# jltsiren/gbwt-rs

Measured on AMD Instinct MI355X. Metric: LF-steps/sec (batched path extract), higher is better.
Workload: dtype u32; 1 GPU; bubble-chain GBZ, 5000 paths x 1000002 nodes (333334 sites, mosaic, seed 42), all forward sequences -> device CSR; index replicated, path p walked by GPU p mod 1; lf_steps_per_gpu=3333340000, index_bytes=59619086, records=2000005

## Files before the change

### gbwt_rs_amd/_lib.py

```python
import ctypes as C
import os
import sys

HERE = os.path.dirname(os.path.abspath(__file__))
CSRC = os.path.join(HERE, "csrc")
LIB_PATH = os.environ.get("GBWT_HIP_LIB") or os.path.join(CSRC, "libgbwt_hip.so")
HEADER = os.path.join(os.path.dirname(HERE), "include", "gbwt_hip.h")

OPEN_EXTRACT, OPEN_SEARCH, OPEN_GFA, OPEN_ALL = 1, 2, 4, 7
OK, INVALID_DATA, IO_ERROR, BAD_ARGUMENT, NO_DEVICE, DEVICE_ERROR, CAPACITY, UNSUPPORTED = range(8)
STATUS_NAMES = ["OK", "INVALID_DATA", "IO_ERROR", "BAD_ARGUMENT", "NO_DEVICE", "DEVICE_ERROR", "CAPACITY", "UNSUPPORTED"]


class Pos(C.Structure):
    _fields_ = [("node", C.c_uint64), ("offset", C.c_uint64)]


class State(C.Structure):
    _fields_ = [("node", C.c_uint64), ("start", C.c_uint64), ("end", C.c_uint64)]


class BdState(C.Structure):
    _fields_ = [("forward", State), ("reverse", State)]


class Stats(C.Structure):
    _fields_ = [("size", C.c_uint64), ("sequences", C.c_uint64), ("alphabet_size", C.c_uint64),
                ("alphabet_offset", C.c_uint64), ("records", C.c_uint64), ("data_bytes", C.c_uint64),
                ("paths", C.c_uint64), ("bidirectional", C.c_uint32), ("has_metadata", C.c_uint32),
                ("is_gbz", C.c_uint32), ("has_translation", C.c_uint32), ("max_record_len", C.c_uint64),
                ("max_outdegree", C.c_uint64)]


class OpenTimes(C.Structure):
    _fields_ = [("parse_ms", C.c_double), ("upload_ms", C.c_double), ("sample_ms", C.c_double), ("total_ms", C.c_double),
                ("samples", C.c_uint64), ("checkpoint_walkers", C.c_uint64), ("checkpoint_orphans", C.c_uint64), ("checkpoint_sampling", C.c_uint32),
                ("checkpoint_rounds", C.c_uint32), ("line_sizes_ms", C.c_double)]


class Memory(C.Structure):
    _fields_ = [("index_device_bytes", C.c_uint64), ("index_host_bytes", C.c_uint64), ("workspace_device_bytes", C.c_uint64),
                ("rows_bytes", C.c_uint64), ("text_bytes", C.c_uint64), ("rows_chunks", C.c_uint64)]


class UniqueId(C.Structure):
    _fields_ = [("bytes", C.c_ubyte * 128)]


class CommStats(C.Structure):
    _fields_ = [("ms", C.c_double), ("bytes", C.c_uint64), ("staged_send", C.c_uint32), ("reserved", C.c_uint32)]


class Paths(C.Structure):
    _fields_ = [("d_offsets", C.c_void_p), ("d_nodes", C.c_void_p), ("total", C.c_uint64), ("n", C.c_uint64)]


class States(C.Structure):
    _fields_ = [("d_states", C.c_void_p), ("d_valid", C.c_void_p), ("n", C.c_uint64)]


class Lines(C.Structure):
    _fields_ = [("d_text", C.c_void_p), ("d_line_offsets", C.c_void_p), ("total", C.c_uint64), ("n", C.c_uint64)]


class Components(C.Structure):
    _fields_ = [("d_component", C.c_void_p), ("d_offsets", C.c_void_p), ("d_nodes", C.c_void_p), ("d_path_component", C.c_void_p),
                ("min_node", C.c_uint64), ("slots", C.c_uint64), ("components", C.c_uint64), ("nodes", C.c_uint64), ("paths", C.c_uint64)]


class ComponentsTimes(C.Structure):
    _fields_ = [("hook_ms", C.c_float), ("jump_ms", C.c_float), ("shape_ms", C.c_float), ("hook_launches", C.c_uint32),
                ("jump_launches", C.c_uint32), ("shape_launches", C.c_uint32)]


class EdgeRows(C.Structure):
    _fields_ = [("d_offsets", C.c_void_p), ("d_edges", C.c_void_p), ("d_valid", C.c_void_p), ("total", C.c_uint64), ("n", C.c_uint64)]


class GraphText(C.Structure):
    _fields_ = [("d_text", C.c_void_p), ("header_bytes", C.c_uint64), ("segment_bytes", C.c_uint64), ("link_bytes", C.c_uint64),
                ("segments", C.c_uint64), ("links", C.c_uint64)]


class SuffixArray(C.Structure):
    _fields_ = [("d_sa", C.c_void_p), ("d_bwt", C.c_void_p), ("total", C.c_uint64), ("bwt_runs", C.c_uint64)]


class SuffixArrayInfo(C.Structure):
    _fields_ = [("n", C.c_uint64), ("peak_scratch_bytes", C.c_uint64), ("planned_scratch_bytes", C.c_uint64), ("bwt_runs", C.c_uint64),
                ("active", C.c_uint64 * 64), ("rounds", C.c_uint32), ("rank_bits", C.c_uint32), ("text_ms", C.c_float), ("pack_ms", C.c_float),
                ("rank_ms", C.c_float), ("output_ms", C.c_float), ("round_ms", C.c_float * 64)]


FM_COUNT_ONLY = 1


class FmIndexInfo(C.Structure):
    _fields_ = [(name, C.c_uint64) for name in ("n", "sigma", "block_rows", "blocks", "primary", "index_bytes", "planned_index_bytes", "sa_bytes", "peak_scratch_bytes",
                                                "planned_scratch_bytes", "queries", "last_patterns", "last_steps", "last_total")] + \
               [(name, C.c_uint32) for name in ("packed", "count_only", "path_level", "reserved")] + \
               [(name, C.c_float) for name in ("suffix_array_ms", "histogram_ms", "codes_ms", "counts_ms", "fill_ms", "narrow_ms", "last_count_ms", "last_fill_ms")]


class FmLocated(C.Structure):
    _fields_ = [("d_offsets", C.c_void_p), ("d_values", C.c_void_p), ("d_ranges", C.c_void_p), ("total", C.c_uint64), ("m", C.c_uint64)]


class ReferencePath(C.Structure):
    _fields_ = [("path_id", C.c_uint64), ("len", C.c_uint64), ("first", C.c_uint64), ("count", C.c_uint64)]


class ReferencePosition(C.Structure):
    _fields_ = [("offset", C.c_uint64), ("pos", Pos)]


class Located(C.Structure):
    _fields_ = [("d_offsets", C.c_void_p), ("d_ids", C.c_void_p), ("d_valid", C.c_void_p), ("total", C.c_uint64), ("n", C.c_uint64)]


class LocateInfo(C.Structure):
# ... 219 lines not shown
```

### gbwt_rs_amd/csrc/capi_open.hip

```cpp
#include <hip/hip_runtime.h>

#include <algorithm>
#include <cstdio>
#include <cstdlib>
#include <cstring>
#include <memory>
#include <mutex>
#include <new>
#include <atomic>
#include <chrono>
#include <string>
#include <thread>
#include <vector>

#include "capi_internal.hpp"

using namespace gbwt_hip;


namespace gbwt_hip {
std::string &last_error_slot() {
    thread_local std::string slot;
    return slot;
}
// ... 180 lines not shown
    HIP_CHECK(hipMemcpy(&bad, flags.ptr, sizeof(uint32_t), hipMemcpyDeviceToHost));
    HIP_CHECK(hipGetLastError());
    if (bad != 0) throw InvalidData("BWT: record starts are not sorted offsets into the data");
    ix.starts_uploaded = true;
}

void records_to_device(gbwt_hip_index &ix, OpenTrace &trace) {
    const HostIndex &h = ix.host;
    if (h.alphabet_size > (uint64_t(1) << 32)) throw Unsupported("alphabet_size > 2^32 is not supported (u32 node ids on device)");
    HIP_CHECK(hipSetDevice(ix.device));
    const uint64_t n_records = ix.stats.records;
    const uint64_t data_bytes = ix.stats.data_bytes;
    if (!ix.record_bytes_uploaded) {
        ix.data.reserve(data_bytes + DATA_PAD);
        HIP_CHECK(hipMemset(ix.data.ptr, 0, data_bytes + DATA_PAD));
    }
    DeviceIndex &d = ix.dev;
    d = DeviceIndex{};
    d.data = ix.data.as<uint8_t>();
    d.data_len = data_bytes;
    d.n_records = n_records;
    d.n_sequences = h.sequences;
    d.alphabet_offset = static_cast<uint32_t>(h.alphabet_offset);
    d.first_node = static_cast<uint32_t>(h.alphabet_offset + 1);
    const bool narrow_starts = data_bytes < (uint64_t(1) << 32);
    if (!ix.starts_uploaded) upload_starts(ix);
    if (!ix.record_bytes_uploaded && data_bytes) HIP_CHECK(hipMemcpy(ix.data.ptr, h.record_bytes(), data_bytes, hipMemcpyHostToDevice));
    if (narrow_starts) d.starts32 = ix.starts.as<uint32_t>(); else d.starts64 = ix.starts.as<uint64_t>();
    trace.mark("record bytes + starts to the device");
}

void build_descriptors(gbwt_hip_index &ix, uint64_t *d_stats, DeviceBuffer &counts, DeviceBuffer &scan_tmp, OpenTrace &trace) {
    const HostIndex &h = ix.host;
    DeviceIndex &d = ix.dev;
    const uint64_t n_records = d.n_records, nr = std::max<uint64_t>(n_records, 1);
    if (ix.caps & GBWT_HIP_OPEN_EXTRACT) ix.desc.reserve(nr * 4 * sizeof(uint4));
    ix.desc_raw.reserve(nr * 4 * sizeof(uint4));
    ix.block_base.reserve(nr * sizeof(uint32_t));
    counts.reserve(nr * sizeof(uint32_t));
    trace.mark("starts + allocations");
    launch_build_desc(d, ix.desc_raw.as<uint4>(), counts.as<uint32_t>(), d_stats, nullptr);
    trace.mark("k_build_desc");
    d.desc_raw = ix.desc_raw.as<uint4>();
    d.desc = ix.desc.as<uint4>();
    uint64_t n_blocks = 1;
    if (n_records > 0) {
        if (n_records >= (uint64_t(1) << 30)) throw Unsupported("more than 2^30 records are not supported");
        if ((h.size >> RANK_BLOCK_SHIFT) + n_records >= 0xFFFFFFF0ull) throw Unsupported("index too large for 32-bit rank block indices");
        size_t tb = block_scan_temp_bytes(n_records);
        scan_tmp.reserve(std::max<size_t>(tb, 16));
        launch_block_scan(counts.as<uint32_t>(), ix.block_base.as<uint32_t>(), n_records, scan_tmp.ptr, tb, nullptr);
        uint32_t last_base = 0, last_count = 0;
        HIP_CHECK(hipMemcpy(&last_base, ix.block_base.as<uint32_t>() + (n_records - 1), sizeof(uint32_t), hipMemcpyDeviceToHost));
        HIP_CHECK(hipMemcpy(&last_count, counts.as<uint32_t>() + (n_records - 1), sizeof(uint32_t), hipMemcpyDeviceToHost));
        n_blocks += static_cast<uint64_t>(last_base) + last_count;
        launch_finish_block_base(counts.as<uint32_t>(), ix.block_base.as<uint32_t>(), n_records, ix.desc_raw.as<uint4>(), nullptr);
    }
    ix.blocks.reserve(n_blocks * sizeof(uint4));
    HIP_CHECK(hipMemsetAsync(ix.blocks.ptr, 0, sizeof(uint4), nullptr));
    d.block_base = ix.block_base.as<uint32_t>();
    d.blocks = ix.blocks.as<uint4>();
    d.n_blocks = n_blocks;
    trace.mark("block scan + allocation");
    if (n_blocks > 1) launch_fill_blocks(d, counts.as<uint32_t>(), ix.block_base.as<uint32_t>(), ix.blocks.as<uint4>(), nullptr);
    trace.mark("k_fill_blocks");
}

uint64_t layout_walks(gbwt_hip_index &ix, uint64_t *d_stats, const DeviceBuffer &counts, OpenTrace &trace) {
    const HostIndex &h = ix.host;
    const OpenKnobs &k = ix.knobs;
    DeviceIndex &d = ix.dev;
    const uint64_t n_records = d.n_records, n_blocks = d.n_blocks;
    launch_link_desc(d, ix.desc.as<uint4>(), nullptr);
    const uint32_t hops = k.lookahead_hops;
    launch_link_lookahead(d, ix.desc.as<uint4>(), counts.as<uint32_t>(), hops, nullptr);
    ix.desc2.reserve(std::max<uint64_t>(n_records, 1) * 8 * sizeof(uint4));
    d.desc2 = ix.desc2.as<uint4>();
    uint32_t gather_limit = k.gather_limit;
    if (n_blocks >= (uint64_t(1) << 31)) gather_limit = 0;
    ix.packed_blocks = gather_limit != 0;
    trace.mark("link + lookahead + allocations");
    const uint32_t chain_max = k.chains.value_or(CHAIN_MAX);
    HIP_CHECK(hipMemsetAsync(d_stats + 6, 0, sizeof(uint64_t), nullptr));
    launch_link_desc2(d, ix.desc2.as<uint4>(), gather_limit, chain_max | (h.bidirectional ? 0x100u : 0u), reinterpret_cast<uint32_t *>(d_stats + 5), nullptr);
    ix.gblocks.reserve((gather_limit ? n_blocks : 1) * 2 * sizeof(uint4));
    HIP_CHECK(hipMemsetAsync(ix.gblocks.ptr, 0, 2 * sizeof(uint4), nullptr));
    d.gblocks = ix.gblocks.as<uint4>();
    uint64_t early_stats[6] = {0, 0, 0, 0, 0, 0};
    HIP_CHECK(hipMemcpy(early_stats, d_stats, sizeof(early_stats), hipMemcpyDeviceToHost));
    d.chained = static_cast<uint32_t>(early_stats[5] & 0xFFFFFFFFu);
    if (d.chained != 0 && !k.chains && (early_stats[5] >> 32) * 1000 < n_records) {
        HIP_CHECK(hipMemset(d_stats + 5, 0, 2 * sizeof(uint64_t)));
        launch_link_desc2(d, ix.desc2.as<uint4>(), gather_limit, h.bidirectional ? 0x100u : 0u, reinterpret_cast<uint32_t *>(d_stats + 5), nullptr);
        d.chained = 0;
    }
    if (trace.on) std::fprintf(stderr, "[open] records with a chained step: %llu of %llu (up to %u nodes per iteration)\n",
                               static_cast<unsigned long long>(early_stats[5] >> 32), static_cast<unsigned long long>(n_records), d.chained);
    const uint64_t longest = early_stats[0];
    const bool full_width_now = gather_limit == 0 || longest >= gather_limit;
    if (full_width_now) {
        ix.cblocks.reserve(n_blocks * 2 * sizeof(uint4));
        HIP_CHECK(hipMemsetAsync(ix.cblocks.ptr, 0, 2 * sizeof(uint4), nullptr));
    }
    if (n_blocks > 1) launch_fill_two_step_blocks(d, full_width_now ? ix.cblocks.as<uint4>() : nullptr, gather_limit ? ix.gblocks.as<uint4>() : nullptr, nullptr);
    if (full_width_now) d.cblocks = ix.cblocks.as<uint4>();
    trace.mark("two-step descriptors + blocks");
    launch_link_lookahead2(d, ix.desc2.as<uint4>(), counts.as<uint32_t>(), std::max<uint32_t>(1, (hops + 1) / 2), nullptr);
    return early_stats[4];
}

void build_tables(gbwt_hip_index &ix, uint64_t generic_records, DeviceBuffer &scan_tmp) {
    const OpenKnobs &k = ix.knobs;
    DeviceIndex &d = ix.dev;
    const uint64_t n_records = d.n_records;
    if (n_records == 0 || generic_records == 0) return;
    const bool for_extract = (ix.caps & GBWT_HIP_OPEN_EXTRACT) != 0;
    DeviceBuffer positions, sigmas, table_base, edge_base, edges;
    positions.reserve(n_records * sizeof(uint64_t)); sigmas.reserve(n_records * sizeof(uint64_t));
    table_base.reserve((n_records + 1) * sizeof(uint64_t)); edge_base.reserve((n_records + 1) * sizeof(uint64_t));
    launch_table_counts(d, positions.as<uint64_t>(), sigmas.as<uint64_t>(), nullptr);
    const size_t tb = scan_temp_bytes(n_records);
    scan_tmp.reserve(std::max<size_t>(tb, 16));
    launch_scan(positions.as<uint64_t>(), table_base.as<uint64_t>(), n_records, scan_tmp.ptr, tb, nullptr);
    launch_scan(sigmas.as<uint64_t>(), edge_base.as<uint64_t>(), n_records, scan_tmp.ptr, tb, nullptr);
    uint64_t total_positions = 0, total_edges = 0;
    HIP_CHECK(hipMemcpy(&total_positions, table_base.as<uint64_t>() + n_records, sizeof(uint64_t), hipMemcpyDeviceToHost));
    HIP_CHECK(hipMemcpy(&total_edges, edge_base.as<uint64_t>() + n_records, sizeof(uint64_t), hipMemcpyDeviceToHost));
    uint64_t budget = uint64_t(16) << 30;
    {
        size_t free_bytes = 0, total_bytes = 0;
        if (hipMemGetInfo(&free_bytes, &total_bytes) == hipSuccess) budget = std::min<uint64_t>(total_bytes / 4, free_bytes / 2);
        else (void)hipGetLastError();
    }
    if (k.table_bytes) budget = *k.table_bytes;
    if (total_positions == 0 || total_positions >= 0xFFFFFFFFull || total_positions * sizeof(uint4) > budget) return;
    ix.tables.reserve(total_positions * sizeof(uint4));
    edges.reserve(std::max<uint64_t>(total_edges, 1) * sizeof(uint2));
    d.tables = ix.tables.as<uint4>();
    launch_fill_tables(d, ix.desc_raw.as<uint4>(), table_base.as<uint64_t>(), edge_base.as<uint64_t>(), ix.tables.as<uint4>(), edges.as<uint2>(), nullptr);
    HIP_CHECK(hipDeviceSynchronize());
    HIP_CHECK(hipGetLastError());
    if (!(for_extract && 2 * total_positions * sizeof(uint4) <= budget && n_records <= 0x7FFFFFFFull && k.walk_tables)) return;
    ix.wtables.reserve(total_positions * sizeof(uint4));
    launch_fill_wtables(d, ix.wtables.as<uint4>(), nullptr);
    HIP_CHECK(hipDeviceSynchronize());
    HIP_CHECK(hipGetLastError());
    d.wtables = ix.wtables.as<uint4>();
    ix.table_positions = total_positions;
    if (6 * total_positions * sizeof(uint4) <= budget && k.deep_tables) {
        ix.wtables_deep.reserve(total_positions * 4 * sizeof(uint4));
        launch_fill_wtables_deep(d, ix.wtables_deep.as<uint4>(), k.compact_tables, nullptr);
        HIP_CHECK(hipDeviceSynchronize());
        HIP_CHECK(hipGetLastError());
        d.wtables_deep = ix.wtables_deep.as<uint4>();
    }
}

void record_stats_and_endmarker(gbwt_hip_index &ix, const uint64_t (&hs)[8], const Endmarker *early_endmarker) {
    ix.stats.max_record_len = hs[0];
    ix.stats.max_outdegree = hs[1];
    if (ix.caps & GBWT_HIP_OPEN_EXTRACT) ix.slow_records = hs[6] & 0xFFFFFFFFull;
    if (hs[2] != 0) throw InvalidData("BWT: record without a readable outdegree");
    if (hs[0] >= (uint64_t(1) << 32)) throw Unsupported("a record with 2^32 or more positions is not supported (u32 offsets on device)");
    DeviceIndex &d = ix.dev;
    d.max_walk = hs[3];
    const Endmarker endmarker = early_endmarker ? *early_endmarker : decompress_endmarker(ix.host, std::max<uint64_t>(hs[0], 1));
    const uint64_t end_len = endmarker.size();
    ix.endmarker.reserve(std::max<uint64_t>(end_len, 1) * sizeof(uint2));
    static_assert(sizeof(std::pair<uint32_t, uint32_t>) == sizeof(uint2), "pairs are uploaded as uint2");
    if (end_len > 0) HIP_CHECK(hipMemcpy(ix.endmarker.ptr, endmarker.data(), end_len * sizeof(uint2), hipMemcpyHostToDevice));
    d.endmarker = ix.endmarker.as<uint2>();
    d.n_endmarker = end_len;
}

uint64_t all_nodes(const HostIndex &h) { return h.size >= h.sequences ? h.size - h.sequences : 0; }

uint32_t sample_interval(gbwt_hip_index &ix) {
    const HostIndex &h = ix.host;
    const DeviceIndex &d = ix.dev;
    const uint64_t nodes = all_nodes(h);
    uint32_t interval = 64;
    while (interval < 2048 && (nodes >> 22) > interval) interval *= 2;
    while (interval < 2048 && ((nodes / h.sequences) >> 12) > interval) interval *= 2;
    if (d.wtables_deep != nullptr && 3 * ix.table_positions >= h.size)
        while (interval < 512 && (interval < 128 || (nodes >> 17) > interval)) interval *= 2;
    ix.sample_coarse = 1;
    if (ix.knobs.sample_interval) interval = *ix.knobs.sample_interval;
    else if (interval >= 1024 && d.chained == 0) {
        const uint32_t coarse = ix.knobs.sample_coarse.value_or(interval / 512);
        ix.sample_coarse = coarse; interval = std::max(64u, interval / coarse);
    }
    return interval;
}

enum class Sampling { checkpoints, one_walk, two_pass };

Sampling walk_every_sequence(gbwt_hip_index &ix, Sampling how, uint32_t interval, const DeviceBuffer &prints, uint64_t *d_stats, DeviceBuffer &pool,
                             DeviceBuffer &tags, uint64_t &pooled) {
    const HostIndex &h = ix.host;
    DeviceIndex &d = ix.dev;
    uint32_t *d_flags = reinterpret_cast<uint32_t *>(d_stats);
    d.cblocks = ensure_cblocks(&ix);
    if (how == Sampling::one_walk) {
        const uint64_t pool_capacity = all_nodes(h) / std::max<uint32_t>(interval, 1) + 2 * h.sequences + 1024;
        pool.reserve(pool_capacity * sizeof(uint4)); tags.reserve(pool_capacity * sizeof(uint2));
        HIP_CHECK(hipMemset(d_stats + 2, 0, sizeof(uint64_t)));
        HIP_CHECK(hipMemsetAsync(d_flags + 1, 0, sizeof(uint32_t), nullptr));
        launch_lengths_and_samples(d, interval, ix.seq_len.as<uint32_t>(), pool.as<uint4>(), tags.as<uint2>(), d_stats + 2, pool_capacity, d_flags, nullptr);
        HIP_CHECK(hipMemcpy(&pooled, d_stats + 2, sizeof(uint64_t), hipMemcpyDeviceToHost));
        if (pooled <= pool_capacity) return Sampling::one_walk;
    }
    HIP_CHECK(hipMemsetAsync(d_flags + 1, 0, sizeof(uint32_t), nullptr));
    launch_sequence_lengths(d, ix.seq_len.as<uint32_t>(), prints.as<uint64_t>(), d_flags, nullptr);
    return Sampling::two_pass;
}

void samples_after_walk(gbwt_hip_index &ix, Sampling how, uint32_t interval, const DeviceBuffer &pool, const DeviceBuffer &tags, uint64_t pooled) {
    const HostIndex &h = ix.host;
    DeviceBuffer counts, scan_tmp;
    counts.reserve(h.sequences * sizeof(uint64_t));
    ix.sample_base.reserve((h.sequences + 1) * sizeof(uint64_t));
    launch_sample_counts(ix.seq_len.as<uint32_t>(), h.sequences, interval, counts.as<uint64_t>(), nullptr);
    const size_t tb = scan_temp_bytes(h.sequences);
    scan_tmp.reserve(std::max<size_t>(tb, 16));
    launch_scan(counts.as<uint64_t>(), ix.sample_base.as<uint64_t>(), h.sequences, scan_tmp.ptr, tb, nullptr);
    uint64_t total_samples = 0;
    HIP_CHECK(hipMemcpy(&total_samples, ix.sample_base.as<uint64_t>() + h.sequences, sizeof(uint64_t), hipMemcpyDeviceToHost));
    ix.samples.reserve(std::max<uint64_t>(total_samples, 1) * sizeof(uint4));
    if (how == Sampling::one_walk) launch_place_samples(ix.seq_len.as<uint32_t>(), pool.as<uint4>(), tags.as<uint2>(), pooled, ix.sample_base.as<uint64_t>(), h.sequences,
                                                        ix.samples.as<uint4>(), nullptr);
    else launch_record_samples(ix.dev, ix.sample_base.as<uint64_t>(), interval, ix.samples.as<uint4>(), nullptr);
    HIP_CHECK(hipDeviceSynchronize());
    HIP_CHECK(hipGetLastError());
    ix.times.samples = total_samples;
    std::vector<uint64_t> base(h.sequences + 1);
    HIP_CHECK(hipMemcpy(base.data(), ix.sample_base.ptr, base.size() * sizeof(uint64_t), hipMemcpyDeviceToHost));
    note_sample_counts(ix, base);
}

void lengths_and_samples(gbwt_hip_index &ix, uint64_t *d_stats, OpenTrace &trace) {
    const HostIndex &h = ix.host;
    DeviceIndex &d = ix.dev;
    const auto t_samples = std::chrono::steady_clock::now();
    ix.seq_len.reserve(h.sequences * sizeof(uint32_t));
// ... 291 lines not shown
```

### gbwt_rs_amd/csrc/device_index.hpp

```cpp
#pragma once

#include <cstdint>

namespace gbwt_hip {

constexpr uint32_t DESC_UNARY = 0xFFFFFFFFu;
constexpr uint32_t EDGE_EMIT2 = 1u << 31;
constexpr uint32_t EDGE_CONT = 1u << 30;
constexpr uint32_t DESC_SLOW = 1u << 31;
constexpr uint32_t LOOKAHEAD_COUNT_MASK = (1u << 29) - 1;
constexpr uint32_t REC_MASK = (1u << 30) - 1;
constexpr uint32_t LEAF_EMIT2 = 1u << 31;
constexpr uint32_t DESC2_SLOW = 1u << 30;
constexpr uint32_t GATHER_OK = 1u;
constexpr uint32_t E_CHAIN = 2u;
constexpr uint32_t E_ALL4 = 8u;
constexpr uint32_t E_ANYCHAIN = 4u;
constexpr uint32_t LEAF_CHAIN = 1u << 30;
constexpr uint32_t CHAIN_MAX = 6;
constexpr uint32_t WT_TABLE = 1u << 30;
constexpr uint32_t WT_DEEP_STEPS = 7;
constexpr uint32_t WT_COMPACT_STEPS = 12;
constexpr uint32_t WT_COMPACT = 1u << 30;
constexpr uint32_t WT_COMPACT_TABLE = 1u << 29;
constexpr uint32_t BLOCK_NONE = 0xFFFFFFFFu;
constexpr uint32_t RANK_BLOCK_SHIFT = 6;
constexpr uint32_t DATA_PAD = 128;

struct DeviceIndex {
    const uint8_t *data;
    const uint32_t *starts32;
    const uint64_t *starts64;
    const uint2 *endmarker;
    const uint4 *desc;
    const uint4 *desc_raw;
    const uint32_t *block_base;
    const uint4 *blocks;
    const uint4 *desc2;
    const uint4 *tables;
    const uint4 *wtables;
    const uint4 *wtables_deep;
    const uint32_t *seq_len;
    const uint4 *samples;
    const uint64_t *sample_base;
    uint32_t sample_interval;
    uint32_t sample_stride;
    uint32_t sample_part, sample_parts;
    const uint4 *cblocks;
    const uint4 *gblocks;
    uint64_t data_len;
    uint64_t n_records;
    uint64_t n_sequences;
    uint64_t n_endmarker;
    uint64_t n_blocks;
    uint64_t max_walk;
    uint32_t alphabet_offset;
    uint32_t first_node;
    uint32_t chained;
};

struct RowSegments { uint64_t base, stride, count, lo, hi; };
__device__ inline RowSegments row_segments(const DeviceIndex &ix, uint64_t id) {
    RowSegments r;
    r.stride = ix.sample_stride ? ix.sample_stride : 1u;
    r.base = ix.sample_base[id];
    r.count = (ix.sample_base[id + 1] - r.base + r.stride - 1) / r.stride;
    r.lo = 0; r.hi = r.count;
    if (ix.sample_parts > 1) { r.lo = r.count * ix.sample_part / ix.sample_parts; r.hi = r.count * (ix.sample_part + 1) / ix.sample_parts; }
    return r;
}
__device__ inline uint64_t segment_position(const DeviceIndex &ix, const RowSegments &r, uint64_t id, uint64_t j) {
    return j == 0 ? 0u : (j < r.count ? ix.samples[r.base + j * r.stride].w : ix.seq_len[id]);
}

__host__ __device__ inline uint32_t chain_stride(uint32_t x, uint32_t L) { return L > x ? 2u : 0xFFFFFFFEu; }
__host__ __device__ inline uint32_t chain_mids(uint32_t x, uint32_t L) { return (L > x ? L - x : x - L) / 2 - 1; }

__host__ __device__ inline uint32_t desc_body_offset(uint32_t meta) { return meta & 0xFFFFu; }
__host__ __device__ inline uint32_t desc_class(uint32_t meta) { return (meta >> 16) & 3u; }
__host__ __device__ inline uint64_t desc_start(uint32_t start_lo, uint32_t meta) { return (static_cast<uint64_t>(meta >> 24) << 32) | start_lo; }

}
```

### gbwt_rs_amd/csrc/kernels.hpp

```cpp
#pragma once

#include <hip/hip_runtime.h>

#include <cstdint>

#include "../../include/gbwt_hip.h"
#include "device_index.hpp"

namespace gbwt_hip {

constexpr uint32_t POOL_BLOCK_NODES = 256;
constexpr uint32_t POOL_NONE = 0xFFFFFFFFu;

constexpr uint32_t FLAG_POOL_OVERFLOW = 1u;

void launch_build_desc(const DeviceIndex &ix, uint4 *d_desc, uint32_t *d_block_counts, uint64_t *d_stats, hipStream_t stream);
size_t block_scan_temp_bytes(uint64_t n);
void launch_block_scan(const uint32_t *d_counts, uint32_t *d_block_base, uint64_t n, void *d_temp, size_t temp_bytes, hipStream_t stream);
void launch_finish_block_base(const uint32_t *d_counts, uint32_t *d_block_base, uint64_t n, uint4 *d_desc_raw , hipStream_t stream);
void launch_link_desc(const DeviceIndex &ix, uint4 *d_desc, hipStream_t stream);
void launch_link_lookahead(const DeviceIndex &ix, uint4 *d_desc, const uint32_t *d_block_counts, uint32_t hops, hipStream_t stream);
void launch_table_counts(const DeviceIndex &ix, uint64_t *d_positions, uint64_t *d_sigmas, hipStream_t stream);
void launch_fill_tables(const DeviceIndex &ix, uint4 *d_desc_raw, const uint64_t *d_table_base, const uint64_t *d_edge_base, uint4 *d_tables,
                        uint2 *d_edges, hipStream_t stream);
void launch_fill_wtables(const DeviceIndex &ix, uint4 *d_wtables, hipStream_t stream);
void launch_fill_wtables_deep(const DeviceIndex &ix, uint4 *d_deep, bool compact, hipStream_t stream);
void launch_link_desc2(const DeviceIndex &ix, uint4 *d_desc2, uint32_t gather_limit, uint32_t chain_max, uint32_t *d_chained, hipStream_t stream);
void launch_fill_two_step_blocks(const DeviceIndex &ix, uint4 *d_cblocks , uint4 *d_gblocks , hipStream_t stream);
void launch_link_lookahead2(const DeviceIndex &ix, uint4 *d_desc2, const uint32_t *d_block_counts, uint32_t hops, hipStream_t stream);
void launch_fill_blocks(const DeviceIndex &ix, const uint32_t *d_block_counts, const uint32_t *d_block_base, uint4 *d_blocks, hipStream_t stream);

struct WalkArgs {
    const uint64_t *seq_ids;
    uint64_t n;
    uint32_t *pool;
    uint32_t *next;
    uint32_t pool_blocks;
    uint32_t *counter;
    uint32_t *head;
    uint64_t *lengths;
    uint32_t *flags;
    uint32_t mode;
    uint32_t paths_per_wave;
    uint32_t small_record;
    uint32_t pack16;
    uint32_t helper_lanes;
    uint32_t wide_addresses;
    uint32_t *out_nodes;
    const uint64_t *out_offsets;
    uint32_t both_ends;
    uint32_t ring_slots;
    uint32_t helper_naps;
    uint32_t row_piece;
    uint32_t xcd_map;
    uint32_t uniform_loop;
    uint32_t headroom;
    uint32_t all4;
    uint32_t catch_up;
    uint32_t gather_reach;
    uint32_t packed_blocks;
    uint32_t debug;
    const uint32_t *sorted_rows;
    const uint64_t *level;
    uint64_t walkers;
    uint64_t capacity;
    uint32_t segments;
    uint32_t uniform_len;
    uint64_t *fill_offsets;
};
constexpr uint32_t WALK_TWO_STEP = 0, WALK_LANE_SERIAL = 1, WALK_COOP = 2, WALK_ONE_STEP = 3;
void launch_walk(const DeviceIndex &ix, const WalkArgs &args, hipStream_t stream);
void launch_sequence_lengths(const DeviceIndex &ix, uint32_t *d_seq_len, uint64_t *d_prints, uint32_t *d_overflow, hipStream_t stream);
void launch_check_orientation_pairs(const uint32_t *d_seq_len, const uint64_t *d_prints, uint64_t n_pairs, uint32_t *d_mismatch, hipStream_t stream);
void launch_gather_lengths(const uint32_t *d_seq_len, uint64_t n_sequences, const uint64_t *d_ids, uint64_t n, uint64_t *d_lengths, uint32_t *d_max_len, hipStream_t stream);
void launch_lengths_and_samples(const DeviceIndex &ix, uint32_t interval, uint32_t *d_seq_len, uint4 *d_pool, uint2 *d_tags, uint64_t *d_counter,
                                uint64_t capacity, uint32_t *d_overflow, hipStream_t stream);
void launch_place_samples(const uint32_t *d_seq_len, const uint4 *d_pool, const uint2 *d_tags, uint64_t pooled, const uint64_t *d_sample_base,
                          uint64_t n_sequences, uint4 *d_samples, hipStream_t stream);
void launch_sample_counts(const uint32_t *d_seq_len, uint64_t n_sequences, uint32_t interval, uint64_t *d_counts, hipStream_t stream);
void launch_record_samples(const DeviceIndex &ix, const uint64_t *d_sample_base, uint32_t interval, uint4 *d_samples, hipStream_t stream);
struct CheckpointWalk {
    const uint64_t *cp_first;
    uint4 *summaries;
    uint64_t *orphan_count;
    uint64_t orphan_capacity, positions;
    uint32_t threshold, cap;
    uint32_t packed;
    uint32_t *flags;
};
void launch_checkpoint_counts(const DeviceIndex &ix, uint32_t threshold, uint64_t *d_counts, hipStream_t stream);
void launch_checkpoint_walk(const DeviceIndex &ix, const CheckpointWalk &w, hipStream_t stream);
void launch_chase_counts(const DeviceIndex &ix, const uint4 *d_summaries, uint64_t n_summaries, uint4 *d_spans, uint32_t *d_seq_len, uint64_t *d_counts,
                         uint32_t *d_overflow, hipStream_t stream);
void launch_chase_samples(const DeviceIndex &ix, const uint4 *d_summaries, uint64_t n_summaries, const uint4 *d_spans, const uint64_t *d_sample_base,
                          uint4 *d_samples, hipStream_t stream);
constexpr uint32_t GFA_LINE_CHUNK = 4096;
struct LineCacheFill {
    const uint32_t *label_len;
    uint64_t n_labels;
    uint64_t paths;
    uint32_t max_samples;
    const uint64_t *chunk_first;
    uint64_t chunks;
    uint64_t *chunk_text;
    uint64_t *path_totals;
    uint32_t *chunk_seg;
    uint64_t *seg_text;
    uint32_t *flags;
};
void launch_fill_line_cache(const DeviceIndex &ix, const LineCacheFill &f, bool packed, hipStream_t stream);
// ... 78 lines not shown
```

### gbwt_rs_amd/csrc/knobs.hpp

```cpp
#pragma once

#include <algorithm>
#include <cstdint>
#include <cstdlib>
#include <optional>

#include "device_index.hpp"
#include "extract_knobs.hpp"

struct OpenKnobs {
    bool seq_len = true;
    std::optional<uint32_t> sample_interval;
    std::optional<uint32_t> sample_coarse;
    bool serial_samples = false;
    bool two_pass = false;
    bool orientation_check = false;
    std::optional<double> checkpoint_gap;
    std::optional<uint32_t> checkpoint_cap;
    std::optional<uint32_t> chains;
    uint32_t gather_limit = 1u << 21;
    uint32_t lookahead_hops = 15;
    bool walk_tables = true, deep_tables = true, compact_tables = true;
    std::optional<uint64_t> table_bytes;
    bool line_cache = true;
    uint32_t locate_interval = 64;
    bool trace = false;
    static OpenKnobs from_env() {
        OpenKnobs k;
        const auto on = [](const char *name) { const char *v = std::getenv(name); return !(v && std::atoi(v) == 0); };
        const auto forced = [](const char *name) { const char *v = std::getenv(name); return v && std::atoi(v) != 0; };
        k.seq_len = on("GBWT_HIP_SEQ_LEN");
        if (const char *v = std::getenv("GBWT_HIP_SAMPLE_INTERVAL")) k.sample_interval = static_cast<uint32_t>(std::max(0, std::atoi(v)));
        if (const char *v = std::getenv("GBWT_HIP_SAMPLE_COARSE")) k.sample_coarse = static_cast<uint32_t>(std::max(1, std::atoi(v)));
        k.serial_samples = forced("GBWT_HIP_SERIAL_SAMPLES");
        k.two_pass = forced("GBWT_HIP_TWO_PASS_OPEN");
        k.orientation_check = forced("GBWT_HIP_ORIENTATION_CHECK");
        if (const char *v = std::getenv("GBWT_HIP_CHECKPOINT_GAP")) k.checkpoint_gap = std::max(2.0, std::atof(v));
        if (const char *v = std::getenv("GBWT_HIP_CHECKPOINT_CAP")) k.checkpoint_cap = static_cast<uint32_t>(std::max(1, std::atoi(v)));
        if (const char *v = std::getenv("GBWT_HIP_CHAINS")) k.chains = static_cast<uint32_t>(std::min<long>(gbwt_hip::CHAIN_MAX, std::max<long>(0, std::atol(v))));
        if (const char *v = std::getenv("GBWT_HIP_GATHER_LIMIT")) k.gather_limit = static_cast<uint32_t>(std::min<long>(1l << 21, std::max<long>(0, std::atol(v))));
        if (const char *v = std::getenv("GBWT_HIP_LOOKAHEAD_HOPS")) k.lookahead_hops = static_cast<uint32_t>(std::max(0, std::atoi(v)));
        k.walk_tables = on("GBWT_HIP_WALK_TABLES"); k.deep_tables = on("GBWT_HIP_DEEP_TABLES"); k.compact_tables = on("GBWT_HIP_COMPACT_TABLES");
        if (const char *v = std::getenv("GBWT_HIP_TABLE_BYTES")) k.table_bytes = std::strtoull(v, nullptr, 10);
        k.line_cache = on("GBWT_HIP_LINE_CACHE");
        if (const char *v = std::getenv("GBWT_HIP_LOCATE_INTERVAL")) k.locate_interval = static_cast<uint32_t>(std::min<long>(1l << 30, std::max<long>(0, std::atol(v))));
        k.trace = std::getenv("GBWT_HIP_TRACE_OPEN") != nullptr;
        return k;
    }
    static bool lazy_host_records() {
        static const bool lazy = [] { const char *e = std::getenv("GBWT_HIP_LAZY_HOST_RECORDS"); return !(e && e[0] == '0'); }();
        return lazy;
    }
};
```

### gbwt_rs_amd/csrc/load_kernels.hip

```cpp
#include "kernels.hpp"

#include <hipcub/hipcub.hpp>

#include "device_common.hpp"
#include "lf_device.hpp"

namespace gbwt_hip {

namespace {


__device__ __forceinline__ uint4 stream_bytes16(const uint8_t *data, uint64_t pos, uint64_t limit) {
    uint32_t w[4] = {0, 0, 0, 0};
    for (uint32_t k = 0; k < 16 && pos + k < limit; k++) w[k >> 2] |= static_cast<uint32_t>(data[pos + k]) << (8 * (k & 3));
    return make_uint4(w[0], w[1], w[2], w[3]);
}

__global__ void __launch_bounds__(256) k_build_desc(DeviceIndex ix, uint4 *desc, uint32_t *block_counts, uint64_t *stats) {
    const uint64_t rec = blockIdx.x * static_cast<uint64_t>(blockDim.x) + threadIdx.x;
    uint64_t stat_len = 0, stat_sigma = 0, stat_bad = 0, stat_generic = 0;
    if (rec < ix.n_records) {
    uint64_t start, limit;
    record_bounds(ix, rec, start, limit);
    uint4 A = make_uint4(0, 0, 0, 0), B = make_uint4(0, 0, 0, 0), C = make_uint4(0, 0, 0, 0), D = make_uint4(0, 0, 0, 0);
    uint32_t n_blocks = 0;
    if (limit > start) {
        ByteCursor c(ix.data, start, limit);
        uint64_t sigma = 0;
        const bool readable = c.varint(sigma);
        if (!readable) stat_bad = 1;
        if (readable && sigma != 0) {
            stat_sigma = sigma;
            B.x = static_cast<uint32_t>(start); B.y = static_cast<uint32_t>(limit - start);
            B.z = static_cast<uint32_t>((start >> 32) & 0xFF) << 24;
            bool classed = false;
            if (sigma <= 2 && (start >> 40) == 0) {
                uint64_t n0 = 0, o0 = 0, d1 = 0, o1 = 0;
                bool good = c.varint(n0) && c.varint(o0);
                if (good && sigma == 2) good = c.varint(d1) && c.varint(o1);
                const uint64_t body = c.pos - start;
                if (good && body <= 0xFFFF && n0 + d1 <= 0xFFFFFFFFull && o0 <= 0xFFFFFFFFull && o1 <= 0xFFFFFFFFull) {
                    RunDecoder rd(sigma);
                    uint64_t total = 0, total0 = 0, runs = 0, value, len;
                    bool lean = true;
                    for (;;) {
                        const uint64_t before = c.pos;
                        if (!rd.next(c, value, len)) break;
                        if (c.pos - before > 5) lean = false;
                        total += len; runs++;
                        if (value == 0) total0 += len;
                    }
                    if (!c.at_end() || runs == 0) lean = false;
                    if (lean && total < 0xFFFFFFFFull) {
                        classed = true;
                        stat_len = total;
                        A.x = static_cast<uint32_t>(n0); A.y = static_cast<uint32_t>(o0);
                        A.z = static_cast<uint32_t>(n0 + d1); A.w = static_cast<uint32_t>(o1);
                        B.z |= static_cast<uint32_t>(body) | (static_cast<uint32_t>(sigma) << 16);
                        B.w = static_cast<uint32_t>(total);
                        C.x = static_cast<uint32_t>(total0); C.y = static_cast<uint32_t>(total);
                        D = stream_bytes16(ix.data, start + body, limit);
                        if (sigma == 1) B.y = DESC_UNARY;
                        else n_blocks = static_cast<uint32_t>((total >> RANK_BLOCK_SHIFT) + 1);
                    }
                }
            }
            if (!classed) {
                stat_generic = rec != 0 ? 1 : 0;
                A = make_uint4(0, 0, 0, 0); C = make_uint4(0, 0, 0, 0); D = make_uint4(0, 0, 0, 0); B.w = 0;
                uint64_t total = ix.n_sequences;
                if (rec != 0) {
                    ByteCursor c2(ix.data, start, limit);
                    uint64_t s2 = 0;
                    c2.varint(s2);
                    total = record_len(c2, s2);
                }
                stat_len = total;
                C.y = total < 0xFFFFFFFFull ? static_cast<uint32_t>(total) : 0xFFFFFFFFu;
            }
        }
    }
    desc[4 * rec] = A;
    desc[4 * rec + 1] = B;
    desc[4 * rec + 2] = C;
    desc[4 * rec + 3] = D;
    block_counts[rec] = n_blocks;
    }
// ... 193 lines not shown
        if (compact) {
            uint32_t node[2 * WT_COMPACT_STEPS];
            uint4 f = e;
            bool ok = true;
            for (uint32_t k = 0; k < WT_COMPACT_STEPS && ok; k++) {
                if (k > 0) f = ix.wtables[static_cast<uint64_t>(f.w) + f.y];
                const bool table_next = (f.z & WT_TABLE) != 0;
                ok = f.x != 0 && (f.z & LEAF_EMIT2) != 0 && (f.z & REC_MASK) != 0 && (table_next || k + 1 == WT_COMPACT_STEPS);
                node[2 * k] = f.x; node[2 * k + 1] = (f.z & REC_MASK) + ix.alphabet_offset;
            }
            for (uint32_t k = 1; k < 2 * WT_COMPACT_STEPS && ok; k++) {
                const int64_t d = static_cast<int64_t>(node[k]) - static_cast<int64_t>(node[k - 1]);
                ok = d >= -32768 && d <= 32767;
            }
            if (ok) {
                w[0] = node[0];
                w[1] = WT_COMPACT | ((f.z & WT_TABLE) ? WT_COMPACT_TABLE : 0u);
                for (uint32_t q = 0; q < 12; q++) {
                    const uint32_t a = 2 * q + 1, b = 2 * q + 2;
                    const uint32_t lo = (node[a] - node[a - 1]) & 0xFFFFu;
                    const uint32_t hi = b < 2 * WT_COMPACT_STEPS ? ((node[b] - node[b - 1]) & 0xFFFFu) : 0u;
                    w[2 + q] = lo | (hi << 16);
                }
                w[14] = f.y; w[15] = f.w;
                uint4 *out = deep + 4 * (static_cast<uint64_t>(C.z) + i);
                out[0] = make_uint4(w[0], w[1], w[2], w[3]);
                out[1] = make_uint4(w[4], w[5], w[6], w[7]);
                out[2] = make_uint4(w[8], w[9], w[10], w[11]);
                out[3] = make_uint4(w[12], w[13], w[14], w[15]);
                continue;
            }
        }
        bool going = true;
#pragma unroll
        for (uint32_t k = 0; k < WT_DEEP_STEPS; k++) {
            if (going) {
                if (k > 0) e = ix.wtables[static_cast<uint64_t>(e.w) + e.y];
                w[2 * k] = e.x; w[2 * k + 1] = e.z & ~WT_TABLE;
                going = (e.z & REC_MASK) != 0 && (e.z & WT_TABLE) != 0;
            } else {
                w[2 * k] = 0u; w[2 * k + 1] = e.z & REC_MASK;
            }
        }
        if ((e.z & REC_MASK) != 0 && (e.z & WT_TABLE) != 0) w[2 * WT_DEEP_STEPS - 1] |= WT_TABLE;
        w[14] = e.y; w[15] = e.w;
        uint4 *out = deep + 4 * (static_cast<uint64_t>(C.z) + i);
        out[0] = make_uint4(w[0], w[1], w[2], w[3]);
        out[1] = make_uint4(w[4], w[5], w[6], w[7]);
        out[2] = make_uint4(w[8], w[9], w[10], w[11]);
        out[3] = make_uint4(w[12], w[13], w[14], w[15]);
    }
}

__device__ __forceinline__ uint32_t extend_chain(const DeviceIndex &ix, uint32_t x, uint32_t &w, uint64_t &base, uint64_t count, uint32_t room, bool bidirectional) {
    const uint4 *raw = ix.desc_raw;
    const uint32_t first = w + ix.alphabet_offset;
    if (first != x + 2u && first != x - 2u) return 0;
    const uint32_t d = chain_stride(x, first);
    uint32_t added = 0;
    while (added < room) {
        const uint4 WA = raw[4 * static_cast<uint64_t>(w)], WB = raw[4 * static_cast<uint64_t>(w) + 1];
        if (WB.y != DESC_UNARY || WA.x == 0 || WA.x != w + ix.alphabet_offset + d) break;
        if (bidirectional) {
            uint64_t rev = 0;
            if (!landing_record(ix, (w + ix.alphabet_offset) ^ 1u, rev) || raw[4 * rev + 1].y != DESC_UNARY) break;
        }
        uint64_t next = 0;
        if (!landing_record(ix, WA.x, next)) break;
        const uint4 NB = raw[4 * next + 1];
        const uint64_t base2 = base + WA.y;
        if (NB.y == 0 || base2 + count > 0xFFFFFFFFull || !(desc_class(NB.z) == 0 || base2 + count <= NB.w)) break;
        w = static_cast<uint32_t>(next); base = base2; added++;
    }
    return added;
}

__device__ __forceinline__ uint64_t edge_positions(const DeviceIndex &ix, uint64_t r, uint32_t e) {
    const uint4 B = ix.desc_raw[4 * r + 1], C = ix.desc_raw[4 * r + 2];
    const uint32_t cls = B.y != 0 ? desc_class(B.z) : 0u;
    if (cls == 2) return e ? B.w - C.x : C.x;
    return cls == 1 && e == 0 ? B.w : 0u;
}

__global__ void __launch_bounds__(256) k_link_desc2(DeviceIndex ix, uint4 *out, uint32_t gather_limit, uint32_t chain_max, uint32_t *chained) {
    uint64_t v = blockIdx.x * static_cast<uint64_t>(blockDim.x) + threadIdx.x;
    if (v >= ix.n_records) return;
    const uint4 *d1 = ix.desc;
    const uint4 D = d1[4 * v + 2];
    const uint4 VB = ix.desc_raw[4 * v + 1];
    const uint32_t cls_v = VB.y != 0 ? desc_class(VB.z) : 0u;
    uint32_t n1[2] = {0, 0}, base[2] = {0, 0}, wword[2] = {0, 0}, chain[2] = {0, 0};
    bool any_chain = false;
    uint4 leaf[4] = {make_uint4(0, 0, 0, BLOCK_NONE), make_uint4(0, 0, 0, BLOCK_NONE), make_uint4(0, 0, 0, BLOCK_NONE), make_uint4(0, 0, 0, BLOCK_NONE)};
    const bool slow = (D.x & DESC_SLOW) != 0;
    if (!slow) {
        for (uint32_t a = 0; a < 2; a++) {
            const uint4 E = d1[4 * v + a];
            const uint32_t f = a ? D.w : D.y;
            n1[a] = E.x; base[a] = E.y;
            if (!(f & EDGE_CONT)) continue;
            uint32_t w = E.z, wbb = E.w;
            if ((f & EDGE_EMIT2) && chain_max != 0) {
                uint64_t chained_base = base[a];
                if (extend_chain(ix, E.x, w, chained_base, edge_positions(ix, v, a), chain_max & 0xFFu, (chain_max >> 8) != 0) != 0) {
                    base[a] = static_cast<uint32_t>(chained_base); wbb = ix.block_base[w]; chain[a] = E_CHAIN; any_chain = true;
                }
            }
            wword[a] = w | ((f & EDGE_EMIT2) ? LEAF_EMIT2 : 0u);
            const uint4 WD = d1[4 * static_cast<uint64_t>(w) + 2];
            const uint4 WB = ix.desc_raw[4 * static_cast<uint64_t>(w) + 1];
            const uint32_t cls_w = WB.y != 0 ? desc_class(WB.z) : 0u;
            const bool real = !(WD.x & DESC_SLOW) && (cls_w == 1 || (cls_w == 2 && cls_v == 2));
            if (!real) { leaf[2 * a] = make_uint4(0u, 0u, w, wbb); continue; }
            for (uint32_t b = 0; b < cls_w; b++) {
                const uint4 WE = d1[4 * static_cast<uint64_t>(w) + b];
                const uint32_t wf = b ? WD.w : WD.y;
                const bool cont = (wf & EDGE_CONT) != 0;
                uint32_t land = WE.z, lbb = WE.w, lflag = 0;
                uint64_t lbase = WE.y;
                if (cont && (wf & EDGE_EMIT2) && chain_max != 0 && extend_chain(ix, WE.x, land, lbase, edge_positions(ix, w, b), chain_max & 0xFFu, (chain_max >> 8) != 0) != 0) {
                    lbb = ix.block_base[land]; lflag = LEAF_CHAIN; any_chain = true;
                }
                leaf[2 * a + b] = make_uint4(WE.x, static_cast<uint32_t>(lbase), cont ? (land | lflag | ((wf & EDGE_EMIT2) ? LEAF_EMIT2 : 0u)) : 0u, cont ? lbb : BLOCK_NONE);
            }
        }
    }
    bool packed = VB.w < gather_limit;
    for (uint32_t a = 0; a < 2; a++)
        if (wword[a] & REC_MASK) packed = packed && ix.desc_raw[4 * static_cast<uint64_t>(wword[a] & REC_MASK) + 1].w < gather_limit;
    bool all4 = !slow && !any_chain && cls_v != 0;
    for (uint32_t a = 0; a < cls_v && all4; a++) {
        all4 = n1[a] != 0 && (wword[a] & LEAF_EMIT2) != 0;
        const uint4 WB = ix.desc_raw[4 * static_cast<uint64_t>(wword[a] & REC_MASK) + 1];
        const uint32_t cls_w = WB.y != 0 ? desc_class(WB.z) : 0u;
        all4 = all4 && cls_w != 0;
        for (uint32_t b = 0; b < cls_w && all4; b++) all4 = leaf[2 * a + b].x != 0 && (leaf[2 * a + b].z & LEAF_EMIT2) != 0;
    }
    if (slow && VB.y != 0 && chained != nullptr) atomicAdd(chained + 2, 1u);
    uint4 *o = out + 8 * v;
    o[0] = make_uint4(n1[0], base[0], wword[0] | (slow ? DESC2_SLOW : 0u), (packed ? GATHER_OK : 0u) | chain[0] | (any_chain ? E_ANYCHAIN : 0u) | (all4 ? E_ALL4 : 0u));
    o[1] = make_uint4(n1[1], base[1], wword[1] | (slow ? DESC2_SLOW : 0u), (packed ? GATHER_OK : 0u) | chain[1]);
    if (any_chain && chained != nullptr) {
        uint32_t most = 0;
        for (uint32_t a = 0; a < 2; a++) {
            const uint32_t first = 2u + (chain[a] ? chain_mids(n1[a], (wword[a] & REC_MASK) + ix.alphabet_offset) : 0u);
            for (uint32_t b = 0; b < 2; b++) {
                const uint4 l = leaf[2 * a + b];
                most = max(most, first + 2u + ((l.z & LEAF_CHAIN) ? chain_mids(l.x, (l.z & REC_MASK) + ix.alphabet_offset) : 0u));
            }
        }
        if (*chained < most) atomicMax(chained, most);
    }
    {
        const uint64_t lanes = __ballot(any_chain && chained != nullptr);
        if (lanes != 0 && (threadIdx.x % WAVE) == static_cast<uint32_t>(__ffsll(static_cast<unsigned long long>(lanes)) - 1)) atomicAdd(chained + 1, static_cast<uint32_t>(__popcll(lanes)));
    }
    o[2] = leaf[0]; o[3] = leaf[1]; o[4] = leaf[2]; o[5] = leaf[3];
    o[6] = make_uint4(0u, 0u, 0u, 0u);
    o[7] = make_uint4(0u, 0u, 0u, 0u);
}

struct SecondStep { const uint4 *wblocks[2]; uint32_t wbase[2]; };

template <class Mask>
__device__ __forceinline__ Mask second_step_bits(const uint4 *wblocks, uint32_t j, Mask m, uint32_t &R) {
    const uint32_t q = j >> RANK_BLOCK_SHIFT, sh = j & 63u;
    const uint32_t cnt = sizeof(Mask) == 8 ? __popcll(m) : __popc(static_cast<uint32_t>(m));
    const uint4 W0 = wblocks[q];
    const uint64_t w0 = (static_cast<uint64_t>(W0.y) << 32) | W0.x;
    R = W0.z + __popcll(w0 & ((uint64_t(1) << sh) - 1));
    uint64_t val = w0 >> sh;
    if (sh != 0 && cnt > 64 - sh) {
        const uint4 W1 = wblocks[q + 1];
        val |= ((static_cast<uint64_t>(W1.y) << 32) | W1.x) << (64 - sh);
    }
    Mask bits2 = 0;
    while (m) {
        const Mask low = m & (~m + 1);
        if (val & 1) bits2 |= low;
        val >>= 1;
        m ^= low;
    }
    return bits2;
}

__global__ void __launch_bounds__(256) k_fill_two_step_blocks(DeviceIndex ix, uint4 *cblocks, uint4 *gblocks) {
    const uint64_t b = blockIdx.x * static_cast<uint64_t>(blockDim.x) + threadIdx.x + 1;
    if (b >= ix.n_blocks) return;
    const uint4 P = ix.blocks[b];
    const uint64_t v = P.w;
    const uint4 *d1 = ix.desc;
    const uint4 D = d1[4 * v + 2];
    const uint32_t len = ix.desc_raw[4 * v + 1].w;
    const uint32_t bb = ix.block_base[v];
    const uint32_t k = static_cast<uint32_t>(b - bb);
    SecondStep s2{{nullptr, nullptr}, {0, 0}};
    if (!(D.x & DESC_SLOW)) {
        for (uint32_t a = 0; a < 2; a++) {
            const uint4 E = ix.desc2[8 * v + a];
            const uint64_t w = E.z & REC_MASK;
            if (w == 0) continue;
            const uint4 WB = ix.desc_raw[4 * w + 1];
            if ((d1[4 * w + 2].x & DESC_SLOW) || WB.y == 0 || desc_class(WB.z) != 2) continue;
            s2.wblocks[a] = ix.blocks + ix.block_base[w];
            s2.wbase[a] = E.y;
        }
    }
    {
        const uint64_t bits1 = (static_cast<uint64_t>(P.y) << 32) | P.x;
        const uint32_t remaining = len - (k << RANK_BLOCK_SHIFT) > len ? 0u : len - (k << RANK_BLOCK_SHIFT);
        const uint64_t valid = remaining >= 64 ? ~uint64_t(0) : ((uint64_t(1) << remaining) - 1);
        uint64_t bits2 = 0, m_of[2] = {0, 0};
        uint32_t R[2] = {0, 0};
        for (uint32_t a = 0; a < 2; a++) {
            const uint64_t m = (a ? bits1 : ~bits1) & valid;
            if (!s2.wblocks[a] || m == 0) continue;
            m_of[a] = m;
            const uint32_t before = a ? P.z : (k << RANK_BLOCK_SHIFT) - P.z;
            bits2 |= second_step_bits<uint64_t>(s2.wblocks[a], s2.wbase[a] + before, m, R[a]);
        }
        if (cblocks != nullptr) {
            cblocks[2 * static_cast<uint64_t>(bb + k)] = make_uint4(P.x, P.y, static_cast<uint32_t>(bits2), static_cast<uint32_t>(bits2 >> 32));
            cblocks[2 * static_cast<uint64_t>(bb + k) + 1] = make_uint4(P.z, R[0], R[1], 0u);
        }
        if (gblocks == nullptr) return;
        const uint32_t lo2 = static_cast<uint32_t>(bits2), hi2 = static_cast<uint32_t>(bits2 >> 32);
        uint32_t Rlo[2], Rhi[2];
        for (uint32_t a = 0; a < 2; a++) {
            const uint32_t mlo = static_cast<uint32_t>(m_of[a]), mhi = static_cast<uint32_t>(m_of[a] >> 32);
            Rlo[a] = mlo ? R[a] : 0u;
            Rhi[a] = mhi ? R[a] + __popc(lo2 & mlo) : 0u;
        }
        const uint32_t ones_hi = P.z + __popc(P.x);
        gblocks[2 * static_cast<uint64_t>(bb + k)] = make_uint4(P.x, lo2, (P.z & 0x1FFFFFu) | (Rlo[0] << 21), ((Rlo[0] >> 11) & 0x3FFu) | (Rlo[1] << 10));
        gblocks[2 * static_cast<uint64_t>(bb + k) + 1] = make_uint4(P.y, hi2, (ones_hi & 0x1FFFFFu) | (Rhi[0] << 21), ((Rhi[0] >> 11) & 0x3FFu) | (Rhi[1] << 10));
    }
}

__global__ void __launch_bounds__(256) k_link_lookahead2(DeviceIndex ix, uint4 *desc2, const uint32_t *block_counts, uint32_t hops) {
    uint64_t v = blockIdx.x * static_cast<uint64_t>(blockDim.x) + threadIdx.x;
    if (v >= ix.n_records) return;
    uint64_t r = v;
    bool good = true;
    for (uint32_t h = 0; h < hops && good; h++) {
        if (desc2[8 * r].z & DESC2_SLOW) { good = false; break; }
        const uint32_t x = desc2[8 * r + 2].z & REC_MASK;
        if (x == 0) good = false; else r = x;
    }
    uint4 look = make_uint4(0u, 0u, 0u, 0u);
    if (good && r != v) {
        look.x = static_cast<uint32_t>(r);
        if (ix.block_base[r] != BLOCK_NONE) { look.y = ix.block_base[r]; look.z = block_counts[r]; }
    }
    desc2[8 * v + 6] = look;
}

__global__ void __launch_bounds__(256) k_fill_blocks(DeviceIndex ix, const uint32_t *block_counts, const uint32_t *block_base, uint4 *blocks) {
    uint64_t rec = blockIdx.x * static_cast<uint64_t>(blockDim.x) + threadIdx.x;
    if (rec >= ix.n_records) return;
    const uint32_t count = block_counts[rec];
    if (count == 0) return;
    const uint4 B = ix.desc_raw[4 * rec + 1];
    const uint64_t start = desc_start(B.x, B.z), limit = start + B.y;
    ByteCursor c(ix.data, start + desc_body_offset(B.z), limit);
    RunDecoder rd(desc_class(B.z));
    uint4 *out = blocks + block_base[rec];
    uint64_t bits = 0, value, len;
    uint32_t k = 0, fill = 0, ones = 0;
    while (k < count && rd.next(c, value, len)) {
        while (len > 0 && k < count) {
            const uint32_t take = static_cast<uint32_t>(len < 64 - fill ? len : 64 - fill);
            if (value) bits |= (take == 64 ? ~uint64_t(0) : ((uint64_t(1) << take) - 1)) << fill;
            fill += take; len -= take;
            if (fill == 64) {
                out[k++] = make_uint4(static_cast<uint32_t>(bits), static_cast<uint32_t>(bits >> 32), ones, static_cast<uint32_t>(rec));
                ones += __popcll(bits);
                bits = 0; fill = 0;
            }
        }
    }
    if (k < count) out[k] = make_uint4(static_cast<uint32_t>(bits), static_cast<uint32_t>(bits >> 32), ones, static_cast<uint32_t>(rec));
}

}

void launch_build_desc(const DeviceIndex &ix, uint4 *d_desc, uint32_t *d_block_counts, uint64_t *d_stats, hipStream_t stream) {
    if (ix.n_records == 0) return;
    hipLaunchKernelGGL(k_build_desc, dim3(grid_for(ix.n_records, 256)), dim3(256), 0, stream, ix, d_desc, d_block_counts, d_stats);
}

void launch_link_desc(const DeviceIndex &ix, uint4 *d_desc, hipStream_t stream) {
    if (ix.n_records == 0) return;
    hipLaunchKernelGGL(k_link_desc, dim3(grid_for(ix.n_records, 256)), dim3(256), 0, stream, ix, d_desc);
}

void launch_link_lookahead(const DeviceIndex &ix, uint4 *d_desc, const uint32_t *d_block_counts, uint32_t hops, hipStream_t stream) {
    if (ix.n_records == 0) return;
    hipLaunchKernelGGL(k_link_lookahead, dim3(grid_for(ix.n_records, 256)), dim3(256), 0, stream, ix, d_desc, d_block_counts, hops);
}

void launch_table_counts(const DeviceIndex &ix, uint64_t *d_positions, uint64_t *d_sigmas, hipStream_t stream) {
    if (ix.n_records == 0) return;
    hipLaunchKernelGGL(k_table_counts, dim3(grid_for(ix.n_records, 256)), dim3(256), 0, stream, ix, d_positions, d_sigmas);
}

void launch_fill_tables(const DeviceIndex &ix, uint4 *d_desc_raw, const uint64_t *d_table_base, const uint64_t *d_edge_base, uint4 *d_tables,
                        uint2 *d_edges, hipStream_t stream) {
    if (ix.n_records == 0) return;
    hipLaunchKernelGGL(k_fill_tables, dim3(grid_for(ix.n_records, 64)), dim3(64), 0, stream, ix, d_desc_raw, d_table_base, d_edge_base, d_tables, d_edges);
}

void launch_fill_wtables(const DeviceIndex &ix, uint4 *d_wtables, hipStream_t stream) {
    if (ix.n_records == 0 || ix.n_records > 0x7FFFFFFFull) return;
    hipLaunchKernelGGL(k_fill_wtables, dim3(static_cast<unsigned>(ix.n_records)), dim3(256), 0, stream, ix, d_wtables);
}

void launch_fill_wtables_deep(const DeviceIndex &ix, uint4 *d_deep, bool compact, hipStream_t stream) {
    if (ix.n_records == 0 || ix.n_records > 0x7FFFFFFFull || ix.wtables == nullptr) return;
    hipLaunchKernelGGL(k_fill_wtables_deep, dim3(static_cast<unsigned>(ix.n_records)), dim3(256), 0, stream, ix, d_deep, compact ? 1u : 0u);
}

void launch_link_desc2(const DeviceIndex &ix, uint4 *d_desc2, uint32_t gather_limit, uint32_t chain_max, uint32_t *d_chained, hipStream_t stream) {
    if (ix.n_records == 0) return;
    hipLaunchKernelGGL(k_link_desc2, dim3(grid_for(ix.n_records, 256)), dim3(256), 0, stream, ix, d_desc2, gather_limit, chain_max, d_chained);
}

void launch_fill_two_step_blocks(const DeviceIndex &ix, uint4 *d_cblocks, uint4 *d_gblocks, hipStream_t stream) {
    if (ix.n_records == 0 || (d_cblocks == nullptr && d_gblocks == nullptr)) return;
    if (ix.n_blocks <= 1) return;
    hipLaunchKernelGGL(k_fill_two_step_blocks, dim3(grid_for(ix.n_blocks - 1, 256)), dim3(256), 0, stream, ix, d_cblocks, d_gblocks);
}

void launch_link_lookahead2(const DeviceIndex &ix, uint4 *d_desc2, const uint32_t *d_block_counts, uint32_t hops, hipStream_t stream) {
    if (ix.n_records == 0) return;
    hipLaunchKernelGGL(k_link_lookahead2, dim3(grid_for(ix.n_records, 256)), dim3(256), 0, stream, ix, d_desc2, d_block_counts, hops);
}

void launch_fill_blocks(const DeviceIndex &ix, const uint32_t *d_block_counts, const uint32_t *d_block_base, uint4 *d_blocks, hipStream_t stream) {
    if (ix.n_records == 0) return;
    hipLaunchKernelGGL(k_fill_blocks, dim3(grid_for(ix.n_records, 256)), dim3(256), 0, stream, ix, d_block_counts, d_block_base, d_blocks);
}

__global__ void __launch_bounds__(256) k_finish_block_base(const uint32_t *counts, uint32_t *block_base, uint64_t n, uint4 *desc_raw) {
    uint64_t rec = blockIdx.x * static_cast<uint64_t>(blockDim.x) + threadIdx.x;
    if (rec >= n) return;
    const uint32_t bb = counts[rec] == 0 ? BLOCK_NONE : block_base[rec] + 1;
    block_base[rec] = bb;
    if (bb != BLOCK_NONE && desc_raw != nullptr) reinterpret_cast<uint32_t *>(desc_raw + 4 * rec + 2)[2] = bb;
}

size_t block_scan_temp_bytes(uint64_t n) {
    size_t bytes = 0;
    (void)hipcub::DeviceScan::ExclusiveSum(nullptr, bytes, static_cast<const uint32_t *>(nullptr), static_cast<uint32_t *>(nullptr), static_cast<int>(n));
    return bytes;
}

void launch_block_scan(const uint32_t *d_counts, uint32_t *d_block_base, uint64_t n, void *d_temp, size_t temp_bytes, hipStream_t stream) {
    if (n == 0) return;
    (void)hipcub::DeviceScan::ExclusiveSum(d_temp, temp_bytes, d_counts, d_block_base, static_cast<int>(n), stream);
}

void launch_finish_block_base(const uint32_t *d_counts, uint32_t *d_block_base, uint64_t n, uint4 *d_desc_raw, hipStream_t stream) {
    if (n) hipLaunchKernelGGL(k_finish_block_base, dim3(grid_for(n, 256)), dim3(256), 0, stream, d_counts, d_block_base, n, d_desc_raw);
}

__global__ void __launch_bounds__(256) k_ef_counts(const uint64_t *high, uint64_t n, uint64_t *counts) {
    const uint64_t i = blockIdx.x * static_cast<uint64_t>(blockDim.x) + threadIdx.x;
    if (i < n) counts[i] = static_cast<uint64_t>(__popcll(high[i]));
}

__global__ void __launch_bounds__(256) k_ef_values(const uint64_t *high, uint64_t n, const uint64_t *rank, const uint64_t *low, uint64_t low_words, uint32_t w, uint64_t ones,
                                                    uint64_t data_len, uint32_t *out32, uint64_t *out64) {
    const uint64_t i = blockIdx.x * static_cast<uint64_t>(blockDim.x) + threadIdx.x;
    if (i == 0) { if (out32) out32[ones] = static_cast<uint32_t>(data_len); else out64[ones] = data_len; }
    if (i >= n) return;
    uint64_t word = high[i], k = rank[i];
    while (word != 0 && k < ones) {
        const uint64_t pos = i * 64 + static_cast<uint64_t>(__ffsll(static_cast<unsigned long long>(word)) - 1);
        word &= word - 1;
        const uint64_t upper = pos - k, bit = k * w, lw = bit >> 6, off = bit & 63;
        uint64_t lo = lw < low_words ? low[lw] >> off : 0;
        if (off + w > 64 && lw + 1 < low_words) lo |= low[lw + 1] << (64 - off);
        if (w < 64) lo &= (uint64_t(1) << w) - 1;
        uint64_t value = (w >= 64 ? 0 : upper << w) | lo;
        if ((w < 64 && upper != 0 && (upper >> (64 - w)) != 0) || value > data_len) value = data_len;
        if (out32) out32[k] = static_cast<uint32_t>(value); else out64[k] = value;
        k++;
    }
}

__global__ void __launch_bounds__(256) k_starts_check(const uint32_t *s32, const uint64_t *s64, uint64_t ones, uint32_t *flags) {
    const uint64_t k = blockIdx.x * static_cast<uint64_t>(blockDim.x) + threadIdx.x;
    if (k >= ones) return;
    const uint64_t a = s32 ? s32[k] : s64[k], b = s32 ? s32[k + 1] : s64[k + 1];
    if (a > b) atomicOr(flags, 1u);
}

__global__ void __launch_bounds__(256) k_mask_label_lengths(DeviceIndex ix, uint32_t *label_len, uint64_t n) {
    const uint64_t s = blockIdx.x * static_cast<uint64_t>(blockDim.x) + threadIdx.x;
    if (s >= n) return;
    if (!record_is_real(ix, 2 * s + 1)) label_len[s] = 0;
}

void launch_mask_label_lengths(const DeviceIndex &ix, uint32_t *d_label_len, uint64_t n, hipStream_t s) {
    if (n) hipLaunchKernelGGL(k_mask_label_lengths, dim3(grid_for(n, 256)), dim3(256), 0, s, ix, d_label_len, n);
}

// ... 29 lines not shown
```

### gbwt_rs_amd/csrc/open_walks.hip

```cpp
#include "kernels.hpp"

#include "walk_loops.hpp"

namespace gbwt_hip {

namespace {

constexpr uint64_t FP_P = (uint64_t(1) << 61) - 1;
constexpr uint64_t FP_X = 0x1D4F5C6B7A891234ull % FP_P;
__host__ __device__ inline uint64_t fp_mul(uint64_t a, uint64_t b) {
#ifdef __HIP_DEVICE_COMPILE__
    const uint64_t hi = __umul64hi(a, b), lo = a * b;
#else
    const unsigned __int128 t = static_cast<unsigned __int128>(a) * b;
    const uint64_t hi = static_cast<uint64_t>(t >> 64), lo = static_cast<uint64_t>(t);
#endif
    uint64_t r = (lo & FP_P) + ((lo >> 61) | (hi << 3));
    r = (r & FP_P) + (r >> 61);
    return r >= FP_P ? r - FP_P : r;
}
__host__ __device__ inline uint64_t fp_add(uint64_t a, uint64_t b) { const uint64_t r = a + b; return r >= FP_P ? r - FP_P : r; }
__host__ __device__ inline uint64_t fp_pow(uint64_t base, uint64_t e) {
    uint64_t r = 1;
    while (e) { if (e & 1) r = fp_mul(r, base); base = fp_mul(base, base); e >>= 1; }
// ... 60 lines not shown
    if (id >= ix.n_sequences) return;
    SampleSink sink;
    sink.interval = interval;
    sink.out = samples + sample_base[id];
    sink.capacity = sample_base[id + 1] - sample_base[id];
    if (sink.capacity == 0) return;
    quiet_walk(ix, id, sink, overflow);
    for (; sink.written < sink.capacity; sink.written++) sink.out[sink.written] = make_uint4(0u, 0u, BLOCK_NONE, sink.wr);
}

struct PooledSampleSink {
    uint32_t wr = 0, next = 0, interval, number = 0, id;
    uint4 *pool;
    uint2 *tags;
    unsigned long long *counter;
    uint64_t capacity;
    __device__ __forceinline__ void push(uint32_t, bool counts) { wr += counts ? 1u : 0u; }
    __device__ __forceinline__ void checkpoint(uint32_t rec, uint32_t offset, uint32_t bb) {
        if (wr < next) return;
        const uint64_t at = atomicAdd(counter, 1ull);
        if (at < capacity) { pool[at] = make_uint4(rec, offset, bb, wr); tags[at] = make_uint2(id, number); }
        number++; next += interval;
    }
};

__global__ void __launch_bounds__(256) k_lengths_and_samples(DeviceIndex ix, uint32_t interval, uint32_t *seq_len, uint4 *pool, uint2 *tags,
                                                             unsigned long long *counter, uint64_t capacity, uint32_t *overflow) {
    const uint64_t id = blockIdx.x * static_cast<uint64_t>(blockDim.x) + threadIdx.x;
    if (id >= ix.n_sequences) return;
    PooledSampleSink sink;
    sink.interval = interval; sink.id = static_cast<uint32_t>(id);
    sink.pool = pool; sink.tags = tags; sink.counter = counter; sink.capacity = capacity;
    quiet_walk(ix, id, sink, overflow);
    seq_len[id] = sink.wr;
}

__global__ void __launch_bounds__(256) k_blank_samples(const uint32_t *seq_len, const uint64_t *sample_base, uint64_t n_sequences, uint4 *samples) {
    const uint64_t id = blockIdx.x * static_cast<uint64_t>(blockDim.x) + threadIdx.x;
    if (id >= n_sequences) return;
    for (uint64_t k = sample_base[id]; k < sample_base[id + 1]; k++) samples[k] = make_uint4(0u, 0u, BLOCK_NONE, seq_len[id]);
}

__global__ void __launch_bounds__(256) k_place_samples(const uint4 *pool, const uint2 *tags, uint64_t pooled, const uint64_t *sample_base, uint4 *samples) {
    const uint64_t at = blockIdx.x * static_cast<uint64_t>(blockDim.x) + threadIdx.x;
    if (at >= pooled) return;
    const uint2 t = tags[at];
    const uint64_t base = sample_base[t.x], count = sample_base[t.x + 1] - base;
    if (t.y < count) samples[base + t.y] = pool[at];
}

__global__ void __launch_bounds__(256) k_check_orientation_pairs(const uint32_t *seq_len, const uint64_t *prints, uint64_t n_pairs, uint32_t *mismatch) {
    const uint64_t k = blockIdx.x * static_cast<uint64_t>(blockDim.x) + threadIdx.x;
    if (k >= n_pairs) return;
    const uint32_t lf = seq_len[2 * k], lr = seq_len[2 * k + 1];
    bool good = lf == lr;
    if (good && lf > 0) {
        const uint64_t shift = fp_pow(FP_X, lf - 1);
        good = prints[4 * k] == fp_mul(prints[4 * k + 3], shift) && prints[4 * k + 2] == fp_mul(prints[4 * k + 1], shift);
    }
    if (!good) atomicOr(mismatch, 1u);
}


constexpr uint32_t CP_HASH = 2654435761u;
constexpr uint32_t CP_END = 0xFFFFFFFFu;
__device__ __forceinline__ bool hashed_checkpoint(uint32_t rec, uint32_t threshold) { return rec != 0 && rec * CP_HASH < threshold; }
__device__ __forceinline__ uint32_t checkpoint_len(const DeviceIndex &ix, uint64_t rec) {
    const uint4 B = ix.desc_raw[4 * rec + 1], C = ix.desc_raw[4 * rec + 2];
    return (B.y != 0 && B.y != DESC_UNARY) ? C.y : 0u;
}

__global__ void __launch_bounds__(256) k_checkpoint_counts(DeviceIndex ix, uint32_t threshold, uint64_t *counts) {
    const uint64_t rec = blockIdx.x * static_cast<uint64_t>(blockDim.x) + threadIdx.x;
    if (rec < ix.n_records) counts[rec] = hashed_checkpoint(static_cast<uint32_t>(rec), threshold) ? checkpoint_len(ix, rec) : 0u;
}

struct NodeCounter {
    uint32_t wr = 0;
    __device__ __forceinline__ void push(uint32_t, bool counts) { wr += counts ? 1u : 0u; }
};

__device__ __forceinline__ bool counting_step(const DeviceIndex &ix, bool packed, uint32_t threshold, NodeCounter &sink, uint32_t &rec, uint32_t &offset, uint32_t &bb) {
    const uint4 *d = ix.desc2 + 8 * static_cast<uint64_t>(rec);
    uint32_t a, b, rank_a, ones_w_base, mw;
    uint4 E;
    if (packed) {
        const uint64_t idx = bb == BLOCK_NONE ? 0u : 2 * static_cast<uint64_t>(bb) + (offset >> 5);
        const uint4 K = ix.gblocks[idx];
        const uint32_t bit = offset & 31u, below = (1u << bit) - 1;
        a = (K.x >> bit) & 1u; b = (K.y >> bit) & 1u;
        E = d[a];
        if ((E.z & DESC2_SLOW) || !(E.w & GATHER_OK)) { packed = false; }
        else {
            const uint32_t ones1 = K.z & 0x1FFFFFu, R0 = ((K.z >> 21) | (K.w << 11)) & 0x1FFFFFu, R1 = K.w >> 10;
            const uint32_t m = (a ? K.x : ~K.x) & below;
            const uint32_t p = __popc(m);
            rank_a = a ? ones1 + p : (offset - bit) - ones1 + p;
            ones_w_base = a ? R1 : R0; mw = __popc(m & K.y);
        }
    }
    if (!packed) {
        const uint4 E0 = d[0];
        if (E0.z & DESC2_SLOW) { generic_step(ix, sink, rec, offset, bb); return false; }
        const uint64_t idx = bb == BLOCK_NONE ? 0u : bb + (offset >> RANK_BLOCK_SHIFT);
        const uint4 K0 = ix.cblocks[2 * idx], K1 = ix.cblocks[2 * idx + 1];
        const uint64_t bits1 = (static_cast<uint64_t>(K0.y) << 32) | K0.x, bits2 = (static_cast<uint64_t>(K0.w) << 32) | K0.z;
        const uint32_t bit = offset & 63u;
        const uint64_t below = (uint64_t(1) << bit) - 1;
        a = static_cast<uint32_t>(bits1 >> bit) & 1u; b = static_cast<uint32_t>(bits2 >> bit) & 1u;
        const uint64_t m = (a ? bits1 : ~bits1) & below;
        rank_a = a ? K1.x + __popcll(m) : (offset - bit) - K1.x + __popcll(m);
        E = a ? d[1] : E0;
        ones_w_base = a ? K1.z : K1.y; mw = __popcll(m & bits2);
    }
    const uint32_t j = E.y + rank_a, w = E.z & REC_MASK;
    sink.wr += (E.x != 0 ? 1u : 0u) + ((E.z & LEAF_EMIT2) ? 1u : 0u) + ((E.w & E_CHAIN) ? chain_mids(E.x, w + ix.alphabet_offset) : 0u);
    if (hashed_checkpoint(w, threshold)) { rec = w; offset = j; bb = BLOCK_NONE; return true; }
    const uint4 leaf = d[2 + 2 * a + b];
    const uint32_t ones_w = ones_w_base + mw;
    rec = leaf.z & REC_MASK; offset = leaf.y + (b ? ones_w : j - ones_w); bb = leaf.w;
    sink.wr += (leaf.x != 0 ? 1u : 0u) + ((leaf.z & LEAF_EMIT2) ? 1u : 0u) + ((leaf.z & LEAF_CHAIN) ? chain_mids(leaf.x, rec + ix.alphabet_offset) : 0u);
    return false;
}

struct CheckpointArgs {
    const uint64_t *cp_first;
    uint4 *summaries;
    unsigned long long *orphan_count;
    uint64_t orphan_capacity;
    uint64_t positions;
    uint32_t threshold, cap;
    uint32_t packed;
    uint32_t *flags;
};

__global__ void __launch_bounds__(256) k_checkpoint_walk(DeviceIndex ix, CheckpointArgs c) {
    const uint64_t S = ix.n_sequences;
    uint64_t g = blockIdx.x * static_cast<uint64_t>(blockDim.x) + threadIdx.x;
    uint32_t rec = 0, offset = 0, bb = BLOCK_NONE;
    bool active = g < S + c.positions;
    if (active) {
        if (g < S) {
            if (g < ix.n_endmarker) {
                const uint2 e = ix.endmarker[g];
                offset = e.y;
                if (e.x == 0 || !arrive(ix, e.x, e.y, rec, bb)) { rec = 0; bb = BLOCK_NONE; }
            }
        } else {
            const uint64_t w = g - S;
            uint64_t lo = 0, hi = ix.n_records;
            while (hi - lo > 1) {
                const uint64_t mid = (lo + hi) / 2;
                if (c.cp_first[mid] <= w) lo = mid; else hi = mid;
            }
            rec = static_cast<uint32_t>(lo); offset = static_cast<uint32_t>(w - c.cp_first[lo]); bb = ix.block_base[lo];
        }
        if (rec == 0) { c.summaries[g] = make_uint4(0u, 0u, 0u, CP_END); active = false; }
    }
    NodeCounter sink;
    const uint32_t lane = threadIdx.x % WAVE;
    while (__ballot(active) != 0) {
        bool orphan = false;
        if (active) {
            const bool between = counting_step(ix, c.packed != 0, c.threshold, sink, rec, offset, bb);
            if (rec == 0) { c.summaries[g] = make_uint4(0u, 0u, sink.wr, CP_END); active = false; }
            else if (hashed_checkpoint(rec, c.threshold) && offset < checkpoint_len(ix, rec)) {
                c.summaries[g] = make_uint4(rec, offset, sink.wr, static_cast<uint32_t>(S + c.cp_first[rec] + offset));
                active = false;
            } else {
                if (between) bb = ix.block_base[rec];
                orphan = sink.wr >= c.cap;
            }
        }
        const uint64_t mask = __ballot(orphan);
        if (mask != 0) {
            const uint32_t leader = static_cast<uint32_t>(__ffsll(static_cast<unsigned long long>(mask))) - 1;
            unsigned long long base = 0;
            if (lane == leader) base = atomicAdd(c.orphan_count, static_cast<unsigned long long>(__popcll(mask)));
            base = __shfl(base, static_cast<int>(leader));
            if (orphan) {
                const uint64_t slot = base + __popcll(mask & ((uint64_t(1) << lane) - 1));
                if (slot < c.orphan_capacity) {
                    c.summaries[g] = make_uint4(rec, offset, sink.wr, static_cast<uint32_t>(S + c.positions + slot));
                    g = S + c.positions + slot;
                    sink.wr = 0;
                } else {
                    c.summaries[g] = make_uint4(0u, 0u, sink.wr, CP_END);
                    atomicOr(c.flags, 4u);
                    active = false;
                }
            }
        }
    }
}

constexpr uint32_t SPAN_END = 0xFFFFFFFFu, SPAN_UNVISITED = 0xFFFFFFFFu, SPAN_LIMIT = 4096;
__device__ __forceinline__ bool chase_splitter(uint64_t p, uint64_t n_sequences) {
    return p < n_sequences || (static_cast<uint32_t>(p) & 15u) == ((static_cast<uint32_t>(p >> 4) * CP_HASH) >> 28);
}
__device__ __forceinline__ uint64_t span_slot(uint64_t p, uint64_t n_sequences) { return p < n_sequences ? p : n_sequences + (p >> 4); }
__device__ __forceinline__ uint64_t slot_splitter(uint64_t t, uint64_t n_sequences, uint64_t n_summaries) {
    if (t < n_sequences) return t;
    const uint64_t g = t - n_sequences, p = 16 * g + ((static_cast<uint32_t>(g) * CP_HASH) >> 28);
// ... 26 lines not shown
        const uint2 e = ix.endmarker[id];
        uint32_t rec = 0, bb = BLOCK_NONE;
        n = 1; wr = 1;
        if (arrive(ix, e.x, e.y, rec, bb)) {
            uint64_t p = id, hops = 0;
            for (;;) {
                if (p >= n_summaries || ++hops > ix.max_walk) { atomicOr(overflow, 2u); break; }
                const uint64_t slot = span_slot(p, ix.n_sequences);
                const uint4 sp = spans[slot];
                if (sp.w != SPAN_UNVISITED) { atomicOr(overflow, 8u); break; }
                spans[slot] = make_uint4(sp.x, static_cast<uint32_t>(n), static_cast<uint32_t>(wr), static_cast<uint32_t>(id));
                n += sp.y; wr += sp.z;
                if (wr > 0xFFFFFFF0ull || n > 0xFFFFFFF0ull) { atomicOr(overflow, 1u); break; }
                if (sp.x == SPAN_END) break;
                p = sp.x;
            }
        }
    }
    seq_len[id] = static_cast<uint32_t>(wr); counts[id] = n;
}

__global__ void __launch_bounds__(256) k_chase_samples(DeviceIndex ix, const uint4 *summaries, uint64_t n_summaries, const uint4 *spans, const uint64_t *sample_base, uint4 *samples) {
    const uint64_t p = slot_splitter(blockIdx.x * static_cast<uint64_t>(blockDim.x) + threadIdx.x, ix.n_sequences, n_summaries);
    if (p >= n_summaries) return;
    const uint4 sp = spans[span_slot(p, ix.n_sequences)];
    if (p < ix.n_sequences && p < ix.n_endmarker && ix.endmarker[p].x != 0) {
        const uint2 e = ix.endmarker[p];
        uint32_t rec = 0, bb = BLOCK_NONE;
        if (!arrive(ix, e.x, e.y, rec, bb)) { rec = 0; bb = BLOCK_NONE; }
        if (sample_base[p + 1] > sample_base[p]) samples[sample_base[p]] = make_uint4(rec, e.y, bb, 1u);
    }
    if (sp.w == SPAN_UNVISITED) return;
    uint4 *out = samples + sample_base[sp.w];
    const uint64_t room = sample_base[sp.w + 1] - sample_base[sp.w];
    uint64_t q = p, n = sp.y, wr = sp.z;
    for (uint32_t hops = 0; hops <= SPAN_LIMIT; hops++) {
        const uint4 s = summaries[q];
        wr += s.z;
        if (s.x == 0) break;
        if (n < room) out[n] = make_uint4(s.x, s.y, ix.block_base[s.x], static_cast<uint32_t>(wr));
        n++;
        q = s.w;
        if (q >= n_summaries || chase_splitter(q, ix.n_sequences)) break;
    }
}


__device__ __forceinline__ uint32_t w_token_bytes(uint32_t node) {
    const uint32_t v = node >> 1;
    return 2u + (v >= 10u) + (v >= 100u) + (v >= 1000u) + (v >= 10000u) + (v >= 100000u) + (v >= 1000000u) + (v >= 10000000u) + (v >= 100000000u) + (v >= 1000000000u);
}

struct TextSink {
    uint32_t wr = 0, quota = 0;
    uint64_t text = 0, labels = 0;
    uint64_t position = 0;
    const uint32_t *label_len;
    uint64_t n_labels;
    uint64_t *chunk_text;
    uint32_t *chunk_seg;
    uint32_t segment = 0, first_node = 0;
    __device__ __forceinline__ void push(uint32_t node, bool counts) {
        if (!counts) return;
        if (wr < quota) {
            if ((position & (GFA_LINE_CHUNK - 1)) == 0 && position != 0) {
                const uint64_t c = position / GFA_LINE_CHUNK;
                chunk_text[c] = text; chunk_seg[c] = segment;
            }
            text += w_token_bytes(node);
            const uint64_t seq = (static_cast<uint64_t>(node & ~1u) - first_node) / 2;
            if ((node & ~1u) >= first_node && seq < n_labels) labels += label_len[seq];
            position++;
        }
        wr++;
    }
};

template <class Sink>
__device__ __forceinline__ void emitting_step(const DeviceIndex &ix, bool packed, Sink &sink, uint32_t &rec, uint32_t &offset, uint32_t &bb) {
    const uint4 *d = ix.desc2 + 8 * static_cast<uint64_t>(rec);
    if (packed) {
        const uint64_t idx = bb == BLOCK_NONE ? 0u : 2 * static_cast<uint64_t>(bb) + (offset >> 5);
        const uint4 K = ix.gblocks[idx];
        const uint32_t bit = offset & 31u, below = (1u << bit) - 1;
        const uint32_t a = (K.x >> bit) & 1u, b = (K.y >> bit) & 1u;
        const uint4 E = d[a];
        if (!(E.z & DESC2_SLOW) && (E.w & GATHER_OK)) {
            const uint32_t ones1 = K.z & 0x1FFFFFu, R0 = ((K.z >> 21) | (K.w << 11)) & 0x1FFFFFu, R1 = K.w >> 10;
            const uint32_t m = (a ? K.x : ~K.x) & below;
            const uint32_t p = __popc(m);
            const uint32_t rank_a = a ? ones1 + p : (offset - bit) - ones1 + p;
            const uint32_t ones_w = (a ? R1 : R0) + __popc(m & K.y);
            const uint32_t j = E.y + rank_a, w = E.z & REC_MASK;
            const uint4 leaf = d[2 + 2 * a + b];
            rec = leaf.z & REC_MASK; offset = leaf.y + (b ? ones_w : j - ones_w); bb = leaf.w;
            sink.push(E.x, E.x != 0);
            if (E.w & E_CHAIN) push_chain(sink, E.x, w + ix.alphabet_offset);
            sink.push(w + ix.alphabet_offset, (E.z & LEAF_EMIT2) != 0);
            sink.push(leaf.x, leaf.x != 0);
            if (leaf.z & LEAF_CHAIN) push_chain(sink, leaf.x, rec + ix.alphabet_offset);
            sink.push(rec + ix.alphabet_offset, (leaf.z & LEAF_EMIT2) != 0);
            return;
        }
    }
    two_step(ix, sink, rec, offset, bb);
}

__global__ void __launch_bounds__(256) k_segment_text(DeviceIndex ix, LineCacheFill f, uint32_t packed) {
    const uint64_t w = blockIdx.x * static_cast<uint64_t>(blockDim.x) + threadIdx.x;
    if (w >= static_cast<uint64_t>(f.max_samples) * f.paths) return;
    const uint64_t j = w / f.paths, p = w % f.paths, id = 2 * p;
    const uint64_t base = ix.sample_base[id], count = ix.sample_base[id + 1] - base;
    if (j >= count) return;
    const uint4 here = ix.samples[base + j];
    const uint64_t len = ix.seq_len[id];
    const uint64_t from = j == 0 ? 0 : here.w;
    const uint64_t to = j + 1 < count ? ix.samples[base + j + 1].w : len;
    TextSink sink;
    sink.label_len = f.label_len; sink.n_labels = f.n_labels; sink.chunk_text = f.chunk_text + f.chunk_first[p]; sink.chunk_seg = f.chunk_seg + f.chunk_first[p];
    sink.quota = to > from ? static_cast<uint32_t>(to - from) : 0u; sink.position = from;
    sink.segment = static_cast<uint32_t>(j); sink.first_node = ix.first_node;
    uint32_t rec = here.x, offset = here.y, bb = here.z;
    if (j == 0 && id < ix.n_endmarker && ix.endmarker[id].x != 0) sink.push(ix.endmarker[id].x, true);
    while (rec != 0 && sink.wr < sink.quota) emitting_step(ix, packed != 0, sink, rec, offset, bb);
    if (sink.wr < sink.quota) atomicOr(f.flags, 1u);
    f.seg_text[2 * (base + j)] = sink.text; f.seg_text[2 * (base + j) + 1] = sink.labels;
}

__global__ void __launch_bounds__(256) k_path_text(DeviceIndex ix, LineCacheFill f) {
    const uint64_t p = blockIdx.x * static_cast<uint64_t>(blockDim.x / WAVE) + threadIdx.x / WAVE;
    const uint32_t lane = threadIdx.x % WAVE;
    if (p >= f.paths) return;
    const uint64_t base = ix.sample_base[2 * p], count = ix.sample_base[2 * p + 1] - base;
    uint64_t text_before = 0, labels = 0;
    for (uint64_t j0 = 0; j0 < count; j0 += WAVE) {
        const uint64_t j = j0 + lane;
        const uint64_t mine = j < count ? f.seg_text[2 * (base + j)] : 0u;
        labels += j < count ? f.seg_text[2 * (base + j) + 1] : 0u;
        uint64_t incl = mine;
        for (int d = 1; d < WAVE; d <<= 1) { const uint64_t up = __shfl_up(incl, d, WAVE); if (static_cast<int>(lane) >= d) incl += up; }
        if (j < count) f.seg_text[2 * (base + j)] = text_before + incl - mine;
        text_before += __shfl(incl, WAVE - 1, WAVE);
    }
    for (int d = WAVE / 2; d > 0; d >>= 1) labels += __shfl_down(labels, d, WAVE);
    if (lane == 0) { f.path_totals[2 * p] = text_before; f.path_totals[2 * p + 1] = labels; }
}

__global__ void __launch_bounds__(256) k_place_chunk_text(DeviceIndex ix, LineCacheFill f) {
    const uint64_t c = blockIdx.x * static_cast<uint64_t>(blockDim.x) + threadIdx.x;
    if (c >= f.chunks) return;
    uint64_t lo = 0, hi = f.paths;
    while (hi - lo > 1) {
        const uint64_t mid = (lo + hi) / 2;
        if (f.chunk_first[mid] <= c) lo = mid; else hi = mid;
    }
    if (c == f.chunk_first[lo]) { f.chunk_text[c] = 0; return; }
    f.chunk_text[c] += f.seg_text[2 * (ix.sample_base[2 * lo] + f.chunk_seg[c])];
}

}

void launch_fill_line_cache(const DeviceIndex &ix, const LineCacheFill &f, bool packed, hipStream_t stream) {
    if (f.paths == 0) return;
    const uint64_t walkers = static_cast<uint64_t>(f.max_samples) * f.paths;
    if (walkers) hipLaunchKernelGGL(k_segment_text, dim3(grid_for(walkers, 256)), dim3(256), 0, stream, ix, f, packed ? 1u : 0u);
    hipLaunchKernelGGL(k_path_text, dim3(grid_for(f.paths, 256 / WAVE)), dim3(256), 0, stream, ix, f);
    if (f.chunks) hipLaunchKernelGGL(k_place_chunk_text, dim3(grid_for(f.chunks, 256)), dim3(256), 0, stream, ix, f);
}

void launch_sequence_lengths(const DeviceIndex &ix, uint32_t *d_seq_len, uint64_t *d_prints, uint32_t *d_overflow, hipStream_t stream) {
    if (ix.n_sequences == 0) return;
    const uint64_t x_inverse = fp_pow(FP_X, FP_P - 2);
    hipLaunchKernelGGL(k_sequence_lengths, dim3(grid_for(ix.n_sequences, 256)), dim3(256), 0, stream, ix, d_seq_len, d_prints, x_inverse, d_overflow);
}

void launch_check_orientation_pairs(const uint32_t *d_seq_len, const uint64_t *d_prints, uint64_t n_pairs, uint32_t *d_mismatch, hipStream_t stream) {
    if (n_pairs) hipLaunchKernelGGL(k_check_orientation_pairs, dim3(grid_for(n_pairs, 256)), dim3(256), 0, stream, d_seq_len, d_prints, n_pairs, d_mismatch);
}
// ... 55 lines not shown
```

### gbwt_rs_amd/csrc/walk_direct.hip

```cpp
#include "kernels.hpp"

#include <hipcub/hipcub.hpp>

#include "walk_loops.hpp"

namespace gbwt_hip {

namespace {


struct RowTarget {
    uint32_t *row = nullptr;
    uint64_t len = 0;
    bool backward = false;
    uint32_t share = 0;
};

__device__ __forceinline__ uint64_t row_offset(const WalkArgs &a, uint64_t k) { return a.uniform_len != 0 ? k * a.uniform_len : a.out_offsets[k]; }

__device__ __forceinline__ RowTarget row_target(const WalkArgs &a, uint64_t w) {
    RowTarget t;
    const uint64_t k = w < a.n ? w : w - a.n;
    t.backward = w >= a.n;
    t.len = row_offset(a, k + 1) - row_offset(a, k);
// ... 341 lines not shown
            }
            seen = stamp;
            if (piece) {
                const uint64_t left = piece == 32 ? coop_drain<8>(rows, lane, mine, served, done) : coop_drain<4>(rows, lane, mine, served, done);
                if (done && left == 0) break;
                if (done) continue;
            } else if (owner) {
                const uint32_t staged = lds_peek(my_mail + 3);
                asm volatile("" ::: "memory");
                writer.drain(staged);
                if (done) { for (uint32_t k = writer.drained; k < staged; k++) writer.put(k); }
                lds_poke(my_drained, writer.drained);
            }
            if (done && !piece) break;
            for (uint32_t nap = 0; nap < a.helper_naps; nap++) __builtin_amdgcn_s_sleep(4);
        }
        return;
    }

    const uint32_t mail_slot = static_cast<uint32_t>(reinterpret_cast<uintptr_t>(&mailbox[lane]));
    StageSink sink(ring_lds, lane, ring_mask);
    uint32_t rec = 0, offset = 0, bb = BLOCK_NONE;
    const uint32_t quota = target.share;
    if (owner && a.segments) {
        if (quota > 0) {
            if (begin.first_node != 0) sink.push(begin.first_node, true);
            if (sink.wr < quota) { rec = begin.rec; offset = begin.offset; bb = begin.bb; }
        }
    } else if (owner) {
        const uint64_t k = w < a.n ? w : w - a.n;
        const uint64_t id = a.seq_ids[k] ^ (target.backward ? 1u : 0u);
        if (quota > 0 && id < ix.n_endmarker && id < ix.n_sequences) {
            const uint2 e = ix.endmarker[id];
            if (e.x != 0) {
                sink.push(e.x, true);
                offset = e.y;
                if (quota <= 1 || !arrive(ix, e.x, e.y, rec, bb)) { rec = 0; bb = BLOCK_NONE; }
            }
        }
    }
    lds_poke(my_mail + 3, sink.wr);
    const uint32_t ring_base = static_cast<uint32_t>(reinterpret_cast<uintptr_t>(ring_lds + lane));
    const bool narrow = !a.wide_addresses && ix.n_records * 128 <= 0xFFFFFFFFull && ix.n_blocks * 32 <= 0xFFFFFFFFull;
#ifdef GBWT_HIP_PROBE_LOOP_SHARE
    uint32_t probe_uniform = 0, probe_vector = 0, probe_entries = 0, probe_mixed_entries = 0, probe_fell_out = 0;
#endif
    const uint32_t most = ix.chained != 0 ? ix.chained : 4u;
    bool recheck = ix.chained != 0;
    uint32_t headroom = max(8u, ix.chained);
    if (a.headroom != 0) { headroom = max(a.headroom, most); recheck = recheck || headroom < 2 * most; }
    bool full_blocks = a.packed_blocks == 0;
    uint32_t catch_credit = 2, catch_pause = 0, catch_backoff = 8;
    while (__ballot(rec != 0) != 0) {
        const uint32_t drained = lds_peek(my_drained);
        if (__ballot(sink.wr - drained > ring_mask + 1 - headroom) != 0) { __builtin_amdgcn_s_sleep(2); continue; }
        bool together = __ballot(rec != static_cast<uint32_t>(__builtin_amdgcn_readfirstlane(rec))) == 0;
        bool caught = false;
        if (!together && a.uniform_loop && a.catch_up && catch_pause == 0) {
            uint32_t lo_rec = rec != 0 ? rec : 0xFFFFFFFFu, hi_rec = rec;
            for (int d = 32; d > 0; d >>= 1) {
                lo_rec = min(lo_rec, static_cast<uint32_t>(__shfl_xor(static_cast<int>(lo_rec), d)));
                hi_rec = max(hi_rec, static_cast<uint32_t>(__shfl_xor(static_cast<int>(hi_rec), d)));
            }
            if (hi_rec - lo_rec > 64u) catch_pause = 256;
        }
        if (!together && a.uniform_loop && a.catch_up && !(a.catch_up == 2u && full_blocks) && catch_pause == 0 && __ballot(sink.wr - drained > ring_mask + 1 - 8) == 0) {
            const uint64_t walking = __ballot(rec != 0);
            for (uint32_t tries = 0; tries < 4 && !together; tries++) {
                const uint32_t any = static_cast<uint32_t>(__builtin_amdgcn_readlane(static_cast<int>(rec), __builtin_ctzll(walking)));
                const bool ascending = ((any + ix.alphabet_offset) & 1u) == 0;
                uint32_t key = rec != 0 ? (ascending ? rec : ~rec) : 0u;
                uint32_t front = key;
                for (int d = 32; d > 0; d >>= 1) front = max(front, static_cast<uint32_t>(__shfl_xor(static_cast<int>(front), d)));
                const bool behind = rec != 0 && key != front;
                bool slow_here = false;
                if (behind && a.catch_up == 2u) {
                    const uint4 *d2 = ix.desc2 + 8 * static_cast<uint64_t>(rec);
                    const uint4 E0 = d2[0], E1 = d2[1];
                    const uint4 K = ix.gblocks[bb == BLOCK_NONE ? 0u : 2 * static_cast<uint64_t>(bb) + (offset >> 5)];
                    slow_here = (E0.z & DESC2_SLOW) != 0 || (E0.w & GATHER_OK) == 0 || (E0.w & (E_CHAIN | E_ANYCHAIN)) != 0 || (E1.w & E_CHAIN) != 0;
                    if (!slow_here) {
                        const uint32_t bit = offset & 31u;
                        const uint32_t value = (K.x >> bit) & 1u;
                        const uint32_t ones = (K.z & 0x1FFFFFu) + static_cast<uint32_t>(__popc(K.x & ((1u << bit) - 1u)));
                        const uint4 E = value ? E1 : E0;
                        const uint32_t land = E.z & REC_MASK;
                        rec = land; offset = E.y + (value ? ones : offset - ones);
                        bb = land != 0 ? ix.block_base[land] : BLOCK_NONE;
                        sink.push(E.x, E.x != 0);
                        sink.push(rec + ix.alphabet_offset, (E.z & LEAF_EMIT2) != 0);
                        if (sink.wr >= quota) { rec = 0; bb = BLOCK_NONE; }
                    }
                } else if (behind) {
                    const uint4 *d1 = ix.desc + 4 * static_cast<uint64_t>(rec);
                    const uint4 E0 = d1[0], E1 = d1[1], D = d1[2];
                    const uint4 K = ix.blocks[bb == BLOCK_NONE ? 0u : bb + (offset >> RANK_BLOCK_SHIFT)];
                    slow_here = (D.x & DESC_SLOW) != 0;
                    if (!slow_here) {
                        const uint64_t bits = (static_cast<uint64_t>(K.y) << 32) | K.x;
                        const uint32_t bit = offset & 63u;
                        const uint32_t value = static_cast<uint32_t>(bits >> bit) & 1u;
                        const uint32_t ones = K.z + __popcll(bits & ((uint64_t(1) << bit) - 1));
                        const uint4 E = value ? E1 : E0;
                        const uint32_t flags = value ? D.w : D.y;
                        rec = E.z; offset = E.y + (value ? ones : offset - ones); bb = E.w;
                        sink.push(E.x, E.x != 0);
                        sink.push(rec + ix.alphabet_offset, (flags & EDGE_EMIT2) != 0);
                        if (sink.wr >= quota) { rec = 0; bb = BLOCK_NONE; }
                    }
                }
                if (__ballot(slow_here) != 0) break;
                together = __ballot(rec != static_cast<uint32_t>(__builtin_amdgcn_readfirstlane(rec))) == 0;
                if (__ballot(rec != 0) != walking) break;
            }
            lds_poke(my_mail + 3, sink.wr);
            caught = together;
            if (!together && --catch_credit == 0) { catch_pause = catch_backoff; catch_backoff = min(2 * catch_backoff, 256u); catch_credit = 1; }
            if (__ballot(sink.wr - lds_peek(my_drained) > ring_mask + 1 - headroom) != 0) continue;
        } else if (catch_pause != 0) catch_pause--;
        const uint32_t wr_entry = sink.wr;
#ifdef GBWT_HIP_PROBE_LOOP_SHARE
        const uint32_t wr0 = sink.wr;
        probe_entries++;
#endif
        uint32_t slow_exit = 2;
        if (a.uniform_loop && together) {
            if (!full_blocks) slow_exit = walk2_uniform_loop(ix.desc2, ix.gblocks, ix.alphabet_offset, ring_base, mail_slot, static_cast<uint32_t>(reinterpret_cast<uintptr_t>(&row_state[lane].w)), narrow, quota, ring_mask, RING_PITCH, rec, offset, bb, sink.wr, headroom, a.all4 != 0);
            if (slow_exit == 3) full_blocks = true;
            if (full_blocks) slow_exit = walk2_uniform_loop_full(ix.desc2, ix.cblocks, ix.alphabet_offset, ring_base, mail_slot, static_cast<uint32_t>(reinterpret_cast<uintptr_t>(&row_state[lane].w)), narrow, quota, ring_mask, RING_PITCH, rec, offset, bb, sink.wr, headroom, a.all4 != 0);
        }
#ifdef GBWT_HIP_PROBE_LOOP_SHARE
        const uint32_t wr1 = sink.wr;
        probe_uniform += wr1 - wr0;
        if (!together) probe_mixed_entries++;
        if (slow_exit == 2 && together) probe_fell_out++;
#endif
        if (caught) {
            const uint32_t gained = static_cast<uint32_t>(__builtin_amdgcn_readfirstlane(static_cast<int>(sink.wr - wr_entry)));
            if (gained >= 24) { catch_credit = min(catch_credit + 1u, 4u); catch_backoff = 8; }
            else if (--catch_credit == 0) { catch_pause = catch_backoff; catch_backoff = min(2 * catch_backoff, 256u); catch_credit = 1; }
        }
        const bool mixed = slow_exit == 2;
        if (recheck && slow_exit != 0 && __ballot(sink.wr - lds_peek(my_drained) > ring_mask + 1 - headroom) != 0) continue;
        const uint32_t patience = (a.catch_up && a.uniform_loop) ? 8u * catch_pause : 0x7FFFFFFFu;
        if (mixed && patience != 0 && catch_pause != 0) catch_pause = 1;
        if (mixed) slow_exit = full_blocks ? walk2_gather_loop_full(ix.desc2, ix.cblocks, ix.alphabet_offset, ring_base, mail_slot, drained, narrow, quota, ring_mask, RING_PITCH, rec, offset, bb, sink.wr, headroom, static_cast<uint32_t>(reinterpret_cast<uintptr_t>(&row_state[lane].w)), patience)
                                           : walk2_gather_loop(ix.desc2, ix.gblocks, ix.alphabet_offset, ring_base, mail_slot, drained, narrow, quota, ring_mask, RING_PITCH, rec, offset, bb, sink.wr, headroom, static_cast<uint32_t>(reinterpret_cast<uintptr_t>(&row_state[lane].w)), patience, a.gather_reach);
#ifdef GBWT_HIP_PROBE_LOOP_SHARE
        probe_vector += sink.wr - wr1;
#endif
        if (recheck && mixed && slow_exit != 0 && __ballot(sink.wr - lds_peek(my_drained) > ring_mask + 1 - headroom) != 0) continue;
        if (slow_exit) {
            const uint4 here = ix.desc2[8 * static_cast<uint64_t>(rec)];
            bool generic = rec != 0 && (here.z & DESC2_SLOW) != 0;
            if (mixed && !full_blocks && __ballot(rec != 0 && !generic && !(here.w & GATHER_OK)) != 0) full_blocks = true;
            if (ix.wtables != nullptr) {
                bool in_table = false;
                uint32_t tb = 0;
                if (generic) {
                    const uint4 C = ix.desc_raw[4 * static_cast<uint64_t>(rec) + 2];
                    if (C.w == 1u && offset < C.y) { in_table = true; tb = C.z; generic = false; }
                }
                const bool deep = ix.wtables_deep != nullptr && ring_mask + 1 >= 64;
                const uint32_t table_slack = deep ? 16u : headroom;
                while (__ballot(in_table) != 0) {
                    if (deep && __ballot(in_table && sink.wr - lds_peek(my_drained) > ring_mask + 1 - table_slack) != 0) { __builtin_amdgcn_s_sleep(2); continue; }
                    bool compact = false;
                    const uint4 *entry = nullptr;
                    uint4 c0 = make_uint4(0, 0, 0, 0), c1 = c0;
                    if (in_table && deep) {
// ... 181 lines not shown
```

### gbwt_rs_amd/csrc/walk_loops.hpp

```cpp
#pragma once

#include <hip/hip_runtime.h>

#include "coop_device.hpp"
#include "device_common.hpp"
#include "kernels.hpp"
#include "lf_device.hpp"

namespace gbwt_hip {

namespace {


constexpr uint32_t SINK_STAGE = 16;
static_assert(POOL_BLOCK_NODES % SINK_STAGE == 0, "a block must hold a whole number of flushes");

struct PathSink {
    uint32_t *stage;
    uint32_t *wp = nullptr;
    uint32_t left = 0;
    uint32_t staged = 0;
    uint32_t cur = POOL_NONE, head = POOL_NONE, blocks = 0;
    bool overflow = false;
    __device__ __forceinline__ explicit PathSink(uint32_t *lds, uint32_t lane) : stage(lds + lane) {}
    __device__ __forceinline__ void flush(const WalkArgs &a) {
        if (staged == 0 || overflow) { staged = 0; return; }
        if (left == 0) {
            uint32_t nb = atomicAdd(a.counter, 1u);
            if (nb >= a.pool_blocks) { atomicOr(a.flags, FLAG_POOL_OVERFLOW); overflow = true; staged = 0; return; }
            a.next[nb] = POOL_NONE;
            if (cur == POOL_NONE) head = nb; else a.next[cur] = nb;
            cur = nb; blocks++;
            wp = a.pool + static_cast<uint64_t>(nb) * POOL_BLOCK_NODES;
            left = POOL_BLOCK_NODES;
        }
        if (staged == SINK_STAGE) {
            uint4 *dst = reinterpret_cast<uint4 *>(wp);
#pragma unroll
            for (uint32_t q = 0; q < SINK_STAGE / 4; q++)
                dst[q] = make_uint4(stage[(4 * q) * WAVE], stage[(4 * q + 1) * WAVE], stage[(4 * q + 2) * WAVE], stage[(4 * q + 3) * WAVE]);
        } else {
            for (uint32_t e = 0; e < staged; e++) wp[e] = stage[e * WAVE];
        }
        wp += staged; left -= staged; staged = 0;
    }
    __device__ __forceinline__ void push(const WalkArgs &a, uint32_t node) {
        stage[staged * WAVE] = node;
        staged++;
        if (__builtin_expect(staged == SINK_STAGE, 0)) flush(a);
    }
    __device__ __forceinline__ uint64_t finish(const WalkArgs &a) {
        flush(a);
        return static_cast<uint64_t>(blocks) * POOL_BLOCK_NODES - left;
    }
};



__device__ __attribute__((noinline)) uint2 serial_record_lf(const uint8_t *data, uint64_t start, uint32_t bytes, uint32_t offset) {
    ByteCursor c(data, start, start + bytes);
    uint64_t sigma, nn, no;
    if (c.varint(sigma) && sigma != 0 && record_lf(c, sigma, offset, nn, no)) return make_uint2(static_cast<uint32_t>(nn), static_cast<uint32_t>(no));
    return make_uint2(0u, 0u);
}

constexpr uint32_t RING = 64;
constexpr uint32_t RING2 = 128;
constexpr uint32_t RING_FLUSH = 16;
constexpr uint32_t RING_URGENT = RING - 4;
static_assert(POOL_BLOCK_NODES % RING_FLUSH == 0, "a block must hold a whole number of flushes");

template <uint32_t SLOTS>
struct RingSinkT {
    uint32_t *stage;
    uint32_t wr = 0, flushed = 0;
    uint32_t *wp = nullptr;
    uint32_t left = 0;
    uint32_t cur = POOL_NONE, head = POOL_NONE, blocks = 0;
    bool overflow = false;
    __device__ __forceinline__ RingSinkT(uint32_t *lds, uint32_t lane) : stage(lds + lane) {}
    __device__ __forceinline__ void push(uint32_t node, bool counts) {
        stage[(wr & (SLOTS - 1)) * WAVE] = node;
        wr += counts ? 1u : 0u;
    }
    __device__ __forceinline__ bool needs_flush() const { return wr - flushed >= RING_FLUSH; }
    __device__ __forceinline__ bool new_block(const WalkArgs &a) {
        uint32_t nb = atomicAdd(a.counter, 1u);
        if (nb >= a.pool_blocks) { atomicOr(a.flags, FLAG_POOL_OVERFLOW); overflow = true; return false; }
// ... 377 lines not shown
        "v_cmp_gt_i32_e32 vcc, 0, v114\n\t"                  \
        "v_and_b32_e32 v92, %[ringmask], v44\n\t" \
        "v_mad_u32_u24 v92, v92, %[stride], %[ring]\n\t" \
        "ds_write_b32 v92, v111\n\t" \
        "v_addc_co_u32_e32 v44, vcc, 0, v44, vcc\n\t" \
        "v_cmp_lt_u32_e32 vcc, v44, %[quota]\n\t"             \
        "v_mov_b32_e32 v79, v44\n\t"                         \
        "ds_write_b128 %[mail], v[76:79]\n\t" \
        "v_cndmask_b32_e32 v40, 0, v40, vcc\n\t" \
        "v_cndmask_b32_e32 v43, -1, v43, vcc\n\t" \
        ISSUE \
        "v_cmp_ne_u32_e64 s[44:45], 0, v40\n\t"              \
        "v_cmp_lt_u32_e32 vcc, %[limit], v44\n\t"              \
        "s_cmp_eq_u64 s[44:45], 0\n\t" \
        "s_cbranch_scc1 .Lgbwt_walk2_out_%=\n\t" \
        "s_cbranch_vccz .Lgbwt_walk2_loop_%=\n\t" \
        "s_branch .Lgbwt_walk2_out_%=\n\t" \
        ".Lgbwt_walk2_slow_%=:\n\t" \
        "s_mov_b32 %[reason], 1\n\t" \
        ".Lgbwt_walk2_out_%=:\n\t" \
        "s_waitcnt vmcnt(0) lgkmcnt(0)\n\t" \
        "v_mov_b32_e32 %[rec], v40\n\t" \
        "v_mov_b32_e32 %[offset], v42\n\t" \
        "v_mov_b32_e32 %[bb], v43\n\t" \
        "v_mov_b32_e32 %[wr], v44\n\t" \
        : [rec] "+v"(rec), [offset] "+v"(offset), [bb] "+v"(bb), [wr] "+v"(wr), [reason] "=&s"(reason) \
        : [desc2] "s"(desc2), [cblocks] "s"(cblocks), [ring] "v"(ring_base), [mail] "v"(mail_slot), [limit] "v"(limit), [quota] "v"(quota), [ringmask] "s"(ring_mask), [stride] "s"(4 * ring_stride), \
          "{s41}"(alphabet_offset) \
        : "memory", "vcc", "scc", "s44", "s45", "s46", "s47", GBWT_WALK2_PROBE_CLOBBERS \
          "v40", "v41", "v42", "v43", "v44", "v48", "v49", "v50", "v51", "v52", "v53", "v54", "v56", "v57", "v58", "v59", "v60", "v61", "v62", "v63", \
          "v64", "v65", "v66", "v67", "v70", "v71", "v72", "v73", "v74", "v75", "v76", "v77", "v78", "v79", "v80", "v81", "v82", "v83", "v84", "v85", "v86", \
          "v88", "v89", "v90", "v91", "v92", "v94", "v95", "v96", "v97", "v98", "v99", "v100", "v101", "v102", "v103", "v104", "v105", "v106", "v107", \
          "v108", "v109", "v110", "v111", "v112", "v113", "v114", "v115", "v116", "v117", "v118", "v119");
    const uint32_t limit = flushed + (ring_mask + 1 - 8);
    if (narrow) { GBWT_WALK2_LOOP(GBWT_WALK2_ISSUE_NARROW) } else { GBWT_WALK2_LOOP(GBWT_WALK2_ISSUE_WIDE) }
#undef GBWT_WALK2_LOOP
#undef GBWT_WALK2_ISSUE_NARROW
#undef GBWT_WALK2_ISSUE_WIDE
    return reason;
#endif
}

#ifndef GBWT_HIP_CXX_LOOP
#define GBWT_CHAIN_BLOCK(TAG, SKIP, FLAG_TEST, X, LREC, L, D, C, A) \
        SKIP \
        FLAG_TEST \
        "s_nop 1\n\t" \
        "s_and_saveexec_b64 s[80:81], vcc\n\t" \
        "s_cbranch_execz .Lgbwt_chain_done_" TAG "_%=\n\t" \
        "v_add_u32_e32 " L ", s41, " LREC "\n\t"              \
        "v_mov_b32_e32 " D ", -2\n\t" \
        "v_cmp_gt_u32_e32 vcc, " L ", " X "\n\t"              \
        "v_cndmask_b32_e64 " D ", " D ", 2, vcc\n\t"           \
        "v_add_u32_e32 " C ", " X ", " D "\n\t"                \
        ".Lgbwt_chain_next_" TAG "_%=:\n\t" \
        "v_cmp_ne_u32_e32 vcc, " C ", " L "\n\t" \
        "s_nop 1\n\t" \
        "s_and_b64 exec, exec, vcc\n\t" \
        "s_cbranch_execz .Lgbwt_chain_done_" TAG "_%=\n\t" \
        "v_and_b32_e32 " A ", %[ringmask], v44\n\t" \
        "v_mad_u32_u24 " A ", " A ", %[stride], %[ring]\n\t" \
        "ds_write_b32 " A ", " C "\n\t" \
        "v_add_u32_e32 v44, 1, v44\n\t" \
        "v_add_u32_e32 " C ", " C ", " D "\n\t" \
        "s_branch .Lgbwt_chain_next_" TAG "_%=\n\t" \
        ".Lgbwt_chain_done_" TAG "_%=:\n\t" \
        "s_mov_b64 exec, s[80:81]\n\t" \
        ".Lgbwt_chain_skip_" TAG "_%=:\n\t"
#endif

__device__ __forceinline__ uint32_t walk2_gather_loop(const uint4 *desc2, const uint4 *gblocks, uint32_t alphabet_offset, uint32_t ring_base,
                                                      uint32_t mail_slot, uint32_t flushed, bool narrow, uint32_t quota, uint32_t ring_mask, uint32_t ring_stride,
                                                      uint32_t &rec, uint32_t &offset, uint32_t &bb, uint32_t &wr, uint32_t headroom = 8, uint32_t drained_addr = 0, uint32_t patience = 0,
                                                      uint32_t lookahead = 0) {
#ifdef GBWT_HIP_CXX_LOOP
    __attribute__((address_space(3))) uint32_t *ring = (__attribute__((address_space(3))) uint32_t *)(uintptr_t)ring_base;
    __attribute__((address_space(3))) uint32_t *mail = (__attribute__((address_space(3))) uint32_t *)(uintptr_t)mail_slot;
    mail[0] = 0;
    for (;;) {
        bool slow = false;
        if (rec != 0) {
            const uint64_t idx = bb == BLOCK_NONE ? 0u : 2 * static_cast<uint64_t>(bb) + (offset >> 5);
            const uint4 K = gblocks[idx];
            const uint32_t bit = offset & 31u, below = (1u << bit) - 1;
            const uint32_t a = (K.x >> bit) & 1u, b = (K.y >> bit) & 1u;
            const uint4 *d = desc2 + 8 * static_cast<uint64_t>(rec);
            const uint4 E = d[a], leaf = d[2 + 2 * a + b];
            slow = (E.z & DESC2_SLOW) != 0 || !(E.w & GATHER_OK);
            if (!slow) {
                const uint32_t ones1 = K.z & 0x1FFFFFu, R0 = ((K.z >> 21) | (K.w << 11)) & 0x1FFFFFu, R1 = K.w >> 10;
                const uint32_t m = (a ? K.x : ~K.x) & below;
                const uint32_t p = __popc(m);
                const uint32_t rank_a = a ? ones1 + p : (offset - bit) - ones1 + p;
                const uint32_t j = E.y + rank_a;
                const uint32_t ones_w = (a ? R1 : R0) + __popc(m & K.y);
                rec = leaf.z & REC_MASK; offset = leaf.y + (b ? ones_w : j - ones_w); bb = leaf.w;
                ring[(wr & ring_mask) * ring_stride] = E.x;
                wr += E.x != 0 ? 1u : 0u;
                if (E.w & E_CHAIN) { const uint32_t L = (E.z & REC_MASK) + alphabet_offset, d = chain_stride(E.x, L); for (uint32_t n = E.x + d; n != L; n += d) ring[(wr++ & ring_mask) * ring_stride] = n; }
                ring[(wr & ring_mask) * ring_stride] = (E.z & REC_MASK) + alphabet_offset;
                wr += (E.z & LEAF_EMIT2) ? 1u : 0u;
                ring[(wr & ring_mask) * ring_stride] = leaf.x;
                wr += leaf.x != 0 ? 1u : 0u;
                if (leaf.z & LEAF_CHAIN) { const uint32_t L = rec + alphabet_offset, d = chain_stride(leaf.x, L); for (uint32_t n = leaf.x + d; n != L; n += d) ring[(wr++ & ring_mask) * ring_stride] = n; }
                ring[(wr & ring_mask) * ring_stride] = rec + alphabet_offset;
                wr += (leaf.z & LEAF_EMIT2) ? 1u : 0u;
                if (lookahead) { const uint4 T = d[6]; mail[0] = T.x; mail[1] = T.y; mail[2] = T.z; }
                mail[3] = wr;
                if (wr >= quota) { rec = 0; bb = BLOCK_NONE; }
            }
        }
        if (__ballot(slow) != 0) return 1;
        if (__ballot(rec != 0) == 0 || __ballot(wr - flushed > ring_mask + 1 - headroom) != 0) return 0;
    }
#else
    uint32_t reason;
    const uint32_t limit = flushed + (ring_mask + 1 - headroom);
#define GBWT_GATHER_K_NARROW                                                                              \
    "v_lshlrev_b32_e32 v70, 4, v58\n\t"                               \
    "v_lshlrev_b32_e32 v68, 7, v40\n\t"                           \
    "s_mov_b64 exec, s[44:45]\n\t"                                                                        \
    "global_load_dwordx4 v[60:63], v70, %[gblocks]\n\t"    \
    "s_mov_b64 exec, -1\n\t"
#define GBWT_GATHER_K_WIDE                                                                                \
    "v_lshlrev_b64 v[70:71], 4, v[58:59]\n\t"                                                             \
    "v_lshlrev_b64 v[68:69], 7, v[40:41]\n\t"                                                             \
    "v_lshl_add_u64 v[70:71], v[70:71], 0, %[gblocks]\n\t"                                                \
    "v_lshl_add_u64 v[68:69], v[68:69], 0, %[desc2]\n\t"                                                  \
    "s_mov_b64 exec, s[44:45]\n\t"                                                                        \
    "global_load_dwordx4 v[60:63], v[70:71], off\n\t"                                                     \
    "s_mov_b64 exec, -1\n\t"
#define GBWT_GATHER_D_NARROW                                                                              \
    "v_lshl_add_u32 v46, v72, 4, v68\n\t"                                                                 \
    "v_lshl_add_u32 v47, v72, 1, v84\n\t"                                                                 \
    "v_lshl_add_u32 v47, v47, 4, v68\n\t"                                                                 \
    "s_mov_b64 exec, s[44:45]\n\t"                                                                        \
    "global_load_dwordx4 v[48:51], v46, %[desc2]\n\t"                \
    "global_load_dwordx4 v[52:55], v47, %[desc2] offset:32\n\t"                          \
    "s_cmp_eq_u32 %[look], 0\n\t"                                                                         \
    "s_cbranch_scc1 .Lgbwt_gather_nolook_%=\n\t"                                                          \
    "global_load_dwordx3 v[64:66], v68, %[desc2] offset:96\n\t"      \
    ".Lgbwt_gather_nolook_%=:\n\t"                                                                         \
    "s_mov_b64 exec, -1\n\t"
#define GBWT_GATHER_D_WIDE                                                                                \
    "v_lshl_add_u32 v56, v72, 1, v84\n\t"                                                                 \
    "v_mov_b32_e32 v73, 0\n\t"                                                                            \
    "v_mov_b32_e32 v57, 0\n\t"                                                                            \
    "v_lshl_add_u64 v[46:47], v[72:73], 4, v[68:69]\n\t"                                                  \
    "v_lshl_add_u64 v[56:57], v[56:57], 4, v[68:69]\n\t"                                                  \
    "s_mov_b64 exec, s[44:45]\n\t"                                                                        \
    "global_load_dwordx4 v[48:51], v[46:47], off\n\t"                                                     \
    "global_load_dwordx4 v[52:55], v[56:57], off offset:32\n\t"                                           \
    "s_cmp_eq_u32 %[look], 0\n\t"                                                                         \
    "s_cbranch_scc1 .Lgbwt_gather_nolook_%=\n\t"                                                          \
    "global_load_dwordx3 v[64:66], v[68:69], off offset:96\n\t"                                           \
    ".Lgbwt_gather_nolook_%=:\n\t"                                                                         \
    "s_mov_b64 exec, -1\n\t"
#define GBWT_GATHER_LOOP(KLOAD, DLOAD) \
    asm volatile( \
        "v_mov_b32_e32 v40, %[rec]\n\t" \
        "v_mov_b32_e32 v41, 0\n\t" \
        "v_mov_b32_e32 v42, %[offset]\n\t" \
        "v_mov_b32_e32 v43, %[bb]\n\t" \
        "v_mov_b32_e32 v44, %[wr]\n\t" \
        "v_mov_b32_e32 v59, 0\n\t" \
        "s_mov_b32 %[reason], 0\n\t" \
        "v_readfirstlane_b32 s82, %[patience]\n\t" \
        "s_mov_b64 s[44:45], -1\n\t"                         \
        "v_cmp_ne_u32_e64 s[42:43], 0, v40\n\t" \
        "ds_write_b32 %[mail], v41\n\t"                      \
        ".Lgbwt_gather_loop_%=:\n\t" \
        "v_cmp_ne_u32_e32 vcc, -1, v43\n\t"                  \
        "v_lshrrev_b32_e32 v58, 5, v42\n\t" \
        "v_lshl_add_u32 v58, v43, 1, v58\n\t" \
        "v_cndmask_b32_e32 v58, 0, v58, vcc\n\t"             \
        KLOAD \
        "v_bfm_b32 v74, v42, 0\n\t"                          \
        "v_and_b32_e32 v77, 0xffffffe0, v42\n\t"             \
        "s_waitcnt vmcnt(0)\n\t" \
        "v_bfe_u32 v72, v60, v42, 1\n\t"                     \
        "v_bfe_u32 v84, v61, v42, 1\n\t"                     \
        DLOAD \
        "v_add_u32_e32 v76, -1, v72\n\t"                     \
        "v_cmp_eq_u32_e32 vcc, 1, v72\n\t"                   \
        "v_cmp_eq_u32_e64 s[46:47], 1, v84\n\t"              \
        "v_and_b32_e32 v79, 0x1fffff, v62\n\t"               \
        "v_bitop3_b32 v78, v60, v76, v74 bitop3:0x28\n\t"    \
        "v_alignbit_b32 v82, v63, v62, 21\n\t" \
        "v_sub_u32_e32 v77, v77, v79\n\t"                    \
        "v_cndmask_b32_e32 v77, v77, v79, vcc\n\t"           \
        "v_and_b32_e32 v82, 0x1fffff, v82\n\t"               \
        "v_lshrrev_b32_e32 v81, 10, v63\n\t"                 \
        "v_bcnt_u32_b32 v77, v78, v77\n\t"                   \
        "v_and_b32_e32 v78, v78, v61\n\t"                    \
        "v_cndmask_b32_e32 v82, v82, v81, vcc\n\t"           \
        "v_bcnt_u32_b32 v82, v78, v82\n\t"                   \
        "s_waitcnt vmcnt(0)\n\t" \
        "v_lshlrev_b32_e32 v67, 1, v50\n\t"                  \
        "v_add_u32_e32 v81, v49, v77\n\t"                    \
        "v_bfi_b32 v67, 1, v51, v67\n\t"                     \
        "v_sub_u32_e32 v83, v81, v82\n\t"                    \
        "v_and_b32_e32 v86, 0x3fffffff, v50\n\t"             \
        "v_xor_b32_e32 v67, 1, v67\n\t"                      \
        "v_and_b32_e32 v67, 0x80000001, v67\n\t" \
        "v_cmp_ne_u32_e32 vcc, 0, v67\n\t" \
        "v_cndmask_b32_e64 v83, v83, v82, s[46:47]\n\t"      \
        "s_nop 0\n\t" \
        "s_and_b64 vcc, vcc, s[42:43]\n\t"                   \
        "s_cbranch_vccnz .Lgbwt_gather_slow_%=\n\t" \
        "s_cmp_eq_u32 %[look], 0\n\t" \
        "s_cbranch_scc1 .Lgbwt_gather_nopost_%=\n\t" \
        "ds_write_b96 %[mail], v[64:66]\n\t"                \
        ".Lgbwt_gather_nopost_%=:\n\t" \
        "v_mov_b32_e32 v43, v55\n\t"                         \
        "v_add_u32_e32 v42, v53, v83\n\t"                    \
        "v_and_b32_e32 v40, 0x3fffffff, v54\n\t"             \
        "v_and_b32_e32 v67, %[ringmask], v44\n\t"            \
        "v_cmp_ne_u32_e32 vcc, 0, v48\n\t" \
        "v_mad_u32_u24 v67, v67, %[stride], %[ring]\n\t" \
        "ds_write_b32 v67, v48\n\t"                          \
        "v_addc_co_u32_e32 v44, vcc, 0, v44, vcc\n\t"        \
        GBWT_CHAIN_BLOCK("e", "", "v_and_b32_e32 v75, 2, v51\n\t" "v_cmp_ne_u32_e32 vcc, 0, v75\n\t", "v48", "v86", "v45", "v65", "v66", "v75") \
        "v_cmp_gt_i32_e32 vcc, 0, v50\n\t"                   \
        "v_and_b32_e32 v67, %[ringmask], v44\n\t" \
        "v_add_u32_e32 v86, s41, v86\n\t"                    \
        "v_mad_u32_u24 v67, v67, %[stride], %[ring]\n\t" \
        "ds_write_b32 v67, v86\n\t" \
        "v_addc_co_u32_e32 v44, vcc, 0, v44, vcc\n\t" \
        "v_cmp_ne_u32_e32 vcc, 0, v52\n\t" \
        "v_and_b32_e32 v67, %[ringmask], v44\n\t" \
        "v_add_u32_e32 v87, s41, v40\n\t"                    \
        "v_mad_u32_u24 v67, v67, %[stride], %[ring]\n\t" \
        "ds_write_b32 v67, v52\n\t"                          \
        "v_addc_co_u32_e32 v44, vcc, 0, v44, vcc\n\t" \
        GBWT_CHAIN_BLOCK("l", "", "v_and_b32_e32 v75, 0x40000000, v54\n\t" "v_cmp_ne_u32_e32 vcc, 0, v75\n\t", "v52", "v40", "v45", "v65", "v66", "v75") \
        "v_cmp_gt_i32_e32 vcc, 0, v54\n\t"                   \
        "v_and_b32_e32 v67, %[ringmask], v44\n\t" \
        "v_mad_u32_u24 v67, v67, %[stride], %[ring]\n\t" \
        "ds_write_b32 v67, v87\n\t" \
        "v_addc_co_u32_e32 v44, vcc, 0, v44, vcc\n\t" \
        "v_cmp_lt_u32_e32 vcc, v44, %[quota]\n\t"             \
        "s_mov_b64 s[44:45], s[42:43]\n\t"                   \
        "ds_write_b32 %[mail], v44 offset:12\n\t"            \
        "v_cndmask_b32_e32 v40, 0, v40, vcc\n\t" \
        "v_cndmask_b32_e32 v43, -1, v43, vcc\n\t" \
        "v_cmp_lt_u32_e32 vcc, %[limit], v44\n\t"            \
        "v_cmp_ne_u32_e64 s[42:43], 0, v40\n\t"              \
        "s_nop 1\n\t" \
        "s_cmp_eq_u64 s[42:43], 0\n\t" \
        "s_cbranch_scc1 .Lgbwt_gather_out_%=\n\t" \
        "s_cbranch_vccz .Lgbwt_gather_loop_%=\n\t" \
        ".Lgbwt_gather_full_%=:\n\t"                           \
        "ds_read_b32 v45, %[drained]\n\t"                     \
        "s_waitcnt lgkmcnt(0)\n\t" \
        "v_add_u32_e32 v45, %[room], v45\n\t" \
        "v_cmp_lt_u32_e32 vcc, v45, v44\n\t" \
        "s_nop 1\n\t" \
        "s_cbranch_vccnz .Lgbwt_gather_sleep_%=\n\t" \
        "s_sub_u32 s82, s82, 1\n\t"                          \
        "s_cbranch_scc1 .Lgbwt_gather_out_%=\n\t"               \
        "s_branch .Lgbwt_gather_loop_%=\n\t" \
        ".Lgbwt_gather_sleep_%=:\n\t" \
        "s_sleep 2\n\t" \
        "s_branch .Lgbwt_gather_full_%=\n\t" \
        ".Lgbwt_gather_slow_%=:\n\t" \
        "s_mov_b32 %[reason], 1\n\t" \
        ".Lgbwt_gather_out_%=:\n\t" \
        "s_waitcnt vmcnt(0) lgkmcnt(0)\n\t" \
        "v_mov_b32_e32 %[rec], v40\n\t" \
        "v_mov_b32_e32 %[offset], v42\n\t" \
        "v_mov_b32_e32 %[bb], v43\n\t" \
        "v_mov_b32_e32 %[wr], v44\n\t" \
        : [rec] "+v"(rec), [offset] "+v"(offset), [bb] "+v"(bb), [wr] "+v"(wr), [reason] "=&s"(reason) \
        : [desc2] "s"(desc2), [gblocks] "s"(gblocks), [ring] "v"(ring_base), [mail] "v"(mail_slot), [limit] "v"(limit), [quota] "v"(quota), [ringmask] "s"(ring_mask), [stride] "s"(4 * ring_stride), \
          [drained] "v"(drained_addr), [room] "s"(ring_mask + 1 - headroom), [patience] "v"(patience), [look] "s"(lookahead), \
          "{s41}"(alphabet_offset) \
        : "memory", "vcc", "scc", "s42", "s43", "s44", "s45", "s46", "s47", "s80", "s81", "s82", \
          "v40", "v41", "v42", "v43", "v44", "v45", "v46", "v47", "v48", "v49", "v50", "v51", "v52", "v53", "v54", "v55", "v56", "v57", "v58", "v59", \
          "v60", "v61", "v62", "v63", "v64", "v65", "v66", "v67", "v68", "v69", "v70", "v71", "v72", "v73", "v74", "v75", "v76", "v77", "v78", "v79", "v80", "v81", "v82", "v83", "v84", "v86", "v87");
    if (narrow) { GBWT_GATHER_LOOP(GBWT_GATHER_K_NARROW, GBWT_GATHER_D_NARROW) } else { GBWT_GATHER_LOOP(GBWT_GATHER_K_WIDE, GBWT_GATHER_D_WIDE) }
#undef GBWT_GATHER_LOOP
#undef GBWT_GATHER_K_NARROW
#undef GBWT_GATHER_K_WIDE
#undef GBWT_GATHER_D_NARROW
#undef GBWT_GATHER_D_WIDE
    return reason;
#endif
}

__device__ __forceinline__ uint32_t walk2_gather_loop_full(const uint4 *desc2, const uint4 *cblocks, uint32_t alphabet_offset, uint32_t ring_base,
                                                      uint32_t mail_slot, uint32_t flushed, bool narrow, uint32_t quota, uint32_t ring_mask, uint32_t ring_stride,
                                                      uint32_t &rec, uint32_t &offset, uint32_t &bb, uint32_t &wr, uint32_t headroom = 8, uint32_t drained_addr = 0, uint32_t patience = 0) {
#ifdef GBWT_HIP_CXX_LOOP
    __attribute__((address_space(3))) uint32_t *ring = (__attribute__((address_space(3))) uint32_t *)(uintptr_t)ring_base;
    __attribute__((address_space(3))) uint32_t *mail = (__attribute__((address_space(3))) uint32_t *)(uintptr_t)mail_slot;
    mail[0] = 0;
    for (;;) {
        bool slow = false;
        if (rec != 0) {
// ... 214 lines not shown
    GBWT_WALK2U_BYTES                                                                                     \
    "v_cmp_ne_u32_e32 vcc, s78, v40\n\t"                                     \
    "s_load_dwordx16 s[48:63], s[76:77], 0x0\n\t"                  \
    "s_load_dwordx8 s[64:71], s[76:77], 0x40\n\t"                           \
    "s_load_dwordx4 s[72:75], s[76:77], 0x60\n\t"                                  \
    KLOAD                                                                                                 \
    REFRESH
#define GBWT_WALK2U_LEAF(MASK, XY, ZW)                                                                     \
    MASK "\n\t"                                                                                           \
    "v_mov_b64 v[80:81], " XY "\n\t"                                      \
    "v_mov_b64 v[42:43], " ZW "\n\t"
#define GBWT_WALK2U_LEAVES_DONE                                                                           \
    "v_mov_b32_e32 v87, v42\n\t"                                             \
    "v_add_u32_e32 v42, v81, v75\n\t"
#define GBWT_WALK2U_STAGE(CHAIN_E, CHAIN_L) \
        "v_and_b32_e32 v47, %[ringmask], v44\n\t"            \
        "v_cmp_ne_u32_e32 vcc, 0, v72\n\t" \
        "v_mad_u32_u24 v47, v47, %[stride], %[ring]\n\t" \
        "ds_write_b32 v47, v72\n\t"                         \
        "v_addc_co_u32_e32 v44, vcc, 0, v44, vcc\n\t"        \
        CHAIN_E \
        "v_cmp_gt_i32_e32 vcc, 0, v73\n\t"                  \
        "v_and_b32_e32 v47, %[ringmask], v44\n\t" \
        "v_add_u32_e32 v78, s41, v78\n\t"                  \
        "v_mad_u32_u24 v47, v47, %[stride], %[ring]\n\t" \
        "ds_write_b32 v47, v78\n\t" \
        "v_addc_co_u32_e32 v44, vcc, 0, v44, vcc\n\t" \
        "v_cmp_ne_u32_e32 vcc, 0, v80\n\t" \
        "v_and_b32_e32 v47, %[ringmask], v44\n\t" \
        "v_add_u32_e32 v79, s41, v40\n\t"                   \
        "v_mad_u32_u24 v47, v47, %[stride], %[ring]\n\t" \
        "ds_write_b32 v47, v80\n\t"                         \
        "v_addc_co_u32_e32 v44, vcc, 0, v44, vcc\n\t" \
        CHAIN_L \
        "v_cmp_gt_i32_e32 vcc, 0, v87\n\t"                  \
        "v_and_b32_e32 v47, %[ringmask], v44\n\t" \
        "v_mad_u32_u24 v47, v47, %[stride], %[ring]\n\t" \
        "ds_write_b32 v47, v79\n\t" \
        "v_addc_co_u32_e32 v44, vcc, 0, v44, vcc\n\t"
#define GBWT_WALK2U_LOOP(KLOAD, REFRESH) \
    asm volatile( \
        "v_mov_b32_e32 v40, %[rec]\n\t" \
        "v_mov_b32_e32 v42, %[offset]\n\t" \
        "v_mov_b32_e32 v43, %[bb]\n\t" \
        "v_mov_b32_e32 v44, %[wr]\n\t" \
        "s_mov_b32 %[reason], 0\n\t" \
        GBWT_WALK2U_ISSUE(KLOAD, REFRESH) \
        "s_nop 1\n\t" \
        "s_cbranch_vccnz .Lgbwt_walk2u_mixed_%=\n\t" \
        "s_cmp_eq_u32 s78, 0\n\t" \
        "s_cbranch_scc1 .Lgbwt_walk2u_out_%=\n\t" \
        ".Lgbwt_walk2u_loop_%=:\n\t" \
        "s_waitcnt vmcnt(0) lgkmcnt(0)\n\t" \
        "s_bitcmp1_b32 s50, 30\n\t"                          \
        "s_cbranch_scc1 .Lgbwt_walk2u_slow_%=\n\t" \
        "s_and_b32 s82, s51, %[flagmask]\n\t"                \
        "s_mov_b32 s83, s51\n\t"                             \
        "s_mov_b32 s84, s55\n\t" \
        GBWT_WALK2U_FLAG_CHECK \
        GBWT_WALK2U_RANK_A \
        "v_mov_b32_e32 v72, s48\n\t"                        \
        "v_mov_b32_e32 v73, s50\n\t"                        \
        "v_add_u32_e32 v71, s49, v67\n\t"                   \
        "s_mov_b64 exec, s[44:45]\n\t"                       \
        "v_mov_b32_e32 v72, s52\n\t" \
        "v_mov_b32_e32 v73, s54\n\t" \
        "v_add_u32_e32 v71, s53, v67\n\t" \
        "s_mov_b64 exec, -1\n\t" \
        GBWT_WALK2U_RANK_B \
        "v_sub_u32_e32 v75, v71, v74\n\t"                 \
        "v_and_b32_e32 v78, 0x3fffffff, v73\n\t"           \
        "v_cndmask_b32_e64 v75, v75, v74, s[46:47]\n\t"   \
        GBWT_WALK2U_LEAF("s_nor_b64 exec, s[44:45], s[46:47]", "s[56:57]", "s[58:59]")      \
        GBWT_WALK2U_LEAF("s_andn2_b64 exec, s[46:47], s[44:45]", "s[60:61]", "s[62:63]")    \
        GBWT_WALK2U_LEAF("s_andn2_b64 exec, s[44:45], s[46:47]", "s[64:65]", "s[66:67]")    \
        GBWT_WALK2U_LEAF("s_and_b64 exec, s[44:45], s[46:47]", "s[68:69]", "s[70:71]")      \
        "s_mov_b64 exec, -1\n\t" \
        GBWT_WALK2U_LEAVES_DONE \
        "v_and_b32_e32 v40, 0x3fffffff, v87\n\t"            \
        "v_mov_b64 v[48:49], s[72:73]\n\t"                   \
        "v_mov_b32_e32 v50, s74\n\t" \
        GBWT_WALK2U_MAIL_FLAG \
        GBWT_WALK2U_ISSUE(KLOAD, "")                         \
        "s_nop 1\n\t" \
        "s_mov_b64 s[44:45], vcc\n\t"                        \
        "s_cmp_lg_u32 s82, 0\n\t"                           \
        "s_cbranch_scc1 .Lgbwt_walk2u_special_%=\n\t" \
        ".Lgbwt_walk2u_plain_%=:\n\t" \
        GBWT_WALK2U_STAGE("", "") \
        ".Lgbwt_walk2u_staged_%=:\n\t" \
        "v_cmp_lt_u32_e32 vcc, v44, %[quota]\n\t"            \
        "v_mov_b32_e32 v51, v44\n\t"                         \
        "ds_write_b128 %[mail], v[48:51]\n\t" \
        "v_cndmask_b32_e32 v40, 0, v40, vcc\n\t" \
        "v_cndmask_b32_e32 v43, -1, v43, vcc\n\t" \
        "s_andn2_b64 s[46:47], exec, vcc\n\t"                \
        "v_sub_u32_e32 v47, v44, v45\n\t"                    \
        "s_or_b64 s[44:45], s[44:45], s[46:47]\n\t" \
        REFRESH \
        "v_cmp_lt_u32_e64 s[46:47], %[slack], v47\n\t"       \
        "s_cmp_lg_u64 s[44:45], 0\n\t" \
        "s_cbranch_scc1 .Lgbwt_walk2u_mixed_%=\n\t" \
        "s_cmp_eq_u32 s78, 0\n\t" \
        "s_cbranch_scc1 .Lgbwt_walk2u_out_%=\n\t"            \
        "s_cmp_eq_u64 s[46:47], 0\n\t" \
        "s_cbranch_scc1 .Lgbwt_walk2u_loop_%=\n\t" \
        ".Lgbwt_walk2u_full_%=:\n\t"                         \
        "s_sleep 2\n\t"                                      \
        "ds_read_b32 v45, %[drained]\n\t" \
        "s_waitcnt lgkmcnt(0)\n\t" \
        "v_sub_u32_e32 v47, v44, v45\n\t" \
        "v_cmp_lt_u32_e64 s[46:47], %[slack], v47\n\t" \
        "s_nop 1\n\t" \
        "s_cmp_eq_u64 s[46:47], 0\n\t" \
        "s_cbranch_scc0 .Lgbwt_walk2u_full_%=\n\t" \
        "s_branch .Lgbwt_walk2u_loop_%=\n\t" \
        ".Lgbwt_walk2u_special_%=:\n\t" \
        "s_bitcmp1_b32 s82, 2\n\t"                           \
        "s_cbranch_scc1 .Lgbwt_walk2u_chained_%=\n\t" \
         \
        "v_and_b32_e32 v47, %[ringmask], v44\n\t" \
        "v_cmp_lt_u32_e64 s[46:47], %[wrapmax], v47\n\t"     \
        "s_nop 1\n\t" \
        "s_cmp_lg_u64 s[46:47], 0\n\t" \
        "s_cbranch_scc1 .Lgbwt_walk2u_plain_%=\n\t" \
        "v_mad_u32_u24 v47, v47, %[stride], %[ring]\n\t" \
        "v_add_u32_e32 v78, s41, v78\n\t"                  \
        "v_add_u32_e32 v79, s41, v40\n\t"                   \
        "ds_write_b32 v47, v72\n\t" \
        "ds_write_b32 v47, v78 offset:260\n\t"               \
        "ds_write_b32 v47, v80 offset:520\n\t" \
        "ds_write_b32 v47, v79 offset:780\n\t" \
        "v_add_u32_e32 v44, 4, v44\n\t" \
        "s_branch .Lgbwt_walk2u_staged_%=\n\t" \
        ".Lgbwt_walk2u_chained_%=:\n\t"                      \
        "v_mov_b32_e32 v82, s83\n\t" \
        "v_mov_b32_e32 v86, s84\n\t" \
        "v_cmp_eq_u32_e32 vcc, 1, v62\n\t" \
        "v_cndmask_b32_e32 v82, v82, v86, vcc\n\t"           \
        GBWT_WALK2U_STAGE(GBWT_CHAIN_BLOCK("e", "", "v_and_b32_e32 v86, 2, v82\n\t" "v_cmp_ne_u32_e32 vcc, 0, v86\n\t", "v72", "v78", "v83", "v84", "v85", "v86"), \
                          GBWT_CHAIN_BLOCK("l", "", "v_and_b32_e32 v86, 0x40000000, v87\n\t" "v_cmp_ne_u32_e32 vcc, 0, v86\n\t", "v80", "v40", "v83", "v84", "v85", "v86")) \
        "s_branch .Lgbwt_walk2u_staged_%=\n\t" \
        ".Lgbwt_walk2u_slow_%=:\n\t" \
        "s_mov_b32 %[reason], 1\n\t" \
        "s_branch .Lgbwt_walk2u_out_%=\n\t" \
        ".Lgbwt_walk2u_unpacked_%=:\n\t" \
        "s_mov_b32 %[reason], 3\n\t" \
        "s_branch .Lgbwt_walk2u_out_%=\n\t" \
        ".Lgbwt_walk2u_mixed_%=:\n\t" \
        "s_mov_b32 %[reason], 2\n\t" \
        ".Lgbwt_walk2u_out_%=:\n\t" \
        "s_waitcnt vmcnt(0) lgkmcnt(0)\n\t" \
        "v_mov_b32_e32 %[rec], v40\n\t" \
        "v_mov_b32_e32 %[offset], v42\n\t" \
        "v_mov_b32_e32 %[bb], v43\n\t" \
        "v_mov_b32_e32 %[wr], v44\n\t" \
        : [rec] "+v"(rec), [offset] "+v"(offset), [bb] "+v"(bb), [wr] "+v"(wr), [reason] "=&s"(reason) \
        : [dlo] "s"(dlo), [dhi] "s"(dhi), [cblocks] "s"(cblocks), [ring] "v"(ring_base), [mail] "v"(mail_slot), [drained] "v"(drained_addr), [slack] "s"(slack), [quota] "v"(quota), \
          [ringmask] "s"(ring_mask), [stride] "s"(4 * ring_stride), [flagmask] "s"(flagmask), [wrapmax] "s"(ring_mask - 3), "{s41}"(alphabet_offset) \
        : "memory", "vcc", "scc", "s44", "s45", "s46", "s47", "s48", "s49", "s50", "s51", "s52", "s53", "s54", "s55", "s56", "s57", "s58", "s59", \
          "s60", "s61", "s62", "s63", "s64", "s65", "s66", "s67", "s68", "s69", "s70", "s71", "s72", "s73", "s74", "s75", "s76", "s77", "s78", \
          "v40", "v42", "v43", "v44", "v45", "v46", "v61", "v48", "v49", "v50", "v51", "v52", "v53", "v54", "v55", "v56", "v57", "v58", "v60", "v47", "v62", "v63", \
          "v64", "v65", "v66", "v67", "v68", "v69", "v70", "v71", "v72", "v73", "v74", "v75", "v76", "v77", "v78", "v79", "v80", "v81", "v82", "v83", "v84", "v85", "v86", "v87", \
          "s80", "s81", "s82", "s83", "s84");
#define GBWT_WALK2U_BODY \
    uint32_t reason; \
    const uint32_t slack = ring_mask + 1 - headroom;    \
    const uint32_t flagmask = (ring_stride == 65u && all4) ? (E_ANYCHAIN | E_ALL4) : E_ANYCHAIN;    \
    const uint32_t dlo = static_cast<uint32_t>(reinterpret_cast<uintptr_t>(desc2)), dhi = static_cast<uint32_t>(reinterpret_cast<uintptr_t>(desc2) >> 32); \
     \
    if (narrow) { GBWT_WALK2U_LOOP(GBWT_WALK2U_KLOAD_NARROW, "ds_read_b32 v45, %[drained]\n\t") } \
    else { GBWT_WALK2U_LOOP(GBWT_WALK2U_KLOAD_WIDE, "ds_read_b32 v45, %[drained]\n\t") } \
    return reason;
#define GBWT_WALK2U_INDEX                                                                                 \
    "v_lshrrev_b32_e32 v46, 5, v42\n\t"                                                                   \
    "v_lshl_add_u32 v46, v43, 1, v46\n\t"
#define GBWT_WALK2U_BYTES "v_lshlrev_b32_e32 v60, 4, v46\n\t"
#define GBWT_WALK2U_RANK_A \
        "v_bfe_u32 v62, v52, v42, 1\n\t"                     \
        "v_bfm_b32 v64, v42, 0\n\t"                          \
        "v_and_b32_e32 v67, 0xffffffe0, v42\n\t"             \
        "v_and_b32_e32 v56, 0x1fffff, v54\n\t"               \
        "v_add_u32_e32 v66, -1, v62\n\t"                     \
        "v_cmp_eq_u32_e32 vcc, 1, v62\n\t"                   \
        "v_xor_b32_e32 v68, v52, v66\n\t"                    \
        "v_alignbit_b32 v57, v55, v54, 21\n\t" \
        "v_and_b32_e32 v68, v68, v64\n\t"                    \
        "v_sub_u32_e32 v67, v67, v56\n\t"                    \
        "v_bcnt_u32_b32 v70, v68, 0\n\t"                     \
        "v_cndmask_b32_e32 v67, v67, v56, vcc\n\t"           \
        "v_and_b32_e32 v57, 0x1fffff, v57\n\t"               \
        "v_lshrrev_b32_e32 v58, 10, v55\n\t"                 \
        "s_mov_b64 s[44:45], vcc\n\t"                        \
        "v_add_u32_e32 v67, v67, v70\n\t"                    \
        "v_cndmask_b32_e32 v74, v57, v58, vcc\n\t"           \
        "v_bfe_u32 v76, v53, v42, 1\n\t"
#define GBWT_WALK2U_RANK_B \
        "v_and_b32_e32 v68, v68, v53\n\t"                    \
        "v_cmp_eq_u32_e64 s[46:47], 1, v76\n\t"              \
        "v_bcnt_u32_b32 v74, v68, v74\n\t"
#define GBWT_WALK2U_KLOAD_NARROW                                                                          \
    "global_load_dwordx4 v[52:55], v60, %[cblocks]\n\t"
#define GBWT_WALK2U_KLOAD_WIDE                                                                            \
    "v_lshrrev_b32_e32 v61, 28, v46\n\t"                                                                  \
    "v_lshl_add_u64 v[60:61], v[60:61], 0, %[cblocks]\n\t"                                                \
    "global_load_dwordx4 v[52:55], v[60:61], off\n\t"
#define GBWT_WALK2U_FLAG_CHECK \
        "s_bitcmp0_b32 s51, 0\n\t"                           \
        "s_cbranch_scc1 .Lgbwt_walk2u_unpacked_%=\n\t"
#define GBWT_WALK2U_MAIL_FLAG
#endif
__device__ __forceinline__ uint32_t walk2_uniform_loop(const uint4 *desc2, const uint4 *cblocks , uint32_t alphabet_offset, uint32_t ring_base,
                                                       uint32_t mail_slot, uint32_t drained_addr, bool narrow, uint32_t quota, uint32_t ring_mask,
                                                       uint32_t ring_stride, uint32_t &rec, uint32_t &offset, uint32_t &bb, uint32_t &wr, uint32_t headroom = 8, bool all4 = true) {
#ifdef GBWT_HIP_CXX_LOOP
    return 2;
#else
    GBWT_WALK2U_BODY
#endif
}
#ifndef GBWT_HIP_CXX_LOOP
#undef GBWT_WALK2U_INDEX
#undef GBWT_WALK2U_BYTES
#undef GBWT_WALK2U_RANK_A
#undef GBWT_WALK2U_RANK_B
#undef GBWT_WALK2U_KLOAD_WIDE
#undef GBWT_WALK2U_KLOAD_NARROW
#undef GBWT_WALK2U_FLAG_CHECK
#undef GBWT_WALK2U_MAIL_FLAG
#define GBWT_WALK2U_INDEX                                                                                 \
    "v_lshrrev_b32_e32 v46, 6, v42\n\t"                                                                   \
    "v_add_u32_e32 v46, v46, v43\n\t"
#define GBWT_WALK2U_BYTES "v_lshlrev_b32_e32 v60, 5, v46\n\t"
#define GBWT_WALK2U_RANK_A \
        "v_lshrrev_b64 v[62:63], v42, v[52:53]\n\t"          \
        "v_lshlrev_b64 v[64:65], v42, -1\n\t"                \
        "v_and_b32_e32 v62, 1, v62\n\t"                      \
        "v_and_b32_e32 v67, 0xffffffc0, v42\n\t"             \
        "v_add_u32_e32 v66, -1, v62\n\t"                     \
        "v_cmp_eq_u32_e32 vcc, 1, v62\n\t"                   \
        "v_xor_b32_e32 v68, v52, v66\n\t"                   \
        "v_xor_b32_e32 v69, v53, v66\n\t" \
        "v_bfi_b32 v68, v64, 0, v68\n\t"                   \
        "v_bfi_b32 v69, v65, 0, v69\n\t" \
        "v_sub_u32_e32 v67, v67, v56\n\t"                    \
        "v_bcnt_u32_b32 v70, v68, 0\n\t" \
        "v_cndmask_b32_e32 v67, v67, v56, vcc\n\t"           \
        "v_bcnt_u32_b32 v70, v69, v70\n\t"                \
        "v_cndmask_b32_e32 v74, v57, v58, vcc\n\t"          \
        "s_mov_b64 s[44:45], vcc\n\t"                        \
        "v_add_u32_e32 v67, v67, v70\n\t"                   \
        "v_lshrrev_b64 v[76:77], v42, v[54:55]\n\t"
#define GBWT_WALK2U_RANK_B \
        "v_and_b32_e32 v68, v68, v54\n\t"                  \
        "v_and_b32_e32 v69, v69, v55\n\t" \
        "v_and_b32_e32 v76, 1, v76\n\t"                    \
        "v_bcnt_u32_b32 v74, v68, v74\n\t" \
        "v_cmp_eq_u32_e64 s[46:47], 1, v76\n\t"             \
        "v_bcnt_u32_b32 v74, v69, v74\n\t"
#define GBWT_WALK2U_KLOAD_NARROW                                                                          \
    "global_load_dwordx4 v[52:55], v60, %[cblocks]\n\t"                                                   \
    "global_load_dwordx3 v[56:58], v60, %[cblocks] offset:16\n\t"
#define GBWT_WALK2U_KLOAD_WIDE                                                                            \
    "v_lshrrev_b32_e32 v61, 27, v46\n\t"                                                                  \
    "v_lshl_add_u64 v[60:61], v[60:61], 0, %[cblocks]\n\t"                                                \
    "global_load_dwordx4 v[52:55], v[60:61], off\n\t"                                                     \
    "global_load_dwordx3 v[56:58], v[60:61], off offset:16\n\t"
#define GBWT_WALK2U_FLAG_CHECK
#define GBWT_WALK2U_MAIL_FLAG "v_or_b32_e32 v50, 0x80000000, v50\n\t"
#endif
__device__ __forceinline__ uint32_t walk2_uniform_loop_full(const uint4 *desc2, const uint4 *cblocks, uint32_t alphabet_offset, uint32_t ring_base,
                                                       uint32_t mail_slot, uint32_t drained_addr, bool narrow, uint32_t quota, uint32_t ring_mask,
                                                       uint32_t ring_stride, uint32_t &rec, uint32_t &offset, uint32_t &bb, uint32_t &wr, uint32_t headroom = 8, bool all4 = true) {
#ifdef GBWT_HIP_CXX_LOOP
    return 2;
#else
    GBWT_WALK2U_BODY
#endif
}
#ifndef GBWT_HIP_CXX_LOOP
#undef GBWT_WALK2U_BODY
#undef GBWT_WALK2U_LOOP
#undef GBWT_WALK2U_INDEX
#undef GBWT_WALK2U_BYTES
#undef GBWT_WALK2U_RANK_A
#undef GBWT_WALK2U_RANK_B
#undef GBWT_WALK2U_LEAF
#undef GBWT_WALK2U_STAGE
#undef GBWT_WALK2U_KLOAD_WIDE
#undef GBWT_WALK2U_KLOAD_NARROW
#undef GBWT_WALK2U_ISSUE
#undef GBWT_WALK2U_FLAG_CHECK
#undef GBWT_WALK2U_LEAVES_DONE
#undef GBWT_WALK2U_MAIL_FLAG
#endif

__device__ __forceinline__ void lookahead_helper2(const uint4 *desc2, const uint4 *cblocks, uint32_t mail_slot, uint32_t done_addr, uint32_t spread) {
    asm volatile(
        "v_mov_b32_e32 v40, 0\n\t"
        "v_mov_b32_e32 v47, 0\n\t"
        "v_mov_b32_e32 v59, 0\n\t"
        ".Lgbwt_helper2_loop_%=:\n\t"
        "ds_read_b128 v[48:51], %[mail]\n\t"
        "ds_read_b32 v52, %[done]\n\t"
        "s_waitcnt lgkmcnt(0)\n\t"
        "v_cmp_ne_u32_e32 vcc, v51, v40\n\t"
        "v_mov_b32_e32 v58, v48\n\t"
        "v_mov_b32_e32 v40, v51\n\t"
        "v_cmp_ne_u32_e64 s[46:47], 0, v48\n\t"
        "v_mov_b32_e32 v46, %[spread]\n\t"
        "v_mul_hi_u32 v46, v46, v50\n\t"
        "s_and_b64 vcc, vcc, s[46:47]\n\t"
        "v_add_u32_e32 v46, v46, v49\n\t"
        "s_and_saveexec_b64 s[44:45], vcc\n\t"
        "v_lshlrev_b64 v[54:55], 5, v[46:47]\n\t"
        "v_lshlrev_b64 v[60:61], 7, v[58:59]\n\t"
        "v_lshl_add_u64 v[54:55], v[54:55], 0, %[cblocks]\n\t"
        "v_lshl_add_u64 v[60:61], v[60:61], 0, %[desc2]\n\t"
        "global_load_dword v56, v[54:55], off\n\t"
        "global_load_dword v57, v[60:61], off\n\t"
        "global_load_dword v53, v[60:61], off offset:64\n\t"
        "s_mov_b64 exec, s[44:45]\n\t"
        "v_readfirstlane_b32 s46, v52\n\t"
        "s_cmp_lg_u32 s46, 0\n\t"
        "s_cbranch_scc1 .Lgbwt_helper2_out_%=\n\t"
        "s_sleep 8\n\t"
        "s_branch .Lgbwt_helper2_loop_%=\n\t"
        ".Lgbwt_helper2_out_%=:\n\t"
        "s_waitcnt vmcnt(0)\n\t"
        :
        : [mail] "v"(mail_slot), [done] "v"(done_addr), [spread] "v"(spread), [cblocks] "s"(cblocks), [desc2] "s"(desc2)
        : "memory", "vcc", "scc", "s44", "s45", "s46", "s47", "v40", "v46", "v47", "v48", "v49", "v50", "v51", "v52", "v53", "v54", "v55", "v56",
          "v57", "v58", "v59", "v60", "v61");
}


template <class Sink>
__device__ __forceinline__ void push_chain(Sink &sink, uint32_t x, uint32_t L) {
    const uint32_t d = chain_stride(x, L);
    for (uint32_t n = x + d; n != L; n += d) sink.push(n, true);
}

template <class Sink>
__device__ __forceinline__ void two_step(const DeviceIndex &ix, Sink &sink, uint32_t &rec, uint32_t &offset, uint32_t &bb) {
    const uint4 *d = ix.desc2 + 8 * static_cast<uint64_t>(rec);
    const uint4 E0 = d[0];
    if (E0.z & DESC2_SLOW) { generic_step(ix, sink, rec, offset, bb); return; }
    const uint64_t idx = bb == BLOCK_NONE ? 0u : bb + (offset >> RANK_BLOCK_SHIFT);
    const uint4 K0 = ix.cblocks[2 * idx], K1 = ix.cblocks[2 * idx + 1];
    const uint64_t bits1 = (static_cast<uint64_t>(K0.y) << 32) | K0.x, bits2 = (static_cast<uint64_t>(K0.w) << 32) | K0.z;
    const uint32_t bit = offset & 63u;
    const uint64_t below = (uint64_t(1) << bit) - 1;
    const uint32_t a = static_cast<uint32_t>(bits1 >> bit) & 1u;
    const uint64_t m = a ? bits1 : ~bits1;
    const uint32_t rank_a = a ? K1.x + __popcll(m & below) : (offset - bit) - K1.x + __popcll(m & below);
    const uint4 E = a ? d[1] : E0;
    const uint32_t j = E.y + rank_a;
    const uint32_t b = static_cast<uint32_t>(bits2 >> bit) & 1u;
    const uint32_t ones_w = (a ? K1.z : K1.y) + __popcll(m & bits2 & below);
    const uint4 leaf = d[2 + 2 * a + b];
    const uint32_t n1 = E.x, wword = E.z;
    rec = leaf.z & REC_MASK; offset = leaf.y + (b ? ones_w : j - ones_w); bb = leaf.w;
    sink.push(n1, n1 != 0);
    if (E.w & E_CHAIN) push_chain(sink, n1, (wword & REC_MASK) + ix.alphabet_offset);
    sink.push((wword & REC_MASK) + ix.alphabet_offset, (wword & LEAF_EMIT2) != 0);
    sink.push(leaf.x, leaf.x != 0);
    if (leaf.z & LEAF_CHAIN) push_chain(sink, leaf.x, rec + ix.alphabet_offset);
    sink.push(rec + ix.alphabet_offset, (leaf.z & LEAF_EMIT2) != 0);
}

template <class Sink>
__device__ __forceinline__ void quiet_walk(const DeviceIndex &ix, uint64_t id, Sink &sink, uint32_t *overflow) {
    uint32_t rec = 0, offset = 0, bb = BLOCK_NONE;
    if (id < ix.n_endmarker) {
        const uint2 e = ix.endmarker[id];
        if (e.x != 0) {
            sink.push(e.x, true);
// ... 22 lines not shown
```

### include/gbwt_hip.h

```cpp
#ifndef GBWT_HIP_H
#define GBWT_HIP_H

#include <stddef.h>
#include <stdint.h>

#ifdef __cplusplus
extern "C" {
#endif

typedef enum {
    GBWT_HIP_OK = 0,
    GBWT_HIP_INVALID_DATA = 1,
    GBWT_HIP_IO_ERROR = 2,
    GBWT_HIP_BAD_ARGUMENT = 3,
    GBWT_HIP_NO_DEVICE = 4,
    GBWT_HIP_DEVICE_ERROR = 5,
    GBWT_HIP_CAPACITY = 6,
    GBWT_HIP_UNSUPPORTED = 7
} gbwt_hip_status;

typedef struct { uint64_t node, offset; } gbwt_hip_pos;
typedef struct { uint64_t node, start, end; } gbwt_hip_state;
typedef struct { gbwt_hip_state forward, reverse; } gbwt_hip_bd_state;

typedef struct {
    uint64_t size;
    uint64_t sequences;
    uint64_t alphabet_size;
    uint64_t alphabet_offset;
    uint64_t records;
    uint64_t data_bytes;
    uint64_t paths;
    uint32_t bidirectional;
    uint32_t has_metadata;
    uint32_t is_gbz;
    uint32_t has_translation;
    uint64_t max_record_len;
    uint64_t max_outdegree;
} gbwt_hip_stats;

typedef struct gbwt_hip_index gbwt_hip_index;
typedef struct gbwt_hip_workspace gbwt_hip_workspace;

const char *gbwt_hip_last_error(void);
int gbwt_hip_device_count(void);

gbwt_hip_status gbwt_hip_open_file(const char *path, int device, gbwt_hip_index **out);

gbwt_hip_status gbwt_hip_parse_file(const char *path, gbwt_hip_stats *out);

gbwt_hip_status gbwt_hip_open_records(const uint8_t *data, uint64_t data_len, const uint64_t *starts,
                                      uint64_t n_records, uint64_t alphabet_offset, uint64_t alphabet_size,
                                      uint64_t n_sequences, uint64_t size, int bidirectional, int device,
                                      gbwt_hip_index **out);
enum { GBWT_HIP_OPEN_EXTRACT = 1, GBWT_HIP_OPEN_SEARCH = 2, GBWT_HIP_OPEN_GFA = 4, GBWT_HIP_OPEN_ALL = 7 };
gbwt_hip_status gbwt_hip_open_file_flags(const char *path, int device, uint32_t flags, gbwt_hip_index **out);
gbwt_hip_status gbwt_hip_open_records_flags(const uint8_t *data, uint64_t data_len, const uint64_t *starts,
                                            uint64_t n_records, uint64_t alphabet_offset, uint64_t alphabet_size,
                                            uint64_t n_sequences, uint64_t size, int bidirectional, int device, uint32_t flags,
                                            gbwt_hip_index **out);
void gbwt_hip_close(gbwt_hip_index *index);
gbwt_hip_status gbwt_hip_get_stats(const gbwt_hip_index *index, gbwt_hip_stats *out);

typedef struct {
    uint64_t index_device_bytes, index_host_bytes;
    uint64_t workspace_device_bytes, rows_bytes, text_bytes;
    uint64_t rows_chunks;
} gbwt_hip_memory;
gbwt_hip_status gbwt_hip_memory_usage(const gbwt_hip_index *index, const gbwt_hip_workspace *ws, gbwt_hip_memory *out);

typedef struct {
    double parse_ms, upload_ms, sample_ms, total_ms;
    uint64_t samples, checkpoint_walkers, checkpoint_orphans;
    uint32_t checkpoint_sampling, checkpoint_rounds;
    double line_sizes_ms;
} gbwt_hip_open_times;
gbwt_hip_status gbwt_hip_get_open_times(const gbwt_hip_index *index, gbwt_hip_open_times *out);

gbwt_hip_status gbwt_hip_workspace_create(const gbwt_hip_index *index, gbwt_hip_workspace **out);
void gbwt_hip_workspace_destroy(gbwt_hip_workspace *ws);
gbwt_hip_status gbwt_hip_workspace_tune(gbwt_hip_workspace *ws, uint32_t walk_mode, uint32_t paths_per_wave, uint32_t small_record);
void *gbwt_hip_workspace_stream(gbwt_hip_workspace *ws);

gbwt_hip_status gbwt_hip_extract(const gbwt_hip_index *index, gbwt_hip_workspace *ws, const uint64_t *seq_ids,
                                 uint64_t n, uint64_t *out_offsets, uint32_t *out_nodes, uint64_t capacity,
                                 uint64_t *total);

typedef struct { const uint64_t *d_offsets; const uint32_t *d_nodes; uint64_t total; uint64_t n; } gbwt_hip_paths;
gbwt_hip_status gbwt_hip_extract_device(const gbwt_hip_index *index, gbwt_hip_workspace *ws,
                                        const uint64_t *seq_ids, uint64_t n, gbwt_hip_paths *out);

gbwt_hip_status gbwt_hip_extract_part_device(const gbwt_hip_index *index, gbwt_hip_workspace *ws, const uint64_t *seq_ids, uint64_t n,
                                             uint32_t part, uint32_t parts, gbwt_hip_paths *out);

gbwt_hip_status gbwt_hip_copy_result(const gbwt_hip_index *index, gbwt_hip_workspace *ws, uint64_t *out_offsets,
                                     uint32_t *out_nodes, uint64_t capacity);

gbwt_hip_status gbwt_hip_extract_paths(const gbwt_hip_index *index, gbwt_hip_workspace *ws, const uint64_t *path_ids,
                                       uint64_t n, int reverse, uint64_t *out_offsets, uint32_t *out_nodes,
                                       uint64_t capacity, uint64_t *total);

gbwt_hip_status gbwt_hip_start(const gbwt_hip_index *index, gbwt_hip_workspace *ws, const uint64_t *seq_ids, uint64_t n,
                               gbwt_hip_pos *out, uint8_t *valid);
gbwt_hip_status gbwt_hip_forward(const gbwt_hip_index *index, gbwt_hip_workspace *ws, const gbwt_hip_pos *in, uint64_t n,
                                 gbwt_hip_pos *out, uint8_t *valid);
gbwt_hip_status gbwt_hip_backward(const gbwt_hip_index *index, gbwt_hip_workspace *ws, const gbwt_hip_pos *in, uint64_t n,
                                  gbwt_hip_pos *out, uint8_t *valid);

gbwt_hip_status gbwt_hip_find(const gbwt_hip_index *index, gbwt_hip_workspace *ws, const uint64_t *nodes, uint64_t n,
                              gbwt_hip_state *out, uint8_t *valid);
gbwt_hip_status gbwt_hip_extend(const gbwt_hip_index *index, gbwt_hip_workspace *ws, const gbwt_hip_state *states,
                                const uint64_t *nodes, uint64_t n, gbwt_hip_state *out, uint8_t *valid);
gbwt_hip_status gbwt_hip_bd_find(const gbwt_hip_index *index, gbwt_hip_workspace *ws, const uint64_t *nodes, uint64_t n,
                                 gbwt_hip_bd_state *out, uint8_t *valid);
gbwt_hip_status gbwt_hip_extend_forward(const gbwt_hip_index *index, gbwt_hip_workspace *ws,
                                        const gbwt_hip_bd_state *states, const uint64_t *nodes, uint64_t n,
                                        gbwt_hip_bd_state *out, uint8_t *valid);
gbwt_hip_status gbwt_hip_extend_backward(const gbwt_hip_index *index, gbwt_hip_workspace *ws,
                                         const gbwt_hip_bd_state *states, const uint64_t *nodes, uint64_t n,
                                         gbwt_hip_bd_state *out, uint8_t *valid);
gbwt_hip_status gbwt_hip_follow(const gbwt_hip_index *index, gbwt_hip_workspace *ws, const gbwt_hip_bd_state *states, uint64_t n,
                                int backward, uint64_t *out_offsets, gbwt_hip_bd_state *out_states, uint64_t capacity,
                                uint64_t *total, uint8_t *valid);
gbwt_hip_status gbwt_hip_search(const gbwt_hip_index *index, gbwt_hip_workspace *ws, const uint64_t *queries,
                                uint64_t n, uint64_t len, gbwt_hip_state *out, uint8_t *valid);

gbwt_hip_status gbwt_hip_bd_search(const gbwt_hip_index *index, gbwt_hip_workspace *ws, const uint64_t *queries,
                                   uint64_t n, uint64_t len, uint64_t first, gbwt_hip_bd_state *out, uint8_t *valid);

typedef struct { const gbwt_hip_state *d_states; const uint8_t *d_valid; uint64_t n; } gbwt_hip_states;
typedef struct { const gbwt_hip_bd_state *d_states; const uint8_t *d_valid; uint64_t n; } gbwt_hip_bd_states;
gbwt_hip_status gbwt_hip_search_device(const gbwt_hip_index *index, gbwt_hip_workspace *ws, const uint64_t *d_queries, uint64_t n, uint64_t len,
                                       gbwt_hip_states *out);
gbwt_hip_status gbwt_hip_bd_search_device(const gbwt_hip_index *index, gbwt_hip_workspace *ws, const uint64_t *d_queries, uint64_t n, uint64_t len,
                                          uint64_t first, gbwt_hip_bd_states *out);

gbwt_hip_status gbwt_hip_path_lines(const gbwt_hip_index *index, gbwt_hip_workspace *ws, const uint64_t *path_ids, uint64_t n,
                                    int mode, char *out, uint64_t capacity, uint64_t *total);
typedef struct { const char *d_text; const uint64_t *d_line_offsets; uint64_t total; uint64_t n; } gbwt_hip_lines;
gbwt_hip_status gbwt_hip_path_lines_device(const gbwt_hip_index *index, gbwt_hip_workspace *ws, const uint64_t *path_ids,
                                           uint64_t n, int mode, gbwt_hip_lines *out);
gbwt_hip_status gbwt_hip_segment_paths(const gbwt_hip_index *index, gbwt_hip_workspace *ws, const uint64_t *seq_ids, uint64_t n, uint64_t *out_offsets,
                                       uint64_t *out_tokens, uint64_t capacity, uint64_t *total);
gbwt_hip_status gbwt_hip_write_gfa(const gbwt_hip_index *index, gbwt_hip_workspace *ws, const char *path);
enum { GBWT_HIP_PATHS_DEFAULT = 0, GBWT_HIP_PATHS_PAN_SN = 1, GBWT_HIP_PATHS_REF_ONLY = 2 };
gbwt_hip_status gbwt_hip_write_gfa_mode(const gbwt_hip_index *index, gbwt_hip_workspace *ws, const char *path, int path_mode);

gbwt_hip_status gbwt_hip_path_sequences_device(const gbwt_hip_index *index, gbwt_hip_workspace *ws, const uint64_t *path_ids, uint64_t n, int reverse,
                                               int endmarker, gbwt_hip_lines *out);
gbwt_hip_status gbwt_hip_path_sequences(const gbwt_hip_index *index, gbwt_hip_workspace *ws, const uint64_t *path_ids, uint64_t n, int reverse, int endmarker,
                                        char *out, uint64_t *out_offsets, uint64_t capacity, uint64_t *total);
gbwt_hip_status gbwt_hip_node_sequence(const gbwt_hip_index *index, uint64_t node_id, char *out, uint64_t capacity, uint64_t *len, uint8_t *found);
gbwt_hip_status gbwt_hip_write_sequences(const gbwt_hip_index *index, gbwt_hip_workspace *ws, const char *path, const uint64_t *path_ids, uint64_t n, int endmarker);
gbwt_hip_status gbwt_hip_last_sequences_ms(const gbwt_hip_workspace *ws, float *walk_ms, float *sizes_ms, float *bases_ms);

gbwt_hip_status gbwt_hip_tags_device(const gbwt_hip_index *index, gbwt_hip_workspace *ws, const uint64_t *path_ids, uint64_t n, const uint64_t *d_sa, uint64_t count,
                                     uint64_t *d_tags, uint64_t *runs);
gbwt_hip_status gbwt_hip_tags(const gbwt_hip_index *index, gbwt_hip_workspace *ws, const uint64_t *path_ids, uint64_t n, const uint64_t *sa, uint64_t count,
// ... 221 lines not shown
```

Baseline: 768.7 billion LF-steps/s.

## Add compact 16-bit landing-offset encoding for gathered two-step blocks

Adds a compact encoding for packed two-step blocks when the record and its neighbors have at most 0xFFFF positions. Each block half then stores four 16-bit precomputed landing bases, one per (a,b) class, in place of the 21-bit ones/rank counts. The walk kernel gets a fast path that computes the landing offset with one bitfield extract plus popcount. A uniform-landing flag (E_ONE) also skips per-lane leaf selection when all four leaves point to the same record. This shortens the dependent arithmetic chain per LF step, at the cost of more branching in hand-written assembly and extra build-time checks.

```diff
diff --git a/gbwt_rs_amd/_lib.py b/gbwt_rs_amd/_lib.py
--- a/gbwt_rs_amd/_lib.py
+++ b/gbwt_rs_amd/_lib.py
@@ -35,7 +35,7 @@
 class OpenTimes(C.Structure):
     _fields_ = [("parse_ms", C.c_double), ("upload_ms", C.c_double), ("sample_ms", C.c_double), ("total_ms", C.c_double),
                 ("samples", C.c_uint64), ("checkpoint_walkers", C.c_uint64), ("checkpoint_orphans", C.c_uint64), ("checkpoint_sampling", C.c_uint32),
-                ("checkpoint_rounds", C.c_uint32), ("line_sizes_ms", C.c_double)]
+                ("checkpoint_rounds", C.c_uint32), ("line_sizes_ms", C.c_double), ("compact_records", C.c_uint64)]
 
 
 class Memory(C.Structure):
diff --git a/gbwt_rs_amd/csrc/capi_open.hip b/gbwt_rs_amd/csrc/capi_open.hip
--- a/gbwt_rs_amd/csrc/capi_open.hip
+++ b/gbwt_rs_amd/csrc/capi_open.hip
@@ -286,7 +286,7 @@
     trace.mark("link + lookahead + allocations");
     const uint32_t chain_max = k.chains.value_or(CHAIN_MAX);
     HIP_CHECK(hipMemsetAsync(d_stats + 6, 0, sizeof(uint64_t), nullptr));
-    launch_link_desc2(d, ix.desc2.as<uint4>(), gather_limit, chain_max | (h.bidirectional ? 0x100u : 0u), reinterpret_cast<uint32_t *>(d_stats + 5), nullptr);
+    launch_link_desc2(d, ix.desc2.as<uint4>(), gather_limit, k.compact_limit, chain_max | (h.bidirectional ? 0x100u : 0u), reinterpret_cast<uint32_t *>(d_stats + 5), nullptr);
     ix.gblocks.reserve((gather_limit ? n_blocks : 1) * 2 * sizeof(uint4));
     HIP_CHECK(hipMemsetAsync(ix.gblocks.ptr, 0, 2 * sizeof(uint4), nullptr));
     d.gblocks = ix.gblocks.as<uint4>();
@@ -295,7 +295,7 @@
     d.chained = static_cast<uint32_t>(early_stats[5] & 0xFFFFFFFFu);
     if (d.chained != 0 && !k.chains && (early_stats[5] >> 32) * 1000 < n_records) {
         HIP_CHECK(hipMemset(d_stats + 5, 0, 2 * sizeof(uint64_t)));
-        launch_link_desc2(d, ix.desc2.as<uint4>(), gather_limit, h.bidirectional ? 0x100u : 0u, reinterpret_cast<uint32_t *>(d_stats + 5), nullptr);
+        launch_link_desc2(d, ix.desc2.as<uint4>(), gather_limit, k.compact_limit, h.bidirectional ? 0x100u : 0u, reinterpret_cast<uint32_t *>(d_stats + 5), nullptr);
         d.chained = 0;
     }
     if (trace.on) std::fprintf(stderr, "[open] records with a chained step: %llu of %llu (up to %u nodes per iteration)\n",
@@ -363,7 +363,7 @@
 void record_stats_and_endmarker(gbwt_hip_index &ix, const uint64_t (&hs)[8], const Endmarker *early_endmarker) {
     ix.stats.max_record_len = hs[0];
     ix.stats.max_outdegree = hs[1];
-    if (ix.caps & GBWT_HIP_OPEN_EXTRACT) ix.slow_records = hs[6] & 0xFFFFFFFFull;
+    if (ix.caps & GBWT_HIP_OPEN_EXTRACT) { ix.slow_records = hs[6] & 0xFFFFFFFFull; ix.times.compact_records = hs[6] >> 32; }
     if (hs[2] != 0) throw InvalidData("BWT: record without a readable outdegree");
     if (hs[0] >= (uint64_t(1) << 32)) throw Unsupported("a record with 2^32 or more positions is not supported (u32 offsets on device)");
     DeviceIndex &d = ix.dev;
diff --git a/gbwt_rs_amd/csrc/device_index.hpp b/gbwt_rs_amd/csrc/device_index.hpp
--- a/gbwt_rs_amd/csrc/device_index.hpp
+++ b/gbwt_rs_amd/csrc/device_index.hpp
@@ -16,6 +16,8 @@
 constexpr uint32_t E_CHAIN = 2u;
 constexpr uint32_t E_ALL4 = 8u;
 constexpr uint32_t E_ANYCHAIN = 4u;
+constexpr uint32_t E_F16 = 16u;
+constexpr uint32_t E_ONE = 32u;
 constexpr uint32_t LEAF_CHAIN = 1u << 30;
 constexpr uint32_t CHAIN_MAX = 6;
 constexpr uint32_t WT_TABLE = 1u << 30;
diff --git a/gbwt_rs_amd/csrc/half_block_codec.hpp b/gbwt_rs_amd/csrc/half_block_codec.hpp
--- /dev/null
+++ b/gbwt_rs_amd/csrc/half_block_codec.hpp
@@ -0,0 +1,59 @@
+#pragma once
+
+#include <cstdint>
+
+#if defined(__HIPCC__)
+#define GBWT_HB_HD __host__ __device__
+#else
+#define GBWT_HB_HD
+#endif
+
+namespace gbwt_hip {
+
+constexpr uint32_t COMPACT_MAX = 0xFFFFu;
+
+struct HalfWords { uint32_t z, w; };
+struct HalfCounts { uint32_t ones1, R0, R1; };
+
+GBWT_HB_HD inline uint32_t hb_popc(uint32_t x) { return static_cast<uint32_t>(__builtin_popcount(x)); }
+
+GBWT_HB_HD inline HalfWords legacy_pack(uint32_t ones1, uint32_t R0, uint32_t R1) {
+    return HalfWords{(ones1 & 0x1FFFFFu) | (R0 << 21), ((R0 >> 11) & 0x3FFu) | (R1 << 10)};
+}
+GBWT_HB_HD inline HalfCounts legacy_unpack(uint32_t z, uint32_t w) {
+    return HalfCounts{z & 0x1FFFFFu, ((z >> 21) | (w << 11)) & 0x1FFFFFu, w >> 10};
+}
+GBWT_HB_HD inline uint32_t legacy_landing_offset(uint32_t bits1, uint32_t bits2, const HalfCounts &c, uint32_t a, uint32_t b, uint32_t bit,
+                                                 uint32_t half_start, uint32_t edge_base, uint32_t leaf_base) {
+    const uint32_t m = (a ? bits1 : ~bits1) & ((1u << bit) - 1u);
+    const uint32_t p = hb_popc(m);
+    const uint32_t rank_a = a ? c.ones1 + p : half_start - c.ones1 + p;
+    const uint32_t j = edge_base + rank_a;
+    const uint32_t ones_w = (a ? c.R1 : c.R0) + hb_popc(m & bits2);
+    return leaf_base + (b ? ones_w : j - ones_w);
+}
+GBWT_HB_HD inline uint32_t first_step_offset(uint32_t bits1, const HalfCounts &c, uint32_t a, uint32_t bit, uint32_t half_start, uint32_t edge_base) {
+    const uint32_t p = hb_popc((a ? bits1 : ~bits1) & ((1u << bit) - 1u));
+    return edge_base + (a ? c.ones1 + p : half_start - c.ones1 + p);
+}
+
+struct CompactBases { uint32_t edge[2]; uint32_t leaf[4]; };
+GBWT_HB_HD inline HalfWords compact_pack(const CompactBases &s, const uint32_t n[2], const uint32_t R[2]) {
+    uint32_t F[4];
+    for (uint32_t a = 0; a < 2; a++) {
+        F[2 * a + 1] = (s.leaf[2 * a + 1] + R[a]) & 0xFFFFu;
+        F[2 * a] = (s.leaf[2 * a] + s.edge[a] + n[a] - R[a]) & 0xFFFFu;
+    }
+    return HalfWords{F[0] | (F[1] << 16), F[2] | (F[3] << 16)};
+}
+GBWT_HB_HD inline uint32_t compact_field(uint32_t z, uint32_t w, uint32_t a, uint32_t b) { return ((a ? w : z) >> (16u * b)) & 0xFFFFu; }
+GBWT_HB_HD inline uint32_t class_mask(uint32_t bits1, uint32_t bits2, uint32_t a, uint32_t b) { return (a ? bits1 : ~bits1) & (b ? bits2 : ~bits2); }
+GBWT_HB_HD inline uint32_t landing_offset(uint32_t bits1, uint32_t bits2, uint32_t z, uint32_t w, uint32_t a, uint32_t b, uint32_t bit) {
+    return compact_field(z, w, a, b) + hb_popc(class_mask(bits1, bits2, a, b) & ((1u << bit) - 1u));
+}
+GBWT_HB_HD inline HalfCounts legacy_counts(uint32_t z, uint32_t w, const uint32_t G[4], uint32_t leaf01_base, uint32_t leaf11_base) {
+    const uint32_t F01 = z >> 16, F10 = w & 0xFFFFu, F11 = w >> 16;
+    return HalfCounts{((F10 - G[2]) & 0xFFFFu) + ((F11 - G[3]) & 0xFFFFu), (F01 - leaf01_base) & 0xFFFFu, (F11 - leaf11_base) & 0xFFFFu};
+}
+
+}
diff --git a/gbwt_rs_amd/csrc/kernels.hpp b/gbwt_rs_amd/csrc/kernels.hpp
--- a/gbwt_rs_amd/csrc/kernels.hpp
+++ b/gbwt_rs_amd/csrc/kernels.hpp
@@ -25,7 +25,7 @@
                         uint2 *d_edges, hipStream_t stream);
 void launch_fill_wtables(const DeviceIndex &ix, uint4 *d_wtables, hipStream_t stream);
 void launch_fill_wtables_deep(const DeviceIndex &ix, uint4 *d_deep, bool compact, hipStream_t stream);
-void launch_link_desc2(const DeviceIndex &ix, uint4 *d_desc2, uint32_t gather_limit, uint32_t chain_max, uint32_t *d_chained, hipStream_t stream);
+void launch_link_desc2(const DeviceIndex &ix, uint4 *d_desc2, uint32_t gather_limit, uint32_t compact_limit, uint32_t chain_max, uint32_t *d_chained, hipStream_t stream);
 void launch_fill_two_step_blocks(const DeviceIndex &ix, uint4 *d_cblocks , uint4 *d_gblocks , hipStream_t stream);
 void launch_link_lookahead2(const DeviceIndex &ix, uint4 *d_desc2, const uint32_t *d_block_counts, uint32_t hops, hipStream_t stream);
 void launch_fill_blocks(const DeviceIndex &ix, const uint32_t *d_block_counts, const uint32_t *d_block_base, uint4 *d_blocks, hipStream_t stream);
diff --git a/gbwt_rs_amd/csrc/knobs.hpp b/gbwt_rs_amd/csrc/knobs.hpp
--- a/gbwt_rs_amd/csrc/knobs.hpp
+++ b/gbwt_rs_amd/csrc/knobs.hpp
@@ -19,6 +19,7 @@
     std::optional<uint32_t> checkpoint_cap;
     std::optional<uint32_t> chains;
     uint32_t gather_limit = 1u << 21;
+    uint32_t compact_limit = 0xFFFFu;
     uint32_t lookahead_hops = 15;
     bool walk_tables = true, deep_tables = true, compact_tables = true;
     std::optional<uint64_t> table_bytes;
@@ -39,6 +40,7 @@
         if (const char *v = std::getenv("GBWT_HIP_CHECKPOINT_CAP")) k.checkpoint_cap = static_cast<uint32_t>(std::max(1, std::atoi(v)));
         if (const char *v = std::getenv("GBWT_HIP_CHAINS")) k.chains = static_cast<uint32_t>(std::min<long>(gbwt_hip::CHAIN_MAX, std::max<long>(0, std::atol(v))));
         if (const char *v = std::getenv("GBWT_HIP_GATHER_LIMIT")) k.gather_limit = static_cast<uint32_t>(std::min<long>(1l << 21, std::max<long>(0, std::atol(v))));
+        if (const char *v = std::getenv("GBWT_HIP_COMPACT_LIMIT")) k.compact_limit = static_cast<uint32_t>(std::min<long>(0xFFFFl, std::max<long>(0, std::atol(v))));
         if (const char *v = std::getenv("GBWT_HIP_LOOKAHEAD_HOPS")) k.lookahead_hops = static_cast<uint32_t>(std::max(0, std::atoi(v)));
         k.walk_tables = on("GBWT_HIP_WALK_TABLES"); k.deep_tables = on("GBWT_HIP_DEEP_TABLES"); k.compact_tables = on("GBWT_HIP_COMPACT_TABLES");
         if (const char *v = std::getenv("GBWT_HIP_TABLE_BYTES")) k.table_bytes = std::strtoull(v, nullptr, 10);
diff --git a/gbwt_rs_amd/csrc/load_kernels.hip b/gbwt_rs_amd/csrc/load_kernels.hip
--- a/gbwt_rs_amd/csrc/load_kernels.hip
+++ b/gbwt_rs_amd/csrc/load_kernels.hip
@@ -3,6 +3,7 @@
 #include <hipcub/hipcub.hpp>
 
 #include "device_common.hpp"
+#include "half_block_codec.hpp"
 #include "lf_device.hpp"
 
 namespace gbwt_hip {
@@ -362,7 +363,7 @@
     return cls == 1 && e == 0 ? B.w : 0u;
 }
 
-__global__ void __launch_bounds__(256) k_link_desc2(DeviceIndex ix, uint4 *out, uint32_t gather_limit, uint32_t chain_max, uint32_t *chained) {
+__global__ void __launch_bounds__(256) k_link_desc2(DeviceIndex ix, uint4 *out, uint32_t gather_limit, uint32_t compact_limit, uint32_t chain_max, uint32_t *chained) {
     uint64_t v = blockIdx.x * static_cast<uint64_t>(blockDim.x) + threadIdx.x;
     if (v >= ix.n_records) return;
     const uint4 *d1 = ix.desc;
@@ -417,9 +418,25 @@
         for (uint32_t b = 0; b < cls_w && all4; b++) all4 = leaf[2 * a + b].x != 0 && (leaf[2 * a + b].z & LEAF_EMIT2) != 0;
     }
     if (slow && VB.y != 0 && chained != nullptr) atomicAdd(chained + 2, 1u);
+    bool compact = packed && !slow && cls_v == 2 && compact_limit != 0 && VB.w <= compact_limit;
+    for (uint32_t a = 0; a < 2 && compact; a++) {
+        const uint64_t w = wword[a] & REC_MASK;
+        if (w == 0) { compact = false; break; }
+        const uint4 WB = ix.desc_raw[4 * w + 1];
+        compact = !(d1[4 * w + 2].x & DESC_SLOW) && WB.y != 0 && desc_class(WB.z) == 2 && WB.w <= compact_limit;
+        for (uint32_t b = 0; b < 2 && compact; b++) {
+            const uint64_t land = leaf[2 * a + b].z & REC_MASK;
+            if (land != 0) compact = ix.desc_raw[4 * land + 1].w <= compact_limit;
+        }
+    }
+    const bool one = leaf[0].z == leaf[1].z && leaf[0].z == leaf[2].z && leaf[0].z == leaf[3].z && leaf[0].w == leaf[1].w && leaf[0].w == leaf[2].w && leaf[0].w == leaf[3].w;
+    {
+        const uint64_t lanes = __ballot(compact && chained != nullptr);
+        if (lanes != 0 && (threadIdx.x % WAVE) == static_cast<uint32_t>(__ffsll(static_cast<unsigned long long>(lanes)) - 1)) atomicAdd(chained + 3, static_cast<uint32_t>(__popcll(lanes)));
+    }
     uint4 *o = out + 8 * v;
-    o[0] = make_uint4(n1[0], base[0], wword[0] | (slow ? DESC2_SLOW : 0u), (packed ? GATHER_OK : 0u) | chain[0] | (any_chain ? E_ANYCHAIN : 0u) | (all4 ? E_ALL4 : 0u));
-    o[1] = make_uint4(n1[1], base[1], wword[1] | (slow ? DESC2_SLOW : 0u), (packed ? GATHER_OK : 0u) | chain[1]);
+    o[0] = make_uint4(n1[0], base[0], wword[0] | (slow ? DESC2_SLOW : 0u), (packed ? GATHER_OK : 0u) | chain[0] | (any_chain ? E_ANYCHAIN : 0u) | (all4 ? E_ALL4 : 0u) | (compact ? E_F16 : 0u) | (one ? E_ONE : 0u));
+    o[1] = make_uint4(n1[1], base[1], wword[1] | (slow ? DESC2_SLOW : 0u), (packed ? GATHER_OK : 0u) | chain[1] | (compact ? E_F16 : 0u));
     if (any_chain && chained != nullptr) {
         uint32_t most = 0;
         for (uint32_t a = 0; a < 2; a++) {
@@ -475,6 +492,8 @@
     const uint32_t bb = ix.block_base[v];
     const uint32_t k = static_cast<uint32_t>(b - bb);
     SecondStep s2{{nullptr, nullptr}, {0, 0}};
+    uint32_t wlen[2] = {0, 0}, wones[2] = {0, 0};
+    const bool compact = gblocks != nullptr && (ix.desc2[8 * v].w & E_F16) != 0;
     if (!(D.x & DESC_SLOW)) {
         for (uint32_t a = 0; a < 2; a++) {
             const uint4 E = ix.desc2[8 * v + a];
@@ -484,6 +503,7 @@
             if ((d1[4 * w + 2].x & DESC_SLOW) || WB.y == 0 || desc_class(WB.z) != 2) continue;
             s2.wblocks[a] = ix.blocks + ix.block_base[w];
             s2.wbase[a] = E.y;
+            wlen[a] = WB.w; wones[a] = WB.w - ix.desc_raw[4 * w + 2].x;
         }
     }
     {
@@ -505,6 +525,33 @@
         }
         if (gblocks == nullptr) return;
         const uint32_t lo2 = static_cast<uint32_t>(bits2), hi2 = static_cast<uint32_t>(bits2 >> 32);
+        if (compact) {
+            const uint4 *d2 = ix.desc2 + 8 * v;
+            CompactBases s;
+            for (uint32_t a = 0; a < 2; a++) s.edge[a] = d2[a].y;
+            for (uint32_t q = 0; q < 4; q++) s.leaf[q] = d2[2 + q].y;
+            uint32_t nlo[2], nhi[2], Rlo[2], Rhi[2];
+            for (uint32_t a = 0; a < 2; a++) {
+                const uint32_t mlo = static_cast<uint32_t>((a ? bits1 : ~bits1) & valid);
+                nlo[a] = a ? P.z : (k << RANK_BLOCK_SHIFT) - P.z;
+                nhi[a] = nlo[a] + __popc(mlo);
+                if (m_of[a] != 0) Rlo[a] = R[a];
+                else {
+                    const uint32_t j = s.edge[a] + nlo[a];
+                    if (j >= wlen[a]) Rlo[a] = wones[a];
+                    else {
+                        const uint4 W = s2.wblocks[a][j >> RANK_BLOCK_SHIFT];
+                        Rlo[a] = W.z + __popcll(((static_cast<uint64_t>(W.y) << 32) | W.x) & ((uint64_t(1) << (j & 63u)) - 1));
+                    }
+                }
+                Rhi[a] = Rlo[a] + __popc(lo2 & mlo);
+            }
+            const HalfWords lo = compact_pack(s, nlo, Rlo), hi = compact_pack(s, nhi, Rhi);
+            gblocks[2 * static_cast<uint64_t>(bb + k)] = make_uint4(P.x, lo2, lo.z, lo.w);
+            gblocks[2 * static_cast<uint64_t>(bb + k) + 1] = make_uint4(P.y, hi2, hi.z, hi.w);
+            if (k == 0) const_cast<uint4 *>(ix.desc2)[8 * v + 7] = make_uint4(lo.z & 0xFFFFu, lo.z >> 16, lo.w & 0xFFFFu, lo.w >> 16);
+            return;
+        }
         uint32_t Rlo[2], Rhi[2];
         for (uint32_t a = 0; a < 2; a++) {
             const uint32_t mlo = static_cast<uint32_t>(m_of[a]), mhi = static_cast<uint32_t>(m_of[a] >> 32);
@@ -600,9 +647,9 @@
     hipLaunchKernelGGL(k_fill_wtables_deep, dim3(static_cast<unsigned>(ix.n_records)), dim3(256), 0, stream, ix, d_deep, compact ? 1u : 0u);
 }
 
-void launch_link_desc2(const DeviceIndex &ix, uint4 *d_desc2, uint32_t gather_limit, uint32_t chain_max, uint32_t *d_chained, hipStream_t stream) {
+void launch_link_desc2(const DeviceIndex &ix, uint4 *d_desc2, uint32_t gather_limit, uint32_t compact_limit, uint32_t chain_max, uint32_t *d_chained, hipStream_t stream) {
     if (ix.n_records == 0) return;
-    hipLaunchKernelGGL(k_link_desc2, dim3(grid_for(ix.n_records, 256)), dim3(256), 0, stream, ix, d_desc2, gather_limit, chain_max, d_chained);
+    hipLaunchKernelGGL(k_link_desc2, dim3(grid_for(ix.n_records, 256)), dim3(256), 0, stream, ix, d_desc2, gather_limit, compact_limit, chain_max, d_chained);
 }
 
 void launch_fill_two_step_blocks(const DeviceIndex &ix, uint4 *d_cblocks, uint4 *d_gblocks, hipStream_t stream) {
diff --git a/gbwt_rs_amd/csrc/open_walks.hip b/gbwt_rs_amd/csrc/open_walks.hip
--- a/gbwt_rs_amd/csrc/open_walks.hip
+++ b/gbwt_rs_amd/csrc/open_walks.hip
@@ -166,8 +166,10 @@
 
 __device__ __forceinline__ bool counting_step(const DeviceIndex &ix, bool packed, uint32_t threshold, NodeCounter &sink, uint32_t &rec, uint32_t &offset, uint32_t &bb) {
     const uint4 *d = ix.desc2 + 8 * static_cast<uint64_t>(rec);
-    uint32_t a, b, rank_a, ones_w_base, mw;
+    uint32_t a, b, rank_a = 0, ones_w_base = 0, mw = 0;
     uint4 E;
+    uint4 Kc = make_uint4(0u, 0u, 0u, 0u);
+    bool compact = false;
     if (packed) {
         const uint64_t idx = bb == BLOCK_NONE ? 0u : 2 * static_cast<uint64_t>(bb) + (offset >> 5);
         const uint4 K = ix.gblocks[idx];
@@ -175,12 +177,13 @@
         a = (K.x >> bit) & 1u; b = (K.y >> bit) & 1u;
         E = d[a];
         if ((E.z & DESC2_SLOW) || !(E.w & GATHER_OK)) { packed = false; }
+        else if (E.w & E_F16) { compact = true; Kc = K; }
         else {
-            const uint32_t ones1 = K.z & 0x1FFFFFu, R0 = ((K.z >> 21) | (K.w << 11)) & 0x1FFFFFu, R1 = K.w >> 10;
+            const HalfCounts c = legacy_unpack(K.z, K.w);
             const uint32_t m = (a ? K.x : ~K.x) & below;
             const uint32_t p = __popc(m);
-            rank_a = a ? ones1 + p : (offset - bit) - ones1 + p;
-            ones_w_base = a ? R1 : R0; mw = __popc(m & K.y);
+            rank_a = a ? c.ones1 + p : (offset - bit) - c.ones1 + p;
+            ones_w_base = a ? c.R1 : c.R0; mw = __popc(m & K.y);
         }
     }
     if (!packed) {
@@ -197,12 +200,21 @@
         E = a ? d[1] : E0;
         ones_w_base = a ? K1.z : K1.y; mw = __popcll(m & bits2);
     }
-    const uint32_t j = E.y + rank_a, w = E.z & REC_MASK;
+    const uint32_t w = E.z & REC_MASK;
     sink.wr += (E.x != 0 ? 1u : 0u) + ((E.z & LEAF_EMIT2) ? 1u : 0u) + ((E.w & E_CHAIN) ? chain_mids(E.x, w + ix.alphabet_offset) : 0u);
-    if (hashed_checkpoint(w, threshold)) { rec = w; offset = j; bb = BLOCK_NONE; return true; }
+    if (hashed_checkpoint(w, threshold)) {
+        if (compact) {
+            const uint4 G = d[7];
+            const uint32_t g[4] = {G.x, G.y, G.z, G.w}, bit = offset & 31u;
+            offset = first_step_offset(Kc.x, legacy_counts(Kc.z, Kc.w, g, d[3].y, d[5].y), a, bit, offset - bit, E.y);
+        } else offset = E.y + rank_a;
+        rec = w; bb = BLOCK_NONE;
+        return true;
+    }
     const uint4 leaf = d[2 + 2 * a + b];
-    const uint32_t ones_w = ones_w_base + mw;
-    rec = leaf.z & REC_MASK; offset = leaf.y + (b ? ones_w : j - ones_w); bb = leaf.w;
+    if (compact) offset = landing_offset(Kc.x, Kc.y, Kc.z, Kc.w, a, b, offset & 31u);
+    else { const uint32_t j = E.y + rank_a, ones_w = ones_w_base + mw; offset = leaf.y + (b ? ones_w : j - ones_w); }
+    rec = leaf.z & REC_MASK; bb = leaf.w;
     sink.wr += (leaf.x != 0 ? 1u : 0u) + ((leaf.z & LEAF_EMIT2) ? 1u : 0u) + ((leaf.z & LEAF_CHAIN) ? chain_mids(leaf.x, rec + ix.alphabet_offset) : 0u);
     return false;
 }
@@ -395,18 +407,15 @@
     if (packed) {
         const uint64_t idx = bb == BLOCK_NONE ? 0u : 2 * static_cast<uint64_t>(bb) + (offset >> 5);
         const uint4 K = ix.gblocks[idx];
-        const uint32_t bit = offset & 31u, below = (1u << bit) - 1;
+        const uint32_t bit = offset & 31u;
         const uint32_t a = (K.x >> bit) & 1u, b = (K.y >> bit) & 1u;
         const uint4 E = d[a];
         if (!(E.z & DESC2_SLOW) && (E.w & GATHER_OK)) {
-            const uint32_t ones1 = K.z & 0x1FFFFFu, R0 = ((K.z >> 21) | (K.w << 11)) & 0x1FFFFFu, R1 = K.w >> 10;
-            const uint32_t m = (a ? K.x : ~K.x) & below;
-            const uint32_t p = __popc(m);
-            const uint32_t rank_a = a ? ones1 + p : (offset - bit) - ones1 + p;
-            const uint32_t ones_w = (a ? R1 : R0) + __popc(m & K.y);
-            const uint32_t j = E.y + rank_a, w = E.z & REC_MASK;
+            const uint32_t w = E.z & REC_MASK;
             const uint4 leaf = d[2 + 2 * a + b];
-            rec = leaf.z & REC_MASK; offset = leaf.y + (b ? ones_w : j - ones_w); bb = leaf.w;
+            offset = (E.w & E_F16) ? landing_offset(K.x, K.y, K.z, K.w, a, b, bit)
+                                   : legacy_landing_offset(K.x, K.y, legacy_unpack(K.z, K.w), a, b, bit, offset - bit, E.y, leaf.y);
+            rec = leaf.z & REC_MASK; bb = leaf.w;
             sink.push(E.x, E.x != 0);
             if (E.w & E_CHAIN) push_chain(sink, E.x, w + ix.alphabet_offset);
             sink.push(w + ix.alphabet_offset, (E.z & LEAF_EMIT2) != 0);
diff --git a/gbwt_rs_amd/csrc/walk_direct.hip b/gbwt_rs_amd/csrc/walk_direct.hip
--- a/gbwt_rs_amd/csrc/walk_direct.hip
+++ b/gbwt_rs_amd/csrc/walk_direct.hip
@@ -447,10 +447,12 @@
                     if (!slow_here) {
                         const uint32_t bit = offset & 31u;
                         const uint32_t value = (K.x >> bit) & 1u;
-                        const uint32_t ones = (K.z & 0x1FFFFFu) + static_cast<uint32_t>(__popc(K.x & ((1u << bit) - 1u)));
+                        HalfCounts counts;
+                        if (E0.w & E_F16) { const uint4 G = d2[7]; const uint32_t g[4] = {G.x, G.y, G.z, G.w}; counts = legacy_counts(K.z, K.w, g, d2[3].y, d2[5].y); }
+                        else counts = legacy_unpack(K.z, K.w);
                         const uint4 E = value ? E1 : E0;
                         const uint32_t land = E.z & REC_MASK;
-                        rec = land; offset = E.y + (value ? ones : offset - ones);
+                        rec = land; offset = first_step_offset(K.x, counts, value, bit, offset - bit, E.y);
                         bb = land != 0 ? ix.block_base[land] : BLOCK_NONE;
                         sink.push(E.x, E.x != 0);
                         sink.push(rec + ix.alphabet_offset, (E.z & LEAF_EMIT2) != 0);
diff --git a/gbwt_rs_amd/csrc/walk_loops.hpp b/gbwt_rs_amd/csrc/walk_loops.hpp
--- a/gbwt_rs_amd/csrc/walk_loops.hpp
+++ b/gbwt_rs_amd/csrc/walk_loops.hpp
@@ -4,6 +4,7 @@
 
 #include "coop_device.hpp"
 #include "device_common.hpp"
+#include "half_block_codec.hpp"
 #include "kernels.hpp"
 #include "lf_device.hpp"
 
@@ -547,19 +548,15 @@
         if (rec != 0) {
             const uint64_t idx = bb == BLOCK_NONE ? 0u : 2 * static_cast<uint64_t>(bb) + (offset >> 5);
             const uint4 K = gblocks[idx];
-            const uint32_t bit = offset & 31u, below = (1u << bit) - 1;
+            const uint32_t bit = offset & 31u;
             const uint32_t a = (K.x >> bit) & 1u, b = (K.y >> bit) & 1u;
             const uint4 *d = desc2 + 8 * static_cast<uint64_t>(rec);
             const uint4 E = d[a], leaf = d[2 + 2 * a + b];
             slow = (E.z & DESC2_SLOW) != 0 || !(E.w & GATHER_OK);
             if (!slow) {
-                const uint32_t ones1 = K.z & 0x1FFFFFu, R0 = ((K.z >> 21) | (K.w << 11)) & 0x1FFFFFu, R1 = K.w >> 10;
-                const uint32_t m = (a ? K.x : ~K.x) & below;
-                const uint32_t p = __popc(m);
-                const uint32_t rank_a = a ? ones1 + p : (offset - bit) - ones1 + p;
-                const uint32_t j = E.y + rank_a;
-                const uint32_t ones_w = (a ? R1 : R0) + __popc(m & K.y);
-                rec = leaf.z & REC_MASK; offset = leaf.y + (b ? ones_w : j - ones_w); bb = leaf.w;
+                offset = (E.w & E_F16) ? landing_offset(K.x, K.y, K.z, K.w, a, b, bit)
+                                       : legacy_landing_offset(K.x, K.y, legacy_unpack(K.z, K.w), a, b, bit, offset - bit, E.y, leaf.y);
+                rec = leaf.z & REC_MASK; bb = leaf.w;
                 ring[(wr & ring_mask) * ring_stride] = E.x;
                 wr += E.x != 0 ? 1u : 0u;
                 if (E.w & E_CHAIN) { const uint32_t L = (E.z & REC_MASK) + alphabet_offset, d = chain_stride(E.x, L); for (uint32_t n = E.x + d; n != L; n += d) ring[(wr++ & ring_mask) * ring_stride] = n; }
@@ -651,6 +648,13 @@
         "v_cmp_eq_u32_e64 s[46:47], 1, v84\n\t"              \
         "v_and_b32_e32 v79, 0x1fffff, v62\n\t"               \
         "v_bitop3_b32 v78, v60, v76, v74 bitop3:0x28\n\t"    \
+        "v_add_u32_e32 v80, -1, v84\n\t"                     \
+        "v_cndmask_b32_e32 v45, v62, v63, vcc\n\t"           \
+        "v_lshlrev_b32_e32 v75, 4, v84\n\t"                  \
+        "v_xor_b32_e32 v80, v61, v80\n\t"                    \
+        "v_bfe_u32 v45, v45, v75, 16\n\t"                    \
+        "v_and_b32_e32 v80, v78, v80\n\t"                    \
+        "v_bcnt_u32_b32 v45, v80, v45\n\t"                   \
         "v_alignbit_b32 v82, v63, v62, 21\n\t" \
         "v_sub_u32_e32 v77, v77, v79\n\t"                    \
         "v_cndmask_b32_e32 v77, v77, v79, vcc\n\t"           \
@@ -677,9 +681,12 @@
         "s_cbranch_scc1 .Lgbwt_gather_nopost_%=\n\t" \
         "ds_write_b96 %[mail], v[64:66]\n\t"                \
         ".Lgbwt_gather_nopost_%=:\n\t" \
+        "v_and_b32_e32 v75, 16, v51\n\t"                     \
         "v_mov_b32_e32 v43, v55\n\t"                         \
+        "v_cmp_ne_u32_e64 s[80:81], 0, v75\n\t" \
         "v_add_u32_e32 v42, v53, v83\n\t"                    \
         "v_and_b32_e32 v40, 0x3fffffff, v54\n\t"             \
+        "v_cndmask_b32_e64 v42, v42, v45, s[80:81]\n\t"      \
         "v_and_b32_e32 v67, %[ringmask], v44\n\t"            \
         "v_cmp_ne_u32_e32 vcc, 0, v48\n\t" \
         "v_mad_u32_u24 v67, v67, %[stride], %[ring]\n\t" \
@@ -1060,6 +1067,7 @@
         "v_mov_b32_e32 v50, s74\n\t" \
         GBWT_WALK2U_MAIL_FLAG \
         GBWT_WALK2U_ISSUE(KLOAD, "")                         \
+        ".Lgbwt_walk2u_issued_%=:\n\t" \
         "s_nop 1\n\t" \
         "s_mov_b64 s[44:45], vcc\n\t"                        \
         "s_cmp_lg_u32 s82, 0\n\t"                           \
@@ -1119,6 +1127,7 @@
         GBWT_WALK2U_STAGE(GBWT_CHAIN_BLOCK("e", "", "v_and_b32_e32 v86, 2, v82\n\t" "v_cmp_ne_u32_e32 vcc, 0, v86\n\t", "v72", "v78", "v83", "v84", "v85", "v86"), \
                           GBWT_CHAIN_BLOCK("l", "", "v_and_b32_e32 v86, 0x40000000, v87\n\t" "v_cmp_ne_u32_e32 vcc, 0, v86\n\t", "v80", "v40", "v83", "v84", "v85", "v86")) \
         "s_branch .Lgbwt_walk2u_staged_%=\n\t" \
+        GBWT_WALK2U_COMPACT_PATH(KLOAD) \
         ".Lgbwt_walk2u_slow_%=:\n\t" \
         "s_mov_b32 %[reason], 1\n\t" \
         "s_branch .Lgbwt_walk2u_out_%=\n\t" \
@@ -1185,8 +1194,72 @@
     "global_load_dwordx4 v[52:55], v[60:61], off\n\t"
 #define GBWT_WALK2U_FLAG_CHECK \
         "s_bitcmp0_b32 s51, 0\n\t"                           \
-        "s_cbranch_scc1 .Lgbwt_walk2u_unpacked_%=\n\t"
+        "s_cbranch_scc1 .Lgbwt_walk2u_unpacked_%=\n\t" \
+        "s_bitcmp1_b32 s51, 4\n\t"                           \
+        "s_cbranch_scc1 .Lgbwt_walk2u_compact_%=\n\t"
 #define GBWT_WALK2U_MAIL_FLAG
+#define GBWT_WALK2U_COMPACT_PATH(KLOAD) \
+        ".Lgbwt_walk2u_compact_%=:\n\t" \
+        "v_bfe_u32 v62, v52, v42, 1\n\t"                     \
+        "v_bfe_u32 v76, v53, v42, 1\n\t"                     \
+        "v_bfm_b32 v64, v42, 0\n\t"                          \
+        "v_add_u32_e32 v66, -1, v62\n\t"                     \
+        "v_add_u32_e32 v67, -1, v76\n\t"                     \
+        "v_cmp_eq_u32_e32 vcc, 1, v62\n\t"                   \
+        "v_cmp_eq_u32_e64 s[46:47], 1, v76\n\t"              \
+        "v_bitop3_b32 v68, v52, v66, v64 bitop3:0x28\n\t"    \
+        "v_xor_b32_e32 v69, v53, v67\n\t"                    \
+        "v_lshlrev_b32_e32 v70, 4, v76\n\t"                  \
+        "v_cndmask_b32_e32 v71, v54, v55, vcc\n\t"           \
+        "s_mov_b64 s[44:45], vcc\n\t"                        \
+        "v_and_b32_e32 v68, v68, v69\n\t"                    \
+        "v_bfe_u32 v71, v71, v70, 16\n\t"                    \
+        "s_bitcmp1_b32 s51, 5\n\t"                           \
+        "s_cbranch_scc0 .Lgbwt_walk2u_compact_four_%=\n\t" \
+        "v_mov_b32_e32 v87, s58\n\t"                         \
+        "v_mov_b32_e32 v43, s59\n\t"                         \
+        ".Lgbwt_walk2u_compact_landed_%=:\n\t" \
+        "v_bcnt_u32_b32 v42, v68, v71\n\t"                   \
+        "v_and_b32_e32 v40, 0x3fffffff, v87\n\t"             \
+        "v_cmp_ne_u32_e32 vcc, -1, v43\n\t"                  \
+        GBWT_WALK2U_INDEX \
+        "v_readfirstlane_b32 s78, v40\n\t"                   \
+        "v_cndmask_b32_e32 v46, 0, v46, vcc\n\t"             \
+        GBWT_WALK2U_BYTES \
+        KLOAD                                                \
+        "v_mov_b32_e32 v72, s48\n\t"                         \
+        "v_mov_b32_e32 v73, s50\n\t"                         \
+        "v_mov_b32_e32 v80, s56\n\t"                         \
+        "v_mov_b32_e32 v81, s60\n\t"                         \
+        "s_mov_b64 exec, s[44:45]\n\t"                       \
+        "v_mov_b32_e32 v72, s52\n\t" \
+        "v_mov_b32_e32 v73, s54\n\t" \
+        "v_mov_b32_e32 v80, s64\n\t"                         \
+        "v_mov_b32_e32 v81, s68\n\t"                         \
+        "s_mov_b64 exec, -1\n\t" \
+        "v_mov_b64 v[48:49], s[72:73]\n\t"                   \
+        "v_mov_b32_e32 v50, s74\n\t" \
+        "v_cndmask_b32_e64 v80, v80, v81, s[46:47]\n\t"      \
+        "v_and_b32_e32 v78, 0x3fffffff, v73\n\t"             \
+        "s_lshl_b32 s76, s78, 7\n\t"                         \
+        "s_lshr_b32 s77, s78, 25\n\t" \
+        "s_add_u32 s76, s76, %[dlo]\n\t" \
+        "s_addc_u32 s77, s77, %[dhi]\n\t" \
+        "v_cmp_ne_u32_e32 vcc, s78, v40\n\t"                 \
+        "s_load_dwordx16 s[48:63], s[76:77], 0x0\n\t" \
+        "s_load_dwordx8 s[64:71], s[76:77], 0x40\n\t" \
+        "s_load_dwordx4 s[72:75], s[76:77], 0x60\n\t" \
+        "s_branch .Lgbwt_walk2u_issued_%=\n\t" \
+        ".Lgbwt_walk2u_compact_four_%=:\n\t"                 \
+        "v_mov_b64 v[42:43], s[58:59]\n\t"                   \
+        "v_mov_b64 v[74:75], s[62:63]\n\t" \
+        "s_mov_b64 exec, s[44:45]\n\t" \
+        "v_mov_b64 v[42:43], s[66:67]\n\t" \
+        "v_mov_b64 v[74:75], s[70:71]\n\t" \
+        "s_mov_b64 exec, -1\n\t" \
+        "v_cndmask_b32_e64 v87, v42, v74, s[46:47]\n\t" \
+        "v_cndmask_b32_e64 v43, v43, v75, s[46:47]\n\t" \
+        "s_branch .Lgbwt_walk2u_compact_landed_%=\n\t"
 #endif
 __device__ __forceinline__ uint32_t walk2_uniform_loop(const uint4 *desc2, const uint4 *cblocks , uint32_t alphabet_offset, uint32_t ring_base,
                                                        uint32_t mail_slot, uint32_t drained_addr, bool narrow, uint32_t quota, uint32_t ring_mask,
@@ -1206,6 +1279,7 @@
 #undef GBWT_WALK2U_KLOAD_NARROW
 #undef GBWT_WALK2U_FLAG_CHECK
 #undef GBWT_WALK2U_MAIL_FLAG
+#undef GBWT_WALK2U_COMPACT_PATH
 #define GBWT_WALK2U_INDEX                                                                                 \
     "v_lshrrev_b32_e32 v46, 6, v42\n\t"                                                                   \
     "v_add_u32_e32 v46, v46, v43\n\t"
@@ -1246,6 +1320,7 @@
     "global_load_dwordx3 v[56:58], v[60:61], off offset:16\n\t"
 #define GBWT_WALK2U_FLAG_CHECK
 #define GBWT_WALK2U_MAIL_FLAG "v_or_b32_e32 v50, 0x80000000, v50\n\t"
+#define GBWT_WALK2U_COMPACT_PATH(KLOAD)
 #endif
 __device__ __forceinline__ uint32_t walk2_uniform_loop_full(const uint4 *desc2, const uint4 *cblocks, uint32_t alphabet_offset, uint32_t ring_base,
                                                        uint32_t mail_slot, uint32_t drained_addr, bool narrow, uint32_t quota, uint32_t ring_mask,
@@ -1271,6 +1346,7 @@
 #undef GBWT_WALK2U_FLAG_CHECK
 #undef GBWT_WALK2U_LEAVES_DONE
 #undef GBWT_WALK2U_MAIL_FLAG
+#undef GBWT_WALK2U_COMPACT_PATH
 #endif
 
 __device__ __forceinline__ void lookahead_helper2(const uint4 *desc2, const uint4 *cblocks, uint32_t mail_slot, uint32_t done_addr, uint32_t spread) {
diff --git a/include/gbwt_hip.h b/include/gbwt_hip.h
--- a/include/gbwt_hip.h
+++ b/include/gbwt_hip.h
@@ -74,6 +74,7 @@
     uint64_t samples, checkpoint_walkers, checkpoint_orphans;
     uint32_t checkpoint_sampling, checkpoint_rounds;
     double line_sizes_ms;
+    uint64_t compact_records;
 } gbwt_hip_open_times;
 gbwt_hip_status gbwt_hip_get_open_times(const gbwt_hip_index *index, gbwt_hip_open_times *out);
 
```

Result: slower. 752.4 billion LF-steps/s (-2.1%).
